# polli-labs/linnaeus

Hardware: AMD Instinct MI355X
Metric: images/sec (train fwd+bwd) mFormerV1_sm 3x224x224 (higher is better)
Workload: dtype bf16; 1 GPU; mFormerV1_sm train step (forward + 4-task CE loss + backward + AdamW (one HIP launch)), bf16 operands / fp32 accumulate+residual, batch 256/GPU, 3x224x224 synthetic, DropPath 0.2, gradient checkpointing off; per_gpu_batch=256, global_batch=256, parallelism=dp1, grad_mode=direct

## Files before the change

include/lnx.h:

```cpp
#ifndef LNX_H
#define LNX_H
#include <stdint.h>

#ifdef __cplusplus
extern "C" {
#endif

#define LNX_F32 0
#define LNX_BF16 1

const char* lnx_last_error(void);
int lnx_version(void);
int lnx_device_cus(void);
int lnx_set_cu_margin(int cus);
int lnx_set_deterministic(int on);
int lnx_get_deterministic(void);
int lnx_tile_sched_static(void);

typedef struct lnx_rowmap {
    int group, pad, off;
} lnx_rowmap;

enum { LNX_ACT_NONE = 0, LNX_ACT_GELU = 1, LNX_ACT_RELU = 2, LNX_ACT_GELU_BWD = 3, LNX_ACT_RELU_BWD = 4,
       LNX_ACT_GELU_D = 5, LNX_ACT_MUL_AUX = 6 };
enum { LNX_ADDR_PLAIN = 0, LNX_ADDR_PATCH2 = 1 };

typedef struct lnx_gemm_args {
    int dtype;
    int M, N, K;
    const void* A;
    int64_t lda;
    const void* W;
    int64_t ldw;
    void* C;
    int64_t ldc;
    int out_f32;
    int a_mode, Hin, Win, Cin;
    int c_mode;
    lnx_rowmap c_map;
    const float* bias;
    void* c2;
    int64_t ldc2;
    int act;
    const void* aux;
    int64_t ldaux;
    const float* gamma;
    const float* rowscale;
    int rows_per_sample;
    const float* res;
    int64_t ldres;
    void* c8;
    int64_t ldc8;
    void* c8_scales;
    const int* m_dev;
    const int* perm;
} lnx_gemm_args;

int lnx_gemm_nt(const lnx_gemm_args* args, void* stream);

#define LNX_GEMM_GROUP_MAX 8
int lnx_gemm_nt_group_ok(const lnx_gemm_args* problems, int n, int accumulate);
int lnx_gemm_nt_group(const lnx_gemm_args* problems, int n, int accumulate, void* stream);

enum { LNX_NT_KERNEL_NONE = 0, LNX_NT_KERNEL_V1 = 1 , LNX_NT_KERNEL_V2 = 2 ,
       LNX_NT_KERNEL_SKINNY = 3 , LNX_NT_KERNEL_V4 = 4 ,
       LNX_NT_KERNEL_FP8 = 6 , LNX_NT_KERNEL_V7 = 7 ,
       LNX_NT_KERNEL_MX8 = 8 , LNX_NT_KERNEL_V9 = 9 ,
       LNX_NT_KERNEL_EXPERIMENT = 15 , LNX_NT_KERNEL_KINDS = 16 };
int lnx_last_nt_kernel(void);
int64_t lnx_nt_kernel_launches(int kind);
int lnx_nt_dispatch(const lnx_gemm_args* args);

int lnx_amax(const void* x, int x_dtype, int64_t ldx, int rows, int cols, float* amax, void* stream);
int lnx_quantize_fp8(const void* x, int x_dtype, int64_t ldx, int rows, int cols, const float* amax, void* y, int64_t ldy, float* scale_out, void* stream);
int lnx_gemm_nt_fp8(const lnx_gemm_args* args, const float* a_scale, const float* w_scale, void* stream);

int lnx_quantize_mxfp8(const void* x, int x_dtype, int64_t ldx, int rows, int cols, void* y, int64_t ldy, void* scales, void* stream);
int lnx_gemm_nt_mxfp8(const lnx_gemm_args* args, const void* a_scales, const void* w_scales, void* stream);

typedef struct lnx_wgrad_args {
    int dtype;
    int M, N, K;
    const void* dY;
    int64_t lddy;
    const void* A;
    int64_t lda;
    int a_mode, Hin, Win, Cin;
    float* dW;
    int64_t lddw;
    int k_perm_c;
    float* db;
    int splits;
    int k_store;
    float* ws;
    int64_t ws_floats;
    int defer;
    const int* m_dev;
} lnx_wgrad_args;
#define LNX_TN_WS_FLOATS (256 * (256 * 128 + 256))

int lnx_gemm_tn(const lnx_wgrad_args* args, void* stream);
enum { LNX_TN_KERNEL_V1 = 1 ,
       LNX_TN_KERNEL_RING = 2  };
typedef struct lnx_tn_launch {
    int kernel;
    int rw, cw;
    int patch;
    int tiles_n, tiles_k;
    int splits;
    int m_per_split;
    int workspace;
} lnx_tn_launch;
int lnx_gemm_tn_query(const lnx_wgrad_args* args, lnx_tn_launch* out);
int lnx_gemm_tn_flush(void* stream);
int lnx_gemm_tn_discard(void);


typedef struct lnx_ln_args {
    int M, C;
    float eps;
    const void* x;
    int x_dtype;
    int64_t ldx;
    lnx_rowmap x_map;
    const float* w;
    const float* b;
    void* y;
    int y_dtype;
    int64_t ldy;
    lnx_rowmap y_map;
    const void* add;
    int64_t ldadd;
    float* mean;
    float* rstd;
    void* y8;
    int64_t ldy8;
    void* y8_scales;
    const int* perm;
    const int* m_dev;
    int rows_per_sample;
} lnx_ln_args;
int lnx_layernorm_fwd(const lnx_ln_args* args, void* stream);

typedef struct lnx_ln_bwd_args {
    int M, C;
    const void* dy;
    int dy_dtype;
    int64_t lddy;
    lnx_rowmap dy_map;
    const void* x;
    int x_dtype;
    int64_t ldx;
    lnx_rowmap x_map;
    const float* w;
    const float* mean;
    const float* rstd;
    const float* gin;
    int64_t ldgin;
    void* dx;
    int dx_dtype;
    int64_t lddx;
    float* dw;
    float* db;
    int relu_mask;
    float* ws;
    int64_t ws_floats;
    void* dx2;
    int dx2_dtype;
    int64_t lddx2;
    const float* dx2_rowscale;
    int dx2_rows_per_sample;
    void* dx2_8;
    void* dx2_8_scales;
    int64_t lddx2_8;
    int defer;
    const int* perm;
    const int* m_dev;
    const int* dx2_inv;
    const int* dx2_nkeep;
} lnx_ln_bwd_args;
int lnx_layernorm_bwd(const lnx_ln_bwd_args* args, void* stream);
int lnx_layernorm_bwd_flush(void* stream);
int lnx_layernorm_bwd_discard(void);

enum { LNX_LN_COLS_NONE = 0 , LNX_LN_COLS_ATOMICS = 1 ,
       LNX_LN_COLS_WORKSPACE = 2  };
typedef struct lnx_ln_launch {
    int G;
    int V;
    int pair;
    int full;
    int mx;
    int grid;
    int cols;
    int slices;
} lnx_ln_launch;
int lnx_layernorm_fwd_query(const lnx_ln_args* args, lnx_ln_launch* out);
int lnx_layernorm_bwd_query(const lnx_ln_bwd_args* args, lnx_ln_launch* out);

typedef struct lnx_dwconv_args {
    int B, H, W, C;
    const void* x;
    int x_dtype;
    const float* w49;
    const float* bias;
    int flip;
    const float* res;
    void* y;
    int y_dtype;
} lnx_dwconv_args;
int lnx_dwconv7_fwd(const lnx_dwconv_args* args, void* stream);
int lnx_dwconv7_fwd_kept(const lnx_dwconv_args* args, const int* perm, const int* nkeep, void* stream);

typedef struct lnx_dwconv_wgrad_args {
    int B, H, W, C;
    const void* x;
    int x_dtype;
    const void* dy;
    int dy_dtype;
    float* dw;
    float* db;
    float* ws;
    int64_t ws_floats;
} lnx_dwconv_wgrad_args;
int lnx_dwconv7_wgrad(const lnx_dwconv_wgrad_args* args, void* stream);
int lnx_dwconv7_wgrad_kept(const lnx_dwconv_wgrad_args* args, const int* perm, const int* nkeep, void* stream);
int64_t lnx_dwconv7_wgrad_ws_floats(int B, int H, int W, int C, int x_dtype, int dy_dtype);

enum { LNX_ROPE_COS = 0, LNX_ROPE_ROTATE = 1 };
int lnx_rope_cos_table(const float* freqs , int heads, int H, int W, float* cos_out ,
                       float* dsin_out ,
                       void* stream);
int lnx_rope_cos_table_hd(const float* freqs, int heads, int head_dim, int H, int W, float* cos_out, float* dsin_out, void* stream);
int lnx_rope_cossin_table_hd(const float* freqs, int heads, int head_dim, int H, int W, float* cos_out, float* sin_out, float* dsin_out, void* stream);
#define LNX_ROPE_TABLES_MAX 24
typedef struct {
    const float* freqs;
    float* cos_out;
    float* dsin_out;
    int heads, H, W;
    int head_dim;
    int rope_mode;
    float* sin_out;
} lnx_rope_table;
int lnx_rope_cos_tables(const lnx_rope_table* tables, int n, void* stream);
int64_t lnx_attn_bwd_ws_floats(int B, int N, int heads);
int64_t lnx_attn_bwd_ws_floats_hd(int B, int N, int heads, int head_dim);

typedef struct lnx_attn_args {
    int dtype;
    int B, N, E, heads;
    const void* qkv;
    const float* cos_tab;
    void* o;
    float* lse;
    const unsigned char* drop_mask;
    float drop_inv_keep;
    int head_dim;
    int rope_mode;
    const float* sin_tab;
} lnx_attn_args;
int lnx_attn_fwd(const lnx_attn_args* args, void* stream);

typedef struct lnx_attn_bwd_args {
    int dtype;
    int B, N, E, heads;
    const void* qkv;
    const float* cos_tab;
// ... 708 lines not shown
```

linnaeus_amd/_lib.py:

```python
from __future__ import annotations

import ctypes as C
import os

_HERE = os.path.dirname(os.path.abspath(__file__))
LIB_PATH = os.environ.get("LNX_LIB_PATH") or os.path.join(_HERE, "liblnx_hip.so")

F32, BF16 = 0, 1
ACT_NONE, ACT_GELU, ACT_RELU, ACT_GELU_BWD, ACT_RELU_BWD, ACT_GELU_D, ACT_MUL_AUX = 0, 1, 2, 3, 4, 5, 6
TN_WS_FLOATS = 256 * (256 * 128 + 256)
DROP_PARTITION_MAX = 64


def drop_list_ints(B: int) -> int:
    return 2 * B + 2
ADDR_PLAIN, ADDR_PATCH2 = 0, 1


class LnxError(RuntimeError):
    pass


class RowMap(C.Structure):
    _fields_ = [("group", C.c_int), ("pad", C.c_int), ("off", C.c_int)]
# ... 203 lines not shown


class HierLossArgs(C.Structure):
    _fields_ = [("dtype", C.c_int), ("B", C.c_int), ("n_tasks", C.c_int), ("prob", C.c_float), ("mask_mul", C.c_int), ("draws", C.c_void_p),
                ("weights", C.c_void_p), ("ws", C.c_void_p), ("out", C.c_void_p), ("counts", C.c_void_p), ("task", HierLossTask * METRICS_MAX_TASKS)]


HIER_ROUTE_SOFT, HIER_ROUTE_HARD, HIER_ROUTE_GUMBEL = range(3)


class HierRefineLevel(C.Structure):
    _fields_ = [("base", C.c_void_p), ("out", C.c_void_p), ("dout", C.c_void_p), ("dbase", C.c_void_p), ("ld", C.c_int64), ("ldd", C.c_int64),
                ("C", C.c_int), ("mode", C.c_int), ("parent", C.c_void_p), ("child_start", C.c_void_p), ("child_idx", C.c_void_p),
                ("noise", C.c_void_p), ("temperature", C.c_float)]


class HierRefineArgs(C.Structure):
    _fields_ = [("dtype", C.c_int), ("B", C.c_int), ("n_tasks", C.c_int), ("stats", C.c_void_p), ("level", HierRefineLevel * METRICS_MAX_TASKS)]


HIER_REFINE_STRUCTS = {"lnx_hier_refine_level": HierRefineLevel, "lnx_hier_refine_args": HierRefineArgs}


ABSTAIN_MULTITASK, ABSTAIN_SEQUENTIAL = range(2)
ABSTAIN_REWARD_SIMPLE, ABSTAIN_REWARD_OUTCOME = range(2)
ABSTAIN_RANKS_ALL, ABSTAIN_RANKS_FIRST = range(2)
ABSTAIN_CORRECT, ABSTAIN_CORRECT_ABSTAIN, ABSTAIN_MISCLASSIFIED, ABSTAIN_UNNECESSARY_ABSTAIN, ABSTAIN_PREDICTED_AT_NULL, ABSTAIN_OUTCOMES = range(6)
(ABSTAIN_CNT_ABSTAINED, ABSTAIN_CNT_TOTAL, ABSTAIN_CNT_CORRECT_ABSTAIN, ABSTAIN_CNT_UNNECESSARY_ABSTAIN, ABSTAIN_CNT_MISSED_ABSTAIN,
 ABSTAIN_CNT_CORRECT_CLASSIFY, ABSTAIN_CNT_MISCLASSIFY) = range(7)
ABSTAIN_CNT_STRIDE, ABSTAIN_CNT_EPISODES, ABSTAIN_CNT_LENGTH_SUM, ABSTAIN_CNT_REWARD_FIX, ABSTAIN_COUNTS = 8, 64, 65, 66, 72
ABSTAIN_REWARD_FIX_BITS = 20
PPO_WS_LSE, PPO_WS_H, PPO_WS_LOGP, PPO_WS_COEF, PPO_WS_ROWS = range(5)
PPO_OUT_POLICY, PPO_OUT_VALUE, PPO_OUT_ENTROPY, PPO_OUT_TOTAL, PPO_OUT_N, PPO_OUT_RATIO_MEAN, PPO_OUT_CLIP_FRAC = range(7)
PPO_OUT_FLOATS = 8


class AbstainRank(C.Structure):
    _fields_ = [("logits", C.c_void_p), ("ld", C.c_int64), ("C", C.c_int), ("abstain_index", C.c_int), ("null_index", C.c_int), ("target", C.c_void_p),
                ("dlogits", C.c_void_p), ("ldd", C.c_int64)]


class AbstainActArgs(C.Structure):
    _fields_ = [("dtype", C.c_int), ("B", C.c_int), ("R", C.c_int), ("mode", C.c_int), ("greedy", C.c_int), ("reward_kind", C.c_int),
                ("reward_ranks", C.c_int), ("table", C.c_float * ABSTAIN_OUTCOMES), ("outcome_reward", C.c_float * 2), ("u", C.c_void_p),
                ("actions", C.c_void_p), ("logp", C.c_void_p), ("entropy", C.c_void_p), ("taken", C.c_void_p), ("length", C.c_void_p),
                ("reward", C.c_void_p), ("counts", C.c_void_p), ("rank", AbstainRank * METRICS_MAX_TASKS)]


class PpoAdvArgs(C.Structure):
    _fields_ = [("B", C.c_int), ("R", C.c_int), ("mode", C.c_int), ("gamma", C.c_float), ("gae_lambda", C.c_float), ("reward", C.c_void_p),
                ("value", C.c_void_p), ("length", C.c_void_p), ("adv", C.c_void_p), ("ret", C.c_void_p), ("n_trans", C.c_void_p)]


class PpoLossArgs(C.Structure):
    _fields_ = [("dtype", C.c_int), ("B", C.c_int), ("R", C.c_int), ("mode", C.c_int), ("clip_eps", C.c_float), ("vf_coef", C.c_float),
                ("ent_coef", C.c_float), ("actions", C.c_void_p), ("taken", C.c_void_p), ("logp_old", C.c_void_p), ("adv", C.c_void_p),
                ("ret", C.c_void_p), ("value", C.c_void_p), ("ws", C.c_void_p), ("out", C.c_void_p), ("dvalue", C.c_void_p),
                ("rank", AbstainRank * METRICS_MAX_TASKS)]


ABSTENTION_STRUCTS = {"lnx_abstain_rank": AbstainRank, "lnx_abstain_act_args": AbstainActArgs, "lnx_ppo_adv_args": PpoAdvArgs,
                      "lnx_ppo_loss_args": PpoLossArgs}


_lib = None


def lib() -> C.CDLL:
    global _lib
    if _lib is None:
        if not os.path.exists(LIB_PATH):
            raise LnxError(
                f"{LIB_PATH} is missing: build it with `python -c 'import __graft_entry__ as g; g.build()'` "
                "(or `make -C linnaeus_amd/csrc`). linnaeus_amd has no CPU fallback."
            )
        _lib = C.CDLL(LIB_PATH)
        _lib.lnx_last_error.restype = C.c_char_p
        _lib.lnx_nt_kernel_launches.restype = C.c_int64
        _lib.lnx_convmlp_bwd_ws_floats.restype = C.c_int64
        _lib.lnx_meta_heads_bwd_part_floats.restype = C.c_int64
        if hasattr(_lib, "lnx_set_deterministic"):
            _lib.lnx_dwconv7_wgrad_ws_floats.restype = C.c_int64
            _lib.lnx_layerscale_bwd_ws_floats.restype = C.c_int64
        _lib.lnx_attn_bwd_ws_floats.restype = C.c_int64
        _lib.lnx_attn_bwd_ws_floats_hd.restype = C.c_int64
        if hasattr(_lib, "lnx_ademamix_step"):
            _lib.lnx_ademamix_step.argtypes = [C.c_void_p, C.c_void_p, C.c_int, C.c_int, C.POINTER(AdEMAMixHyper), C.c_void_p, C.c_float, C.c_void_p]
        if hasattr(_lib, "lnx_sgd_step"):
            _lib.lnx_sgd_step.argtypes = [C.c_void_p, C.c_int, C.c_int, C.POINTER(SGDHyper), C.c_void_p, C.c_float, C.c_void_p]
            _lib.lnx_optim_launches.restype = C.c_int64
        if hasattr(_lib, "lnx_muon_step"):
            _lib.lnx_muon_layout.argtypes = [C.c_void_p, C.c_int, C.c_void_p, C.c_void_p, C.c_int64, C.POINTER(MuonInfo)]
            _lib.lnx_muon_step.argtypes = [C.POINTER(MuonStepArgs), C.c_void_p]
            _lib.lnx_muon_launches.restype = C.c_int64
        if hasattr(_lib, "lnx_muon_partition"):
            _lib.lnx_muon_partition.argtypes = [C.c_void_p, C.c_void_p, C.c_int, C.c_int, C.c_void_p, C.c_void_p, C.POINTER(C.c_int64), C.c_void_p]
            _lib.lnx_muon_orthogonalize.argtypes = [C.POINTER(MuonStepArgs), C.c_void_p, C.c_void_p, C.c_void_p, C.c_int64, C.c_void_p]
            _lib.lnx_muon_apply_packed.argtypes = [C.c_void_p, C.c_void_p, C.c_int, C.c_void_p, C.c_int64, C.c_int, C.POINTER(StepGuard), C.c_void_p]
        if hasattr(_lib, "lnx_grad_sumsq_guarded"):
            guard = C.POINTER(StepGuard)
            _lib.lnx_grad_sumsq_guarded.argtypes = [C.c_void_p, C.c_int, C.c_int, C.c_void_p, C.c_void_p, guard, C.c_void_p]
            _lib.lnx_adamw_step_guarded.argtypes = [C.c_void_p, C.c_int, C.c_int, C.POINTER(AdamWHyper), C.c_void_p, C.c_float, guard, C.c_void_p]
            _lib.lnx_ademamix_step_guarded.argtypes = [C.c_void_p, C.c_void_p, C.c_int, C.c_int, C.POINTER(AdEMAMixHyper), C.c_void_p, C.c_float, guard, C.c_void_p]
            _lib.lnx_sgd_step_guarded.argtypes = [C.c_void_p, C.c_int, C.c_int, C.POINTER(SGDHyper), C.c_void_p, C.c_float, guard, C.c_void_p]
        if hasattr(_lib, "lnx_gradnorm_sumsq"):
            _lib.lnx_gradnorm_sumsq.argtypes = [C.c_void_p, C.c_int, C.c_int, C.c_int, C.c_int64, C.c_void_p, C.c_void_p, C.c_void_p, C.c_void_p]
        if hasattr(_lib, "lnx_metrics_update"):
            _lib.lnx_metrics_update.argtypes = [C.POINTER(MetricsArgs), C.c_void_p]
            _lib.lnx_metrics_table_sizes.argtypes = [C.c_int, C.c_int, C.c_int, C.POINTER(C.c_int64), C.POINTER(C.c_int64)]
        if hasattr(_lib, "lnx_predict"):
            _lib.lnx_predict.argtypes = [C.POINTER(PredictArgs), C.c_void_p]
            _lib.lnx_predict.restype = C.c_int
        if hasattr(_lib, "lnx_hier_loss_fwd"):
            _lib.lnx_hier_loss_fwd.argtypes = [C.POINTER(HierLossArgs), C.c_void_p]
            _lib.lnx_hier_loss_bwd.argtypes = [C.POINTER(HierLossArgs), C.c_void_p, C.c_void_p]
        if hasattr(_lib, "lnx_taxonomy_rows"):
            _lib.lnx_taxonomy_rows.argtypes = [C.POINTER(TaxonomyRowsArgs), C.c_void_p]
        if hasattr(_lib, "lnx_hier_refine_fwd"):
            _lib.lnx_hier_refine_fwd.argtypes = [C.POINTER(HierRefineArgs), C.c_void_p]
            _lib.lnx_hier_refine_bwd.argtypes = [C.POINTER(HierRefineArgs), C.c_void_p]
            _lib.lnx_hier_refine_launches.restype = C.c_int64
        if hasattr(_lib, "lnx_abstain_act"):
            _lib.lnx_abstain_act.argtypes = [C.POINTER(AbstainActArgs), C.c_void_p]
            _lib.lnx_ppo_advantages.argtypes = [C.POINTER(PpoAdvArgs), C.c_void_p]
            _lib.lnx_ppo_loss_fwd.argtypes = [C.POINTER(PpoLossArgs), C.c_void_p]
            _lib.lnx_ppo_loss_bwd.argtypes = [C.POINTER(PpoLossArgs), C.c_void_p, C.c_void_p]
            _lib.lnx_abstain_launches.restype = C.c_int64
        if hasattr(_lib, "lnx_preprocess"):
            _lib.lnx_resize_taps.argtypes = [C.c_int, C.c_int, C.c_int]
            _lib.lnx_resize_coeffs.argtypes = [C.c_int, C.c_int, C.c_int, C.c_void_p, C.c_void_p]
            _lib.lnx_preprocess_scratch_bytes.argtypes = [C.POINTER(PreprocessImage), C.c_int, C.c_int, C.c_int, C.c_int]
            _lib.lnx_preprocess_scratch_bytes.restype = C.c_int64
            _lib.lnx_preprocess.argtypes = [C.POINTER(PreprocessArgs), C.c_void_p]
            _lib.lnx_preprocess.restype = C.c_int
        if hasattr(_lib, "lnx_meta_mask"):
            _lib.lnx_meta_mask.argtypes = [C.POINTER(MetaMaskArgs), C.c_void_p]
            _lib.lnx_meta_mask.restype = C.c_int
        if hasattr(_lib, "lnx_drop_partition"):
            _lib.lnx_drop_partition.argtypes = [C.c_void_p, C.c_int, C.c_int, C.c_char_p, C.POINTER(C.c_int), C.c_void_p, C.c_void_p]
            _lib.lnx_copy_dropped_rows.argtypes = [C.c_void_p, C.c_void_p, C.c_int64, C.c_void_p, C.c_void_p, C.c_int, C.c_int, C.c_int, C.c_void_p]
            _lib.lnx_drop_compact_branches.restype = C.c_int64
            if hasattr(_lib, "lnx_drop_compact_conv_blocks"):
                _lib.lnx_drop_compact_conv_blocks.restype = C.c_int64
                _lib.lnx_dwconv7_fwd_kept.argtypes = [C.POINTER(DwconvArgs), C.c_void_p, C.c_void_p, C.c_void_p]
                _lib.lnx_dwconv7_wgrad_kept.argtypes = [C.POINTER(DwconvWgradArgs), C.c_void_p, C.c_void_p, C.c_void_p]
            _lib.lnx_scale_cast_compact.argtypes = [C.c_void_p, C.c_int64, C.c_void_p, C.c_int, C.c_void_p, C.c_void_p, C.c_void_p, C.c_int, C.c_int64, C.c_int, C.c_int,
                                                    C.c_void_p]
        if hasattr(_lib, "lnx_plan_set_trainable"):
            _lib.lnx_plan_unit_name.argtypes = [C.c_void_p, C.c_int]
            _lib.lnx_plan_unit_name.restype = C.c_char_p
            _lib.lnx_plan_set_trainable.argtypes = [C.c_void_p, C.c_char_p]
        if hasattr(_lib, "lnx_gemm_tn_query"):
            _lib.lnx_gemm_tn_query.argtypes = [C.POINTER(WgradArgs), C.POINTER(TnLaunch)]
        if hasattr(_lib, "lnx_layernorm_fwd_query"):
            _lib.lnx_layernorm_fwd_query.argtypes = [C.POINTER(LnArgs), C.POINTER(LnLaunch)]
            _lib.lnx_layernorm_bwd_query.argtypes = [C.POINTER(LnBwdArgs), C.POINTER(LnLaunch)]
        older = bool(os.environ.get("LNX_LIB_PATH")) and os.environ.get("LNX_LIB_OLDER") == "1"
        for name in EXPORTS:
            if not hasattr(_lib, name) and not older:
                raise LnxError(f"{LIB_PATH} does not export {name}; rebuild it")
    return _lib


def set_deterministic(on: bool) -> bool:
    return bool(lib().lnx_set_deterministic(1 if on else 0))


def is_deterministic() -> bool:
    return bool(lib().lnx_get_deterministic())


def check(rc: int, what: str) -> None:
    if rc != 0:
        raise LnxError(f"{what} failed (rc={rc}): {lib().lnx_last_error().decode()}")


AUG_CLAMP, AUG_POSTERIZE, AUG_SOLARIZE, AUG_SOLARIZE_ADD, AUG_INVERT, AUG_BRIGHTNESS, AUG_CONTRAST = range(7)

NT_KERNEL_NONE, NT_KERNEL_V1, NT_KERNEL_V2, NT_KERNEL_SKINNY, NT_KERNEL_V4, NT_KERNEL_FP8, NT_KERNEL_V7, NT_KERNEL_MX8, NT_KERNEL_V9, NT_KERNEL_EXPERIMENT = 0, 1, 2, 3, 4, 6, 7, 8, 9, 15

ROPE_COS, ROPE_ROTATE = 0, 1

ATTN_KERNEL_NONE, ATTN_KERNEL_RES4, ATTN_KERNEL_RES8, ATTN_KERNEL_TILED4, ATTN_KERNEL_TILED8 = range(5)

EXPORTS = [
    "lnx_last_error", "lnx_version", "lnx_device_cus", "lnx_set_cu_margin", "lnx_set_deterministic", "lnx_get_deterministic", "lnx_tile_sched_static",
    "lnx_gemm_nt", "lnx_last_nt_kernel", "lnx_nt_kernel_launches", "lnx_nt_dispatch", "lnx_gemm_tn", "lnx_gemm_tn_query", "lnx_gemm_tn_flush", "lnx_gemm_tn_discard", "lnx_amax", "lnx_quantize_fp8", "lnx_gemm_nt_fp8", "lnx_quantize_mxfp8", "lnx_gemm_nt_mxfp8", "lnx_dropout_mul", "lnx_dropout_residual", "lnx_plan_dropout_bytes", "lnx_plan_set_dropout", "lnx_plan_attn_dropout_bytes", "lnx_plan_set_attn_dropout",
    "lnx_layernorm_fwd", "lnx_layernorm_bwd", "lnx_layernorm_bwd_flush", "lnx_layernorm_bwd_discard", "lnx_layernorm_fwd_query", "lnx_layernorm_bwd_query",
    "lnx_dwconv7_fwd", "lnx_dwconv7_fwd_kept", "lnx_dwconv7_wgrad", "lnx_dwconv7_wgrad_kept", "lnx_dwconv7_wgrad_ws_floats",
    "lnx_gemm_nt_group_ok", "lnx_gemm_nt_group", "lnx_rope_cos_table", "lnx_rope_cos_table_hd", "lnx_rope_cossin_table_hd", "lnx_rope_cos_tables", "lnx_attn_bwd_ws_floats", "lnx_attn_bwd_ws_floats_hd", "lnx_attn_fwd", "lnx_attn_bwd", "lnx_attn_bwd_sized", "lnx_attn_fwd_compact", "lnx_attn_bwd_compact", "lnx_attn_bwd_flush", "lnx_attn_bwd_discard", "lnx_attn_dispatch", "lnx_last_attn_kernel", "lnx_last_attn_bwd_launches",
    "lnx_im2col_stem", "lnx_scale_cast", "lnx_scale_cast_compact", "lnx_drop_partition", "lnx_copy_dropped_rows", "lnx_set_drop_compact", "lnx_drop_compact_branches", "lnx_drop_compact_conv_blocks", "lnx_layerscale_bwd", "lnx_layerscale_bwd_ws", "lnx_layerscale_bwd_ws_floats", "lnx_layerscale_apply_wgrad", "lnx_fill_rows", "lnx_colsum_rows",
    "lnx_agg2_fwd", "lnx_agg2_bwd", "lnx_pack_meta", "lnx_meta_heads_supported", "lnx_meta_heads_fwd", "lnx_meta_heads_bwd", "lnx_meta_heads_bwd_part_floats", "lnx_prep_weights", "lnx_prep_blocks", "lnx_softce", "lnx_softce_multi", "lnx_taxonomy_rows", "lnx_stem_fwd", "lnx_stem_fwd_ok", "lnx_adamw_blocks", "lnx_grad_sumsq", "lnx_adamw_step", "lnx_ademamix_step", "lnx_sgd_step", "lnx_optim_launches", "lnx_grad_sumsq_guarded", "lnx_adamw_step_guarded", "lnx_ademamix_step_guarded", "lnx_sgd_step_guarded", "lnx_muon_layout", "lnx_muon_step", "lnx_muon_launches", "lnx_muon_partition", "lnx_muon_orthogonalize", "lnx_muon_apply_packed", "lnx_gradnorm_sumsq", "lnx_gradnorm_update",
    "lnx_metrics_table_sizes", "lnx_metrics_update", "lnx_predict", "lnx_resize_taps", "lnx_resize_coeffs", "lnx_preprocess_scratch_bytes", "lnx_preprocess", "lnx_hier_loss_fwd", "lnx_hier_loss_bwd",
    "lnx_hier_refine_fwd", "lnx_hier_refine_bwd", "lnx_hier_refine_launches",
    "lnx_abstain_act", "lnx_ppo_advantages", "lnx_ppo_loss_fwd", "lnx_ppo_loss_bwd", "lnx_abstain_launches",
    "lnx_mix_rows", "lnx_mix_meta", "lnx_meta_mask",
    "lnx_aug_pointwise", "lnx_aug_saturation", "lnx_aug_rowstat", "lnx_aug_rescale", "lnx_aug_affine", "lnx_aug_stencil", "lnx_erase_rects", "lnx_u8hwc_to_f32chw",
    "lnx_convmlp_supported", "lnx_convmlp_fwd", "lnx_convmlp_bwd", "lnx_convmlp_bwd_ws_floats",
    "lnx_plan_create", "lnx_plan_destroy", "lnx_plan_workspace_bytes", "lnx_plan_num_params", "lnx_plan_param_name",
    "lnx_plan_param_numel", "lnx_plan_num_drop_calls", "lnx_plan_logits_numel", "lnx_plan_logits_offset", "lnx_plan_logits_ld",
    "lnx_plan_bind", "lnx_plan_forward", "lnx_plan_backward", "lnx_plan_backward_into", "lnx_plan_segment_params", "lnx_plan_profile_begin", "lnx_plan_profile_end", "lnx_plan_profile_begin_spans", "lnx_plan_profile_end_ex", "lnx_plan_set_wgrad_stream", "lnx_plan_set_meta_stream",
    "lnx_plan_num_units", "lnx_plan_unit_name", "lnx_plan_param_unit", "lnx_plan_set_trainable", "lnx_plan_first_trained_unit", "lnx_plan_last_backward_units",
]


class MetaHeadArgs(C.Structure):
    _fields_ = [
        ("B", C.c_int), ("C", C.c_int), ("dim", C.c_int), ("off", C.c_int),
        ("meta", C.c_void_p), ("meta_width", C.c_int), ("eps", C.c_float),
        ("w0", C.c_void_p), ("ldw0", C.c_int), ("b0", C.c_void_p), ("ln0_w", C.c_void_p), ("ln0_b", C.c_void_p),
        ("w1", C.c_void_p), ("ldw1", C.c_int), ("b1", C.c_void_p), ("ln1_w", C.c_void_p), ("ln1_b", C.c_void_p),
        ("w2", C.c_void_p), ("ldw2", C.c_int), ("b2", C.c_void_p), ("ln2_w", C.c_void_p), ("ln2_b", C.c_void_p),
        ("t0", C.c_void_p), ("h0", C.c_void_p), ("x", C.c_void_p), ("h1", C.c_void_p), ("n1", C.c_void_p), ("h2", C.c_void_p),
        ("m0", C.c_void_p), ("r0", C.c_void_p), ("m1", C.c_void_p), ("r1", C.c_void_p), ("m2", C.c_void_p), ("r2", C.c_void_p),
        ("tok", C.c_void_p), ("tok_row_stride", C.c_int64), ("tok_row_offset", C.c_int64),
    ]


class MetaHeadBwdArgs(C.Structure):
    _fields_ = [
        ("B", C.c_int), ("C", C.c_int), ("dim", C.c_int),
        ("g", C.c_void_p), ("g_row_stride", C.c_int64), ("g_row_offset", C.c_int64),
        ("w1t", C.c_void_p), ("ldw1t", C.c_int), ("w2t", C.c_void_p), ("ldw2t", C.c_int),
        ("ln0_w", C.c_void_p), ("ln1_w", C.c_void_p), ("ln2_w", C.c_void_p),
        ("t0", C.c_void_p), ("h0", C.c_void_p), ("x", C.c_void_p), ("h1", C.c_void_p), ("n1", C.c_void_p), ("h2", C.c_void_p),
        ("m0", C.c_void_p), ("r0", C.c_void_p), ("m1", C.c_void_p), ("r1", C.c_void_p), ("m2", C.c_void_p), ("r2", C.c_void_p),
        ("dp2", C.c_void_p), ("dp1", C.c_void_p), ("dp0", C.c_void_p), ("part", C.c_void_p),
        ("d_w0", C.c_void_p), ("d_b0", C.c_void_p), ("d_ln0_w", C.c_void_p), ("d_ln0_b", C.c_void_p),
        ("d_w1", C.c_void_p), ("d_b1", C.c_void_p), ("d_ln1_w", C.c_void_p), ("d_ln1_b", C.c_void_p),
        ("d_w2", C.c_void_p), ("d_b2", C.c_void_p), ("d_ln2_w", C.c_void_p), ("d_ln2_b", C.c_void_p),
    ]


class LnArgs(C.Structure):
    _fields_ = [
        ("M", C.c_int), ("C", C.c_int), ("eps", C.c_float),
        ("x", C.c_void_p), ("x_dtype", C.c_int), ("ldx", C.c_int64), ("x_map", RowMap),
        ("w", C.c_void_p), ("b", C.c_void_p),
        ("y", C.c_void_p), ("y_dtype", C.c_int), ("ldy", C.c_int64), ("y_map", RowMap),
        ("add", C.c_void_p), ("ldadd", C.c_int64),
        ("mean", C.c_void_p), ("rstd", C.c_void_p),
        ("y8", C.c_void_p), ("ldy8", C.c_int64), ("y8_scales", C.c_void_p),
        ("perm", C.c_void_p), ("m_dev", C.c_void_p), ("rows_per_sample", C.c_int),
    ]


class LnBwdArgs(C.Structure):
    _fields_ = [
        ("M", C.c_int), ("C", C.c_int),
        ("dy", C.c_void_p), ("dy_dtype", C.c_int), ("lddy", C.c_int64), ("dy_map", RowMap),
        ("x", C.c_void_p), ("x_dtype", C.c_int), ("ldx", C.c_int64), ("x_map", RowMap),
        ("w", C.c_void_p), ("mean", C.c_void_p), ("rstd", C.c_void_p),
        ("gin", C.c_void_p), ("ldgin", C.c_int64),
        ("dx", C.c_void_p), ("dx_dtype", C.c_int), ("lddx", C.c_int64),
        ("dw", C.c_void_p), ("db", C.c_void_p), ("relu_mask", C.c_int),
        ("ws", C.c_void_p), ("ws_floats", C.c_int64),
        ("dx2", C.c_void_p), ("dx2_dtype", C.c_int), ("lddx2", C.c_int64), ("dx2_rowscale", C.c_void_p), ("dx2_rows_per_sample", C.c_int),
        ("dx2_8", C.c_void_p), ("dx2_8_scales", C.c_void_p), ("lddx2_8", C.c_int64),
        ("defer", C.c_int),
        ("perm", C.c_void_p), ("m_dev", C.c_void_p), ("dx2_inv", C.c_void_p), ("dx2_nkeep", C.c_void_p),
    ]


LN_COLS_NONE, LN_COLS_ATOMICS, LN_COLS_WORKSPACE = range(3)


class LnLaunch(C.Structure):
    _fields_ = [("G", C.c_int), ("V", C.c_int), ("pair", C.c_int), ("full", C.c_int), ("mx", C.c_int), ("grid", C.c_int), ("cols", C.c_int), ("slices", C.c_int)]


class RopeTable(C.Structure):
    _fields_ = [
        ("freqs", C.c_void_p), ("cos_out", C.c_void_p), ("dsin_out", C.c_void_p),
        ("heads", C.c_int), ("H", C.c_int), ("W", C.c_int), ("head_dim", C.c_int),
        ("rope_mode", C.c_int), ("sin_out", C.c_void_p),
    ]


class DwconvArgs(C.Structure):
    _fields_ = [
        ("B", C.c_int), ("H", C.c_int), ("W", C.c_int), ("C", C.c_int),
        ("x", C.c_void_p), ("x_dtype", C.c_int), ("w49", C.c_void_p), ("bias", C.c_void_p),
        ("flip", C.c_int), ("res", C.c_void_p), ("y", C.c_void_p), ("y_dtype", C.c_int),
    ]


class DwconvWgradArgs(C.Structure):
    _fields_ = [
        ("B", C.c_int), ("H", C.c_int), ("W", C.c_int), ("C", C.c_int),
        ("x", C.c_void_p), ("x_dtype", C.c_int), ("dy", C.c_void_p), ("dy_dtype", C.c_int),
        ("dw", C.c_void_p), ("db", C.c_void_p),
        ("ws", C.c_void_p), ("ws_floats", C.c_int64),
    ]


class AttnArgs(C.Structure):
    _fields_ = [
        ("dtype", C.c_int), ("B", C.c_int), ("N", C.c_int), ("E", C.c_int), ("heads", C.c_int),
        ("qkv", C.c_void_p), ("cos_tab", C.c_void_p), ("o", C.c_void_p), ("lse", C.c_void_p),
        ("drop_mask", C.c_void_p), ("drop_inv_keep", C.c_float), ("head_dim", C.c_int),
        ("rope_mode", C.c_int), ("sin_tab", C.c_void_p),
    ]


class AttnBwdArgs(C.Structure):
    _fields_ = [
        ("dtype", C.c_int), ("B", C.c_int), ("N", C.c_int), ("E", C.c_int), ("heads", C.c_int),
        ("qkv", C.c_void_p), ("cos_tab", C.c_void_p), ("o", C.c_void_p), ("lse", C.c_void_p),
        ("d_o", C.c_void_p), ("dqkv", C.c_void_p), ("freq_ws", C.c_void_p), ("delta", C.c_void_p),
        ("drop_mask", C.c_void_p), ("drop_inv_keep", C.c_float),
        ("dsin_tab", C.c_void_p), ("dfreqs", C.c_void_p), ("defer_freqs", C.c_int), ("head_dim", C.c_int),
        ("rope_mode", C.c_int), ("sin_tab", C.c_void_p), ("grid_w", C.c_int),
    ]


class PrepDesc(C.Structure):
    _fields_ = [
        ("src", C.c_void_p), ("dst", C.c_void_p), ("dst_t", C.c_void_p),
        ("rows", C.c_int), ("cols", C.c_int), ("ld", C.c_int), ("ld_t", C.c_int),
        ("P", C.c_int), ("mode", C.c_int), ("block_start", C.c_int),
    ]


PREP_CAST, PREP_CONV_PERM, PREP_DW49 = 0, 1, 2


class ConvMlpArgs(C.Structure):
    _fields_ = [
        ("dtype", C.c_int), ("M", C.c_int), ("C", C.c_int),
        ("ln", C.c_void_p), ("w1", C.c_void_p), ("b1", C.c_void_p), ("w2", C.c_void_p), ("b2", C.c_void_p),
        ("gamma", C.c_void_p), ("rowscale", C.c_void_p), ("rows_per_sample", C.c_int),
        ("x", C.c_void_p), ("out", C.c_void_p), ("z", C.c_void_p),
        ("y", C.c_void_p), ("ln_w", C.c_void_p), ("ln_b", C.c_void_p), ("ln_eps", C.c_float), ("ln_out", C.c_void_p),
        ("mean", C.c_void_p), ("rstd", C.c_void_p),
        ("perm", C.c_void_p), ("m_dev", C.c_void_p),
    ]


class ConvMlpBwdArgs(C.Structure):
    _fields_ = [
# ... 37 lines not shown
```

linnaeus_amd/csrc/api.cpp:

```cpp
#include <hip/hip_runtime.h>
#include <stdarg.h>
#include <stdio.h>
#include <stdlib.h>
#include <string.h>

#include <atomic>
#include <mutex>

#include "../../include/lnx.h"

static thread_local char g_err[1024] = "";

void lnx_set_error(const char* fmt, ...) {
    va_list ap;
    va_start(ap, fmt);
    vsnprintf(g_err, sizeof(g_err), fmt, ap);
    va_end(ap);
}

extern "C" const char* lnx_last_error(void) { return g_err; }
extern "C" int lnx_version(void) { return 118; }
extern "C" int lnx_device_cus(void) {
    int dev = 0;
    if (hipGetDevice(&dev) != hipSuccess) return -1;
    hipDeviceProp_t prop;
    if (hipGetDeviceProperties(&prop, dev) != hipSuccess) return -1;
    return prop.multiProcessorCount;
}

static std::atomic<int> g_cu_margin{-1};
int persistent_cus(int cus) {
    int m = g_cu_margin.load(std::memory_order_relaxed);
    if (m < 0) {
        const char* e = getenv("LNX_CU_MARGIN");
        m = e ? atoi(e) : 0;
        if (m < 0) m = 0;
        g_cu_margin.store(m, std::memory_order_relaxed);
    }
    const int room = cus - m;
    return room < 8 ? 8 : room;
}
void set_cu_margin(int m) { g_cu_margin.store(m < 0 ? 0 : m, std::memory_order_relaxed); }
static std::atomic<int> g_deterministic{-1};
bool deterministic() {
    int d = g_deterministic.load(std::memory_order_relaxed);
    if (d < 0) {
        const char* e = getenv("LNX_DETERMINISTIC");
        d = e && atoi(e) == 1 ? 1 : 0;
        int unset = -1;
        if (!g_deterministic.compare_exchange_strong(unset, d, std::memory_order_relaxed)) d = unset;
    }
    return d != 0;
}
extern "C" int lnx_get_deterministic(void) { return deterministic() ? 1 : 0; }
extern "C" int lnx_set_deterministic(int on) {
    const int prev = deterministic() ? 1 : 0;
    g_deterministic.store(on ? 1 : 0, std::memory_order_relaxed);
    return prev;
}
bool tile_sched_static() {
    if (deterministic()) return true;
    const char* e = getenv("LNX_TILE_SCHED");
    return e && strcmp(e, "static") == 0;
}
extern "C" int lnx_tile_sched_static(void) { return tile_sched_static() ? 1 : 0; }
int tile_slot_of(hipStream_t st) {
    static std::mutex mu;
    static hipStream_t known[64];
    static int n = 0;
    std::lock_guard<std::mutex> lock(mu);
    for (int i = 0; i < n; ++i)
        if (known[i] == st) return i;
    if (n < 64) {
        known[n] = st;
        return n++;
    }
    return -1;
}
int device_cus() {
    static std::atomic<int> cached{0};
    int c = cached.load(std::memory_order_relaxed);
    if (c == 0) {
        c = lnx_device_cus();
        if (c > 0) cached.store(c, std::memory_order_relaxed);
    }
    return c > 0 ? c : 0;
}
extern "C" int lnx_set_cu_margin(int cus) {
    if (cus < 0 || cus > 1024) {
        lnx_set_error("lnx_set_cu_margin: %d (0..1024 compute units)", cus);
        return 1;
    }
    set_cu_margin(cus);
    return 0;
}
```

linnaeus_amd/csrc/gemm2.hip:

```cpp
#include "gemm_common.hpp"

namespace lnxg {

template <bool OUT_F32, bool PATCH, int F>
__global__ __launch_bounds__(512) void gemm_nt_v2_kernel(const GemmP p_host) {
    typedef bf16_t T;
    typedef NarrowRing R;
    constexpr int BK = R::BK;
    extern __shared__ __attribute__((aligned(16))) unsigned char smem[];

    const int tid = threadIdx.x;
    const int lane = tid & 63;
    const int wave = __builtin_amdgcn_readfirstlane(tid >> 6);
    const int wm = wave >> 1, wn = wave & 1;
    const int s = lane & 15, g = lane >> 4;

    GemmP p = p_host;
    effective_rows(p);
    int m0, n0;
    one_shot_origin<R::BM, R::BN>(p, m0, n0);
    if (m0 >= p.M) return;

    const unsigned char* src[R::PIECES];
#pragma unroll
// ... 84 lines not shown
}

template <bool OUT_F32, int F>
__global__ __launch_bounds__(512) void gemm_nt_v4_kernel(const GemmP p_host) {
    typedef bf16_t T;
    typedef WideRing R;
    extern __shared__ __attribute__((aligned(16))) unsigned char smem[];

    const int tid = threadIdx.x;
    const int lane = tid & 63;
    const int wave = __builtin_amdgcn_readfirstlane(tid >> 6);
    const int wm = wave & 1, wn = wave >> 1;
    const int s = lane & 15, g = lane >> 4;

    GemmP p = p_host;
    effective_rows(p);
    int m0, n0;
    one_shot_origin<R::BM, R::BN>(p, m0, n0);
    if (m0 >= p.M) return;

    const unsigned char* src[R::PIECES];
#pragma unroll
    for (int j = 0; j < R::PIECES; ++j) {
        const int i = wave + 8 * j;
        const int row = R::ROWS_PER_PIECE * i + (lane >> R::CHUNK_SHIFT);
        const int slot = lane & (R::CHUNKS - 1);
        if (row < R::BM) {
            const int chunk = slot ^ R::key(row);
            int m = m0 + row;
            if (m >= p.M) m = p.M - 1;
            src[j] = p.A + ((int64_t)m * p.lda + chunk * 8) * 2;
        } else {
            const int wr = row - R::BM;
            const int chunk = slot ^ R::key(wr);
            int n = n0 + wr;
            if (n >= p.N) n = p.N - 1;
            src[j] = p.W + ((int64_t)n * p.ldw + chunk * 8) * 2;
        }
    }
    auto issue_stage = [&](int kt, int stage) {
#pragma unroll
        for (int j = 0; j < R::PIECES; ++j) {
            const int i = wave + 8 * j;
            __builtin_amdgcn_global_load_lds((const __attribute__((address_space(1))) void*)(src[j] + (int64_t)kt * R::BK * 2),
                                             (__attribute__((address_space(3))) void*)(smem + stage * R::STAGE + i * 1024), 16, 0, 0);
        }
    };

    const int frag_row = (s >> 2) * 16 + (s & 3);
    const uint32_t chunk_off = (uint32_t)((g ^ (((s >> 2) & 1) * 3)) << 4);
    const uint32_t lds_base = (uint32_t)(uintptr_t)(__attribute__((address_space(3))) unsigned char*)smem;
    const uint32_t a_off = (uint32_t)((wm * 128 + frag_row) * R::ROWBYTES) + chunk_off;
    const uint32_t w_off = (uint32_t)((R::BM + wn * 64 + frag_row) * R::ROWBYTES) + chunk_off;

    f32x4_t acc0[4][4], acc1[4][4];
#pragma unroll
    for (int i = 0; i < 4; ++i)
#pragma unroll
        for (int j = 0; j < 4; ++j) {
            acc0[i][j] = f32x4_t{0.f, 0.f, 0.f, 0.f};
            acc1[i][j] = f32x4_t{0.f, 0.f, 0.f, 0.f};
        }

    const int nk = p.K / R::BK;
    issue_stage(0, 0);
    issue_stage(1, 1);
    issue_stage(2, 2);
    const int grp = wave >> 2;
    asm volatile("s_waitcnt vmcnt(8)" ::: "memory");
    __builtin_amdgcn_s_barrier();
    if (grp) __builtin_amdgcn_s_barrier();
    for (int kt = 0; kt < nk; ++kt) {
        const uint32_t st = lds_base + (kt % R::NST) * R::STAGE;
        uint4 wf[4], af0[4], af1[4];
        lds_read4<R::ROWBYTES>(wf, st + w_off);
        lds_read4<R::ROWBYTES>(af0, st + a_off);
        lds_read4<R::ROWBYTES>(af1, st + a_off + 64 * R::ROWBYTES);
        if (kt + 3 < nk) {
            issue_stage(kt + 3, (kt + 3) % R::NST);
            asm volatile("s_waitcnt vmcnt(8)" ::: "memory");
        } else if (kt + 2 < nk) {
            asm volatile("s_waitcnt vmcnt(4)" ::: "memory");
        } else {
            asm volatile("s_waitcnt vmcnt(0)" ::: "memory");
        }
        asm volatile("s_waitcnt lgkmcnt(0)" ::: "memory");
        __builtin_amdgcn_s_barrier();
        __builtin_amdgcn_sched_barrier(0);
        __builtin_amdgcn_s_setprio(1);
#pragma unroll
        for (int ni = 0; ni < 4; ++ni)
#pragma unroll
            for (int mi = 0; mi < 4; ++mi) Mfma<T>::run(acc0[ni][mi], wf[ni], af0[mi]);
#pragma unroll
        for (int ni = 0; ni < 4; ++ni)
#pragma unroll
            for (int mi = 0; mi < 4; ++mi) Mfma<T>::run(acc1[ni][mi], wf[ni], af1[mi]);
        __builtin_amdgcn_s_setprio(0);
        __builtin_amdgcn_sched_barrier(0);
        if (!(grp && kt + 1 == nk)) __builtin_amdgcn_s_barrier();
    }
    if (F == F_GENERIC) {
        gemm_epilogue<T, OUT_F32>(p, acc0, m0 + wm * 128, n0 + wn * 64, lane);
        gemm_epilogue<T, OUT_F32>(p, acc1, m0 + wm * 128 + 64, n0 + wn * 64, lane);
    } else {
        gemm_epilogue_fast<T, OUT_F32, F>(p, acc0, m0 + wm * 128, n0 + wn * 64, lane);
        gemm_epilogue_fast<T, OUT_F32, F>(p, acc1, m0 + wm * 128 + 64, n0 + wn * 64, lane);
    }
}

constexpr bool nt_v2_carries(bool out_f32, int f) { return f == F_GENERIC || nt_v4_carries(out_f32, f); }

int launch_nt_v4(const GemmP& p0, int f, bool out_f32, hipStream_t st) {
    typedef WideRing R;
    GemmP p = p0;
    p.tiles_m = cdiv(p.M, R::BM);
    p.tiles_n = p.N / R::BN;
    const int grid = p.tiles_m * p.tiles_n;
    return with_nt_form<nt_v4_carries>("gemm_nt_v4", out_f32, f, [&](auto form) {
        using Form = decltype(form);
        return launch_with_lds<gemm_nt_v4_kernel<Form::out_f32, Form::f>>(grid, 512, R::NST * R::STAGE, st, p);
    });
}

int launch_nt_v2(const GemmP& p0, int f, bool out_f32, hipStream_t st) {
    typedef NarrowRing R;
    GemmP p = p0;
    p.tiles_m = cdiv(p.M, R::BM);
    p.tiles_n = cdiv(p.N, R::BN);
    const int grid = p.tiles_m * p.tiles_n;
    const size_t lds = R::NST * R::STAGE;
    const bool patch = p.a_mode == LNX_ADDR_PATCH2;
    LNX_CHECK(!patch || f == F_GENERIC, "gemm_nt_v2: the 2x2 patch gather is compiled with the generic epilogue only (f = %d)", f);
    return with_nt_form<nt_v2_carries>("gemm_nt_v2", out_f32, f, [&](auto form) {
        using Form = decltype(form);
        if constexpr (Form::f == F_GENERIC) {
            if (patch) return launch_with_lds<gemm_nt_v2_kernel<Form::out_f32, true, Form::f>>(grid, 512, lds, st, p);
        }
        return launch_with_lds<gemm_nt_v2_kernel<Form::out_f32, false, Form::f>>(grid, 512, lds, st, p);
    });
}

constexpr int TBM = 64;
__device__ const uint4 g_tn_zero16 = {0u, 0u, 0u, 0u};

#define DS_READ_TR2(lo, hi, addr, off2)                                                                                  \
    do {                                                                                                                 \
        const uint32_t a_ = (addr);                                                                                      \
        asm volatile("ds_read_b64_tr_b16 %0, %1" : "=v"(lo) : "v"(a_) : "memory");                                       \
        asm volatile("ds_read_b64_tr_b16 %0, %1 offset:%2" : "=v"(hi) : "v"(a_), "i"(off2) : "memory");                 \
    } while (0)

template <int RW, int CW, bool PATCH>
__global__ __launch_bounds__(512) void gemm_tn_v2_kernel(const WgradP p) {
    typedef bf16_t T;
    constexpr int RROW = RW * 2, CROW = CW * 2;
    constexpr int RBYTES = TBM * RROW, CBYTES = TBM * CROW;
    constexpr int STG = RBYTES + CBYTES;
    constexpr int RINS = RBYTES / 1024, CINS = CBYTES / 1024;
    constexpr int NINS = (RINS + CINS) / 8;
    constexpr int WC = CW / 64;
    extern __shared__ __attribute__((aligned(16))) unsigned char smem[];

    const int tid = threadIdx.x;
    const int lane = tid & 63;
    const int wave = __builtin_amdgcn_readfirstlane(tid >> 6);
    const int wr = wave / WC, wc = wave % WC;
    const int s = lane & 15, g = lane >> 4;

    int bid = xcd_remap(blockIdx.x, p.tiles_n * p.tiles_k * p.splits);
    const int split = bid / (p.tiles_n * p.tiles_k);
    bid -= split * (p.tiles_n * p.tiles_k);
    const int tc = bid % p.tiles_k;
    const int tr = bid / p.tiles_k;
    const int n0 = tr * RW, k0 = tc * CW;
    int m_all = p.M, m_per = p.m_per_split;
    if (p.m_dev) {
        m_all = min(p.M, max(*p.m_dev, 0));
        const int mt = (m_all + TBM - 1) / TBM;
        m_per = (mt + p.splits - 1) / p.splits * TBM;
    }
    const int m_begin = split * m_per;
    const int m_end = min(m_all, m_begin + m_per);
    if (m_begin >= m_end && !(p.m_dev && p.ws)) return;
    const int ntile = m_begin < m_end ? (m_end - m_begin + TBM - 1) / TBM : 0;

    const unsigned char* src[NINS];
    int64_t step[NINS];
    int pr[NINS], po[NINS];
    const int Wo = PATCH ? p.pg.Win >> 1 : 1;
    const int qa = TBM / Wo, qb = TBM - qa * Wo;
#pragma unroll
    for (int j = 0; j < NINS; ++j) {
        pr[j] = po[j] = 0;
        const int i = wave + 8 * j;
        if (i < RINS) {
            constexpr int CPR = RW / 8, RPI = 64 / CPR;
            const int row = i * RPI + lane / CPR, slot = lane % CPR;
            int col = n0 + ((slot ^ ((row & 7) << 1)) << 3);
            const int lim = ((p.N + 7) >> 3) << 3;
            if (col >= lim) col = lim - 8;
            src[j] = p.dY + ((int64_t)(m_begin + row) * p.lddy + col) * 2;
            step[j] = (int64_t)TBM * p.lddy * 2;
        } else {
            constexpr int CPR = CW / 8, RPI = 64 / CPR;
            const int row = (i - RINS) * RPI + lane / CPR, slot = lane % CPR;
            int col = k0 + ((slot ^ ((row & 7) << 1)) << 3);
            const int lim = ((p.K + 7) >> 3) << 3;
            if (col >= lim) col = lim - 8;
            if (PATCH) {
                src[j] = p.A + patch_col(p.pg, col) * 2;
                step[j] = (int64_t)p.pg.Cin * 4;
                const int m = m_begin + row, t = m / Wo;
                pr[j] = m - t * Wo;
                po[j] = m + t * Wo;
            } else {
                src[j] = p.A + ((int64_t)(m_begin + row) * p.lda + col) * 2;
                step[j] = (int64_t)TBM * p.lda * 2;
            }
        }
    }
    int m_issue = m_begin;
    auto issue_tile = [&](int stage) {
        const bool ragged = m_issue + TBM > m_end;
#pragma unroll
        for (int j = 0; j < NINS; ++j) {
            const int i = wave + 8 * j;
            const unsigned char* gp = src[j];
            if (PATCH && i >= RINS) {
                gp += (int64_t)po[j] * step[j];
                const int r = pr[j] + qb;
                const bool wrap = r >= Wo;
                pr[j] = wrap ? r - Wo : r;
                po[j] += TBM + (qa + (wrap ? 1 : 0)) * Wo;
            } else {
                src[j] += step[j];
            }
            if (ragged) {
                const int row = i < RINS ? i * (64 / (RW / 8)) + lane / (RW / 8) : (i - RINS) * (64 / (CW / 8)) + lane / (CW / 8);
                if (m_issue + row >= m_end) gp = reinterpret_cast<const unsigned char*>(&g_tn_zero16);
            }
            __builtin_amdgcn_global_load_lds((const __attribute__((address_space(1))) void*)gp,
                                             (__attribute__((address_space(3))) void*)(smem + stage * STG + i * 1024), 16, 0, 0);
        }
        m_issue += TBM;
    };

    const int q = s >> 2, pp = s & 3;
    uint32_t offR[2][4], offC[2][4];
#pragma unroll
    for (int ks = 0; ks < 2; ++ks) {
        const int row = ks * 32 + 4 * g + q;
        const int key = (row & 7) << 1;
#pragma unroll
        for (int i = 0; i < 4; ++i) {
            const int cr = (wr * 64 + i * 16 + 4 * pp) >> 3, cc = (wc * 64 + i * 16 + 4 * pp) >> 3;
            offR[ks][i] = row * RROW + ((cr ^ key) << 4) + (pp & 1) * 8;
            offC[ks][i] = RBYTES + row * CROW + ((cc ^ key) << 4) + (pp & 1) * 8;
        }
    }
    const uint32_t lds_base = (uint32_t)(uintptr_t)(__attribute__((address_space(3))) unsigned char*)smem;

    f32x4_t acc[4][4], accb[4];
#pragma unroll
    for (int i = 0; i < 4; ++i) {
        accb[i] = f32x4_t{0.f, 0.f, 0.f, 0.f};
#pragma unroll
        for (int j = 0; j < 4; ++j) acc[i][j] = f32x4_t{0.f, 0.f, 0.f, 0.f};
    }
    const bool do_bias = p.db != nullptr && tc == 0 && wc == 0;
    const uint4 ones = make_uint4(0x3F803F80u, 0x3F803F80u, 0x3F803F80u, 0x3F803F80u);

    if (ntile > 0) issue_tile(0);
    if (ntile > 1) issue_tile(1);
    const int grp = wave >> 2;
    if (ntile > 1) asm volatile("s_waitcnt vmcnt(6)" ::: "memory");
    else asm volatile("s_waitcnt vmcnt(0)" ::: "memory");
    __builtin_amdgcn_s_barrier();
    if (grp && ntile > 0) __builtin_amdgcn_s_barrier();
    for (int t = 0; t < ntile; ++t) {
        const uint32_t st = lds_base + (t % NarrowRing::NST) * STG;
        uint2 rl[2][4], rh[2][4], cl[2][4], chh[2][4];
#pragma unroll
        for (int ks = 0; ks < 2; ++ks)
#pragma unroll
            for (int i = 0; i < 4; ++i) {
                DS_READ_TR2(rl[ks][i], rh[ks][i], st + offR[ks][i], 16 * RROW);
                DS_READ_TR2(cl[ks][i], chh[ks][i], st + offC[ks][i], 16 * CROW);
            }
        if (t + 2 < ntile) {
            issue_tile((t + 2) % NarrowRing::NST);
            asm volatile("s_waitcnt vmcnt(6)" ::: "memory");
        } else {
            asm volatile("s_waitcnt vmcnt(0)" ::: "memory");
        }
        asm volatile("s_waitcnt lgkmcnt(0)" ::: "memory");
        __builtin_amdgcn_s_barrier();
        __builtin_amdgcn_sched_barrier(0);
        __builtin_amdgcn_s_setprio(1);
#pragma unroll
        for (int ks = 0; ks < 2; ++ks) {
            uint4 rf[4], cf[4];
#pragma unroll
            for (int i = 0; i < 4; ++i) {
                rf[i] = make_uint4(rl[ks][i].x, rl[ks][i].y, rh[ks][i].x, rh[ks][i].y);
                cf[i] = make_uint4(cl[ks][i].x, cl[ks][i].y, chh[ks][i].x, chh[ks][i].y);
            }
#pragma unroll
            for (int ri = 0; ri < 4; ++ri)
#pragma unroll
                for (int ci = 0; ci < 4; ++ci) Mfma<T>::run(acc[ri][ci], rf[ri], cf[ci]);
            if (do_bias) {
#pragma unroll
                for (int ri = 0; ri < 4; ++ri) Mfma<T>::run(accb[ri], rf[ri], ones);
            }
        }
        __builtin_amdgcn_s_setprio(0);
        __builtin_amdgcn_sched_barrier(0);
        if (!(grp && t + 1 == ntile)) __builtin_amdgcn_s_barrier();
    }
    if (p.ws) {
        const int tiles = p.tiles_n * p.tiles_k;
        float4* wt = reinterpret_cast<float4*>(p.ws + (size_t)(split * tiles + tr * p.tiles_k + tc) * (RW * CW)) + (wave * 16) * 64 + lane;
#pragma unroll
        for (int ri = 0; ri < 4; ++ri)
#pragma unroll
            for (int ci = 0; ci < 4; ++ci) wt[(ri * 4 + ci) * 64] = make_float4(acc[ri][ci][0], acc[ri][ci][1], acc[ri][ci][2], acc[ri][ci][3]);
        if (do_bias && s == 0) {
#pragma unroll
            for (int ri = 0; ri < 4; ++ri)
#pragma unroll
                for (int r = 0; r < 4; ++r)
                    p.ws[(size_t)p.splits * tiles * (RW * CW) + (size_t)(split * p.tiles_n + tr) * RW + wr * 64 + ri * 16 + 4 * g + r] = accb[ri][r];
        }
        return;
    }
#pragma unroll
    for (int ri = 0; ri < 4; ++ri) {
#pragma unroll
        for (int r = 0; r < 4; ++r) {
            const int n = n0 + wr * 64 + ri * 16 + 4 * g + r;
            if (n >= p.N) continue;
#pragma unroll
            for (int ci = 0; ci < 4; ++ci) {
                const int k = k0 + wc * 64 + ci * 16 + s;
                if (k >= p.k_store) continue;
                int col = k;
                if (p.k_perm_c > 0) {
                    const int P = p.K / p.k_perm_c;
                    const int pq = k / p.k_perm_c;
                    col = (k - pq * p.k_perm_c) * P + pq;
                }
                atomicAdd(p.dW + (int64_t)n * p.lddw + col, acc[ri][ci][r]);
            }
            if (do_bias && s == 0) atomicAdd(p.db + n, accb[ri][r]);
        }
    }
}

__device__ __forceinline__ void tn_reduce_body(const WgradP& p, int RW, int CW, const int64_t idx) {
    const int tiles = p.tiles_n * p.tiles_k;
    const int tile_f4 = RW * CW / 4;
    const size_t tile_floats = (size_t)RW * CW;
    if (idx < (int64_t)tiles * tile_f4) {
        const int tile = (int)(idx / tile_f4), f = (int)(idx - (int64_t)tile * tile_f4);
        const int tr = tile / p.tiles_k, tc = tile - tr * p.tiles_k;
        const int lane = f & 63, ci = (f >> 6) & 3, ri = (f >> 8) & 3, wave = f >> 10;
        const int WC = CW / 64, wr = wave / WC, wc = wave - wr * WC;
        const int n0 = tr * RW + wr * 64 + ri * 16 + 4 * (lane >> 4);
        const int k = tc * CW + wc * 64 + ci * 16 + (lane & 15);
        if (n0 >= p.N || k >= p.k_store) return;
        const float4* src = reinterpret_cast<const float4*>(p.ws + (size_t)tile * tile_floats) + f;
        float4 part[8];
#pragma unroll
        for (int j = 0; j < 8; ++j) part[j] = make_float4(0.f, 0.f, 0.f, 0.f);
        const size_t sstep = (size_t)tiles * tile_floats / 4;
        int sp = 0;
        for (; sp + 8 <= p.splits; sp += 8) {
            float4 v[8];
#pragma unroll
            for (int j = 0; j < 8; ++j) v[j] = src[(size_t)(sp + j) * sstep];
#pragma unroll
            for (int j = 0; j < 8; ++j) {
                part[j].x += v[j].x;
                part[j].y += v[j].y;
                part[j].z += v[j].z;
                part[j].w += v[j].w;
            }
        }
        for (; sp < p.splits; ++sp) {
            const float4 v = src[(size_t)sp * sstep];
            part[0].x += v.x;
            part[0].y += v.y;
            part[0].z += v.z;
            part[0].w += v.w;
        }
#pragma unroll
        for (int w = 4; w > 0; w >>= 1)
#pragma unroll
            for (int j = 0; j < w; ++j) {
                part[j].x += part[j + w].x;
                part[j].y += part[j + w].y;
                part[j].z += part[j + w].z;
                part[j].w += part[j + w].w;
            }
        const float av[4] = {part[0].x, part[0].y, part[0].z, part[0].w};
        int col = k;
        if (p.k_perm_c > 0) {
            const int P = p.K / p.k_perm_c;
            const int pq = k / p.k_perm_c;
            col = (k - pq * p.k_perm_c) * P + pq;
        }
#pragma unroll
        for (int r = 0; r < 4; ++r)
            if (n0 + r < p.N) p.dW[(int64_t)(n0 + r) * p.lddw + col] += av[r];
    } else if (p.db != nullptr) {
        const int64_t n = idx - (int64_t)tiles * tile_f4;
        if (n < p.N) {
            const int tr = (int)n / RW;
            const float* src = p.ws + (size_t)p.splits * tiles * tile_floats + (size_t)tr * RW + (n - tr * RW);
            float a = 0.f;
            for (int sp = 0; sp < p.splits; ++sp) a += src[(size_t)sp * p.tiles_n * RW];
            p.db[n] += a;
        }
    }
}

__global__ __launch_bounds__(256) void gemm_tn_reduce_kernel(const WgradP p, int RW, int CW) {
    tn_reduce_body(p, RW, CW, (int64_t)blockIdx.x * 256 + threadIdx.x);
}

constexpr int TN_BATCH = 8;
struct TnReduceDesc {
    WgradP p;
    int RW, CW, block_start;
};
struct TnReduceBatch {
    TnReduceDesc d[TN_BATCH];
    int n;
};
__global__ __launch_bounds__(256) void gemm_tn_reduce_batch_kernel(const TnReduceBatch b) {
    int j = 0;
#pragma unroll
    for (int i = 1; i < TN_BATCH; ++i)
        if (i < b.n && (int)blockIdx.x >= b.d[i].block_start) j = i;
    tn_reduce_body(b.d[j].p, b.d[j].RW, b.d[j].CW, (int64_t)((int)blockIdx.x - b.d[j].block_start) * 256 + threadIdx.x);
}

static thread_local TnReduceBatch g_tn_pending = {};
static thread_local int g_tn_pending_blocks = 0;
static thread_local hipStream_t g_tn_pending_stream = nullptr;

int tn_flush(hipStream_t st) {
    if (g_tn_pending.n == 0) return 0;
    if (st != nullptr && st != g_tn_pending_stream) return 1;
    hipLaunchKernelGGL(gemm_tn_reduce_batch_kernel, dim3((unsigned)g_tn_pending_blocks), dim3(256), 0, g_tn_pending_stream, g_tn_pending);
    g_tn_pending.n = 0;
    g_tn_pending_blocks = 0;
    return 0;
}

int tn_discard() {
    const int n = g_tn_pending.n;
    g_tn_pending.n = 0;
    g_tn_pending_blocks = 0;
    g_tn_pending_stream = nullptr;
    return n;
}

int launch_tn_v2(const WgradP& p, const TnPlan& t, hipStream_t st, bool defer) {
    static_assert(TBM == TN_RING_ROWS, "tn_plan splits the contraction in this kernel's ring stages");
    const bool wide_r = t.RW == 256, patch = t.patch;
    const int RW = t.RW, CW = t.CW;
    const int tiles = p.tiles_n * p.tiles_k;
    const int grid = tiles * p.splits;
    const size_t lds = NarrowRing::NST * (size_t)(TBM * (RW + CW) * 2);
    int rc;
    if (wide_r) rc = patch ? launch_with_lds<gemm_tn_v2_kernel<256, 128, true>>(grid, 512, lds, st, p) : launch_with_lds<gemm_tn_v2_kernel<256, 128, false>>(grid, 512, lds, st, p);
    else rc = patch ? launch_with_lds<gemm_tn_v2_kernel<128, 256, true>>(grid, 512, lds, st, p) : launch_with_lds<gemm_tn_v2_kernel<128, 256, false>>(grid, 512, lds, st, p);
    if (rc != 0) return rc;
    if (p.ws) {
        const int64_t work = (int64_t)tiles * (RW * CW / 4) + (p.db ? p.N : 0);
        const int blocks = (int)cdiv(work, 256);
        if (defer) {
            if (g_tn_pending.n > 0 && (g_tn_pending_stream != st || g_tn_pending.n == TN_BATCH)) (void)tn_flush(nullptr);
            TnReduceDesc& d = g_tn_pending.d[g_tn_pending.n++];
            d.p = p;
            d.RW = RW;
            d.CW = CW;
            d.block_start = g_tn_pending_blocks;
            g_tn_pending_blocks += blocks;
            g_tn_pending_stream = st;
        } else {
            hipLaunchKernelGGL(gemm_tn_reduce_kernel, dim3((unsigned)blocks), dim3(256), 0, st, p, RW, CW);
        }
    }
    return 0;
}

}
```

linnaeus_amd/csrc/gemm_common.hpp:

```cpp
#pragma once
#include "common.hpp"
#include "../../include/lnx.h"

namespace lnxg {

constexpr int TILE = 128;
constexpr int ROWB = 128;
constexpr int TILE_BYTES = TILE * ROWB;

struct PatchGeom {
    int Hin, Win, Cin;
};

struct GemmP {
    const unsigned char* A;
    const unsigned char* W;
    unsigned char* C;
    unsigned char* C2;
    const unsigned char* aux;
    const float* bias;
    const float* gamma;
    const float* rowscale;
    const float* res;
    int64_t lda, ldw, ldc, ldc2, ldaux, ldres;
// ... 430 lines not shown
    if (p.N % 16 != 0 || !al16(p.C) || (p.ldc * (out_f32 ? 4 : esz)) % 16 != 0) return F_GENERIC;
    const int64_t lim = (int64_t)1 << 31;
    if ((int64_t)p.M * p.ldc >= lim) return F_GENERIC;
    int f = 0;
    if (p.bias) {
        if (!al16(p.bias)) return F_GENERIC;
        f |= F_BIAS;
    }
    if (p.C2) {
        if (!al16(p.C2) || (p.ldc2 * esz) % 16 != 0 || (int64_t)p.M * p.ldc2 >= lim) return F_GENERIC;
        f |= F_C2;
    }
    if (p.act == LNX_ACT_GELU) f |= F_GELU;
    else if (p.act == LNX_ACT_GELU_D) {
        if (!p.C2) return F_GENERIC;
        f |= F_GELU;
    } else if (p.act == LNX_ACT_GELU_BWD || p.act == LNX_ACT_MUL_AUX) {
        if (!al16(p.aux) || (p.ldaux * esz) % 16 != 0 || (int64_t)p.M * p.ldaux >= lim) return F_GENERIC;
        f |= F_GELU_BWD;
    } else if (p.act != LNX_ACT_NONE) return F_GENERIC;
    if (p.res) {
        if (!al16(p.res) || (p.ldres * 4) % 16 != 0 || (int64_t)p.M * p.ldres >= lim) return F_GENERIC;
        f |= F_RES;
    }
    if (p.rowscale && !p.res) return F_GENERIC;
    if (!out_f32 && (f == 0 || f == F_BIAS || f == (F_BIAS | F_C2 | F_GELU) || f == (F_BIAS | F_GELU) || f == F_GELU_BWD)) return f;
    if (out_f32 && f == (F_BIAS | F_RES)) return f;
    return F_GENERIC;
}

struct WgradP {
    const unsigned char* dY;
    const unsigned char* A;
    float* dW;
    float* db;
    int64_t lddy, lda, lddw;
    int M, N, K;
    int a_mode;
    PatchGeom pg;
    int k_perm_c, k_store;
    float* ws;
    int64_t ws_floats;
    int tiles_n, tiles_k, splits, m_per_split;
    const int* m_dev = nullptr;
};


struct NtSwitches {
    bool force_v1;
    bool skinny;
    bool v4;
    bool tile_cost;
    bool generic_epi;
    int v7, v9;
    bool fp8_x8;
};
NtSwitches nt_switches();

void fill_gemm_p(const lnx_gemm_args* a, GemmP& p);

struct NtChoice {
    int kind, f;
};
NtChoice nt_choose(const GemmP& p, int dtype, bool out_f32);

typedef int (*nt_experiment_fn)(const GemmP& p, int f, bool out_f32, hipStream_t st);
extern nt_experiment_fn g_nt_experiment;

void note_nt_kernel(int kind);

template <bool O, int FF>
struct NtForm {
    static constexpr bool out_f32 = O;
    static constexpr int f = FF;
};
int nt_form_error(const char* family, bool out_f32, int f);

template <auto Carries, bool O, int FF, class Launch>
int nt_form_case(const char* family, Launch& launch) {
    if constexpr (Carries(O, FF)) return launch(NtForm<O, FF>{});
    else return nt_form_error(family, O, FF);
}

template <auto Carries, class Launch>
int with_nt_form(const char* family, bool out_f32, int f, Launch&& launch) {
    if (f == F_GENERIC) return out_f32 ? nt_form_case<Carries, true, F_GENERIC>(family, launch) : nt_form_case<Carries, false, F_GENERIC>(family, launch);
    if (out_f32) {
        if (f == (F_BIAS | F_RES)) return nt_form_case<Carries, true, F_BIAS | F_RES>(family, launch);
        return nt_form_error(family, out_f32, f);
    }
    switch (f) {
        case 0: return nt_form_case<Carries, false, 0>(family, launch);
        case F_BIAS: return nt_form_case<Carries, false, F_BIAS>(family, launch);
        case F_BIAS | F_C2 | F_GELU: return nt_form_case<Carries, false, F_BIAS | F_C2 | F_GELU>(family, launch);
        case F_BIAS | F_C2 | F_GELU | F_MXOUT: return nt_form_case<Carries, false, F_BIAS | F_C2 | F_GELU | F_MXOUT>(family, launch);
        case F_BIAS | F_GELU: return nt_form_case<Carries, false, F_BIAS | F_GELU>(family, launch);
        case F_GELU_BWD: return nt_form_case<Carries, false, F_GELU_BWD>(family, launch);
        case F_GELU_BWD | F_MXOUT: return nt_form_case<Carries, false, F_GELU_BWD | F_MXOUT>(family, launch);
    }
    return nt_form_error(family, out_f32, f);
}

int launch_nt_v1(const GemmP& p, int dtype, bool out_f32, hipStream_t st);
int launch_tn_v1(const WgradP& p, int dtype, hipStream_t st);

bool nt_skinny_ok(const GemmP& p, int dtype, bool out_f32);
int launch_nt_skinny(const GemmP& p, bool out_f32, hipStream_t st);
int launch_nt_skinny_group(const GemmP* ps, int n, bool accumulate, bool out_f32, hipStream_t st);

int launch_nt_v2(const GemmP& p, int f, bool out_f32, hipStream_t st);
int launch_nt_v4(const GemmP& p, int f, bool out_f32, hipStream_t st);

constexpr bool nt_v4_carries(bool out_f32, int f) {
    if (out_f32) return f == (F_BIAS | F_RES);
    return f == 0 || f == F_BIAS || f == (F_BIAS | F_C2 | F_GELU) || f == (F_BIAS | F_GELU) || f == F_GELU_BWD;
}

inline bool fits_32bit_offsets(const GemmP& p) {
    const int64_t lim = (int64_t)1 << 31;
    return (int64_t)p.M * p.lda * 2 < lim && (int64_t)p.N * p.ldw * 2 < lim;
}
template <class R>
int persistent_geometry(GemmP& p, hipStream_t st, size_t& lds) {
    const int ntiles = p.tiles_m * p.tiles_n;
    const int cus = device_cus();
    if (cus <= 0) return 0;
    const int room = persistent_cus(cus);
    lds = R::NST * R::STAGE + 16;
    p.tile_slot = tile_sched_static() ? -1 : tile_slot_of(st);
    return ntiles < room ? ntiles : room;
}

bool nt_v7_ok(const GemmP& p, int f, bool out_f32);
int launch_nt_v7(const GemmP& p, int f, bool out_f32, hipStream_t st);

bool nt_v9_ok(const GemmP& p, int f, bool out_f32);
int launch_nt_v9(const GemmP& p, int f, bool out_f32, hipStream_t st);

constexpr int TN_RING_ROWS = 64;
struct TnPlan {
    bool ring;
    int RW, CW;
    bool patch;
    int tiles_n, tiles_k, splits, m_per_split;
    bool workspace;
};
TnPlan tn_plan(const WgradP& p, int dtype, int splits_hint);

int launch_tn_v2(const WgradP& p, const TnPlan& t, hipStream_t st, bool defer);
int tn_flush(hipStream_t st);
int tn_discard();
bool tn_v2_ok(const WgradP& p, int dtype);

}
using namespace lnxg;
```

linnaeus_amd/csrc/gemm_tn_dispatch.cpp:

```cpp
#include <stdlib.h>

#include "gemm_common.hpp"

namespace lnxg {

bool tn_v2_ok(const WgradP& p, int dtype) {
    return dtype == LNX_BF16 && p.M % TN_RING_ROWS == 0 && p.M >= 4096 && p.N >= 8 && p.K >= 8;
}

TnPlan tn_plan(const WgradP& p, int dtype, int splits_hint) {
    TnPlan t{};
    t.patch = p.a_mode == LNX_ADDR_PATCH2;
    t.ring = tn_v2_ok(p, dtype) && !nt_switches().force_v1;
    if (!t.ring) {
        t.RW = t.CW = TILE;
        t.tiles_n = cdiv(p.N, TILE);
        t.tiles_k = cdiv(p.K, TILE);
        const int bmc = dtype == LNX_BF16 ? 64 : 32;
        int splits = splits_hint;
        if (splits <= 0) {
            const int tiles = t.tiles_n * t.tiles_k;
            splits = cdiv(2 * 256, tiles);
            const int max_splits = cdiv(p.M, 4 * bmc);
            if (splits > max_splits) splits = max_splits;
            if (splits < 1) splits = 1;
        }
        if (deterministic()) splits = 1;
        int mps = cdiv(p.M, splits);
        mps = cdiv(mps, bmc) * bmc;
        t.splits = cdiv(p.M, mps);
        t.m_per_split = mps;
        t.workspace = false;
        return t;
    }
    auto waste = [&](int rw, int cw) { return (double)cdiv(p.N, rw) * rw * cdiv(p.K, cw) * cw; };
    static const char* force = getenv("LNX_TN_ORIENT");
    const bool wide_r = force ? force[0] == 'r' : waste(256, 128) <= waste(128, 256);
    const int RW = wide_r ? 256 : 128, CW = wide_r ? 128 : 256;
    t.RW = RW;
    t.CW = CW;
    t.tiles_n = cdiv(p.N, RW);
    t.tiles_k = cdiv(p.K, CW);
    const int tiles = t.tiles_n * t.tiles_k;
    const int mtiles = p.M / TN_RING_ROWS;
    int splits = splits_hint;
    if (splits <= 0) {
        splits = 256 / tiles;
        if (splits < 1) splits = 1;
        const int max_splits = mtiles / 8 > 0 ? mtiles / 8 : 1;
        if (splits > max_splits) splits = max_splits;
    }
    if (splits > mtiles) splits = mtiles;
    if (splits < 1) splits = 1;
    const bool det = deterministic();
    auto ws_need = [&](int sp) { return (size_t)sp * tiles * (256 * 128) + (size_t)sp * t.tiles_n * RW; };
    const size_t have = p.ws ? (size_t)p.ws_floats : 0;
    if (det) {
        while (splits > 1 && ws_need(cdiv(mtiles, cdiv(mtiles, splits))) > have) --splits;
    }
    const int per = cdiv(mtiles, splits);
    t.m_per_split = per * TN_RING_ROWS;
    t.splits = cdiv(mtiles, per);
    static const bool no_ws = getenv("LNX_TN_ATOMIC") != nullptr;
    const bool sparse_tiles = (double)p.N * p.k_store < 0.7 * (double)tiles * (256 * 128);
    if (det) t.workspace = t.splits >= 2;
    else t.workspace = !(no_ws || p.ws == nullptr || have < ws_need(t.splits) || t.splits < 2 || sparse_tiles);
    return t;
}

}

namespace {

int tn_check_sizes(const lnx_wgrad_args* a, const char* who) {
    LNX_CHECK(a != nullptr, "%s: null args", who);
    LNX_CHECK(a->dtype == LNX_F32 || a->dtype == LNX_BF16, "%s: bad dtype %d", who, a->dtype);
    const int epv = a->dtype == LNX_F32 ? 4 : 8;
    LNX_CHECK(a->M > 0 && a->N > 0 && a->K > 0, "%s: empty problem", who);
    LNX_CHECK(a->lddy % epv == 0 && a->lddy >= (int64_t)cdiv(a->N, epv) * epv, "%s: lddy=%lld must be a multiple of %d and >= roundup(N)", who, (long long)a->lddy, epv);
    LNX_CHECK(a->K % epv == 0, "%s: K=%d must be a multiple of %d", who, a->K, epv);
    if (a->a_mode == LNX_ADDR_PATCH2) {
        LNX_CHECK(a->Hin % 2 == 0 && a->Win % 2 == 0 && a->Cin % epv == 0 && a->K == 4 * a->Cin, "%s: bad PATCH2 geometry", who);
    } else {
        LNX_CHECK(a->lda % epv == 0, "%s: lda must be a multiple of %d", who, epv);
    }
    if (a->k_perm_c > 0) LNX_CHECK(a->K % a->k_perm_c == 0, "%s: K %% k_perm_c != 0", who);
    return 0;
}

void fill_wgrad_p(const lnx_wgrad_args* a, WgradP& p) {
    p.dY = (const unsigned char*)a->dY;
    p.A = (const unsigned char*)a->A;
    p.dW = a->dW;
    p.db = a->db;
    p.lddy = a->lddy;
    p.lda = a->lda;
    p.lddw = a->lddw;
    p.M = a->M;
    p.N = a->N;
    p.K = a->K;
    p.a_mode = a->a_mode;
    p.pg = PatchGeom{a->Hin, a->Win, a->Cin};
    p.k_perm_c = a->k_perm_c;
    p.ws = a->ws;
    p.ws_floats = a->ws ? a->ws_floats : 0;
    p.k_store = (a->k_store > 0 && a->k_store < a->K) ? a->k_store : a->K;
    p.m_dev = a->m_dev;
}

}

extern "C" int lnx_gemm_tn_query(const lnx_wgrad_args* a, lnx_tn_launch* out) {
    LNX_CHECK(out != nullptr, "lnx_gemm_tn_query: null result");
    if (tn_check_sizes(a, "lnx_gemm_tn_query") != 0) return 1;
    WgradP p;
    fill_wgrad_p(a, p);
    const TnPlan t = tn_plan(p, a->dtype, a->splits);
    out->kernel = t.ring ? LNX_TN_KERNEL_RING : LNX_TN_KERNEL_V1;
    out->rw = t.RW;
    out->cw = t.CW;
    out->patch = t.patch ? 1 : 0;
    out->tiles_n = t.tiles_n;
    out->tiles_k = t.tiles_k;
    out->splits = t.splits;
    out->m_per_split = t.m_per_split;
    out->workspace = t.workspace ? 1 : 0;
    return 0;
}

extern "C" int lnx_gemm_tn(const lnx_wgrad_args* a, void* stream) {
    if (tn_check_sizes(a, "lnx_gemm_tn") != 0) return 1;
    LNX_CHECK(a->dY && a->A && a->dW, "lnx_gemm_tn: null operand");
    LNX_CHECK((((uintptr_t)a->A) & 15) == 0 && (((uintptr_t)a->dY) & 15) == 0, "lnx_gemm_tn: operands must be 16-byte aligned");
    WgradP p;
    fill_wgrad_p(a, p);
    const TnPlan t = tn_plan(p, a->dtype, a->splits);
    p.tiles_n = t.tiles_n;
    p.tiles_k = t.tiles_k;
    p.splits = t.splits;
    p.m_per_split = t.m_per_split;
    if (t.ring && !t.workspace) p.ws = nullptr;
    hipStream_t st = (hipStream_t)stream;
    static const bool no_defer = getenv("LNX_TN_NO_DEFER") != nullptr;
    int rc;
    if (t.ring) rc = launch_tn_v2(p, t, st, a->defer != 0 && !no_defer);
    else rc = launch_tn_v1(p, a->dtype, st);
    if (rc != 0) return rc;
    LNX_LAUNCH_CHECK();
    return 0;
}
```

linnaeus_amd/csrc/plan.cpp:

```cpp
#include <hip/hip_runtime.h>
#include <stdlib.h>
#include <string.h>

#include <mutex>
#include <atomic>
#include <string>
#include <vector>

#include "../../include/lnx.h"

void lnx_set_error(const char* fmt, ...);

#define RUN(expr)                  \
    do {                           \
        const int rc_ = (expr);    \
        if (rc_ != 0) return rc_;  \
    } while (0)
#define FAIL(...)                   \
    do {                            \
        lnx_set_error(__VA_ARGS__); \
        return 1;                   \
    } while (0)
#define HIPRUN(expr)                                                         \
    do {                                                                     \
        const hipError_t e_ = (expr);                                        \
        if (e_ != hipSuccess) FAIL("%s: %s", #expr, hipGetErrorString(e_)); \
    } while (0)

namespace {

constexpr int LN_DEFER_SLOTS = 16;
constexpr int FREQ_DEFER_SLOTS = 8;

inline int64_t align_up(int64_t v, int64_t a) { return (v + a - 1) / a * a; }

struct OpW {
    int param = -1;
    int N = 0, K = 0;
    int ld = 0;
    int ld_t = 0;
    int mode = LNX_PREP_CAST, P = 0;
    bool f32 = false;
    int64_t off = 0, off_t = 0;
    int64_t off8 = 0, off8s = 0;
    int64_t off8t = 0, off8ts = 0;
};

struct ConvBlk {
    bool fused = false;
    bool fused_ln = false;
    int gamma, dww, dwb, lnw, lnb, b1, b2;
    OpW w1, w2;
    int64_t w49;
    int64_t xin, y, ln, mean, rstd, hpre, act, z;
};
struct RopeBlk {
    int n1w, n1b, n2w, n2b, freqs, qkvb, projb, fc1b, fc2b;
    OpW qkv, proj, fc1, fc2;
    int64_t xin, n1, mean1, rstd1, qkvbuf, cos, dsin, o, lse, xmid, n2, mean2, rstd2, hpre, act;
    int64_t dm_proj = 0, dm_hid = 0, dm_fc2 = 0;
    int64_t dm_attn = 0;
};
struct MetaHead {
    int b0, lnw0, lnb0, nf1w, nf1b, nf2w, nf2b, b1, b2;
    OpW w0, w1, w2;
    int dim, off;
    int64_t t0, h0, x, m0, r0, h1, n1, m1, r1, h2, m2, r2;
    int64_t dp2 = 0, dp1 = 0, dp0 = 0, part = 0;
};
struct Down {
    int lnw, lnb, cb;
    OpW w;
    int64_t ln, mean, rstd;
};

}

constexpr int TN_WS_SLOTS = 4;

struct lnx_plan {
    lnx_mformer_cfg c;
    int esz;
    int E;
    int H[4], W[4], HW[4];
    int Ntok[2];
    std::vector<std::string> names;
    std::vector<int64_t> numel;
    std::vector<signed char> seg;
    std::vector<std::string> unit_names;
    std::vector<int> unit_of;
    int u_conv[2] = {0, 0}, u_down[2] = {0, 0}, u_tok[2] = {0, 0}, u_rope[2] = {0, 0}, u_mid = 0, u_tail = 0, u_heads = 0;
    int cut = 0;
    bool frozen_prefix = true;
    int bwd_units = 0;
    bool runs(int unit) const { return unit >= cut; }
    std::vector<const float*> P;
    std::vector<float*> G;
    bool bound = false, has_grads = false, fwd_done = false;
    unsigned char* ws = nullptr;
    int64_t ws_bytes = 0;

    int stem_b, stem_lnw, stem_lnb, cls[2], norm_w[2], norm_b[2], fin_w, fin_b, agg_w, agg_b, cl_b1, cl_b2, cl_lnw, cl_lnb;
    OpW stem_w, cl_w1, cl_w2;
    std::vector<int> head_b;
    std::vector<OpW> head_w;
    std::vector<int> logit_ld;
    std::vector<int64_t> logit_off;
    int64_t logits_numel = 0;
    Down down[3];
    std::vector<ConvBlk> conv[2];
    std::vector<RopeBlk> rope[2];
    std::vector<MetaHead> meta[2];
    std::vector<OpW*> all_w;
    std::vector<int> drop_conv[2], drop_attn[2], drop_mlp[2];
    int n_drop = 0;

    int64_t o_descs = 0, n_descs = 0, prep_blocks = 0;
    int64_t arena_end = 0;
    int64_t n_descs_t = 0, n_descs_f = 0, prep_blocks_f = 0;
    int64_t o_patches, o_stem_pre, o_stem_mean, o_stem_rstd;
    int64_t o_stage_out[4];
    int64_t o_tok[2];
    int64_t o_t1, o_t1_mean, o_t1_rstd;
    int64_t o_cl_hpre, o_cl_act, o_cl_u, o_cl_mean, o_cl_rstd, o_c1n;
    int64_t o_c2n, o_n2_mean, o_n2_rstd, o_agg, o_fin_mean, o_fin_rstd, o_feats, o_featsT;
    int64_t o_g[4];
    int64_t o_sA, o_sB = 0, o_sC, o_sD;
    int64_t o_lnws = 0, lnws_floats = 0, o_lnws_side = 0, lnws_side_floats = 0;
    int64_t lnws_defer_floats = 0;
    int64_t o_lnws_defer = 0;
    int ln_pending = 0;
    int64_t gcos_floats = 0;
    int freq_pending = 0;
    bool freq_defer = true;
    bool ln_defer = true;
    int64_t o_tnws = 0;
    int64_t o_lsws = 0, lsws_floats = 0;
    bool det = false;
    int64_t o_detws = 0, detws_floats = 0;
    int64_t o_gcos , o_delta, o_dt1, o_tail[6], o_mtmp[4], o_dlT;
    int64_t o_a8 = 0, o_a8s = 0, o_h8 = 0, o_h8s = 0;
    const float* last_drop = nullptr;
    const unsigned char* last_mask = nullptr;
    std::vector<unsigned char> mask_host;
    const float* last_meta = nullptr;
    int resident[4] = {-1, -1, -1, -1};
    const unsigned char* dmask = nullptr;
    float inv_keep = 1.0f;
    int64_t dmask_bytes = 0;
    const unsigned char* amask = nullptr;
    float a_inv_keep = 1.0f;
    int64_t amask_bytes = 0;
    hipStream_t side = nullptr;
    hipEvent_t ev_fork = nullptr, ev_meta = nullptr, ev_bfork[2] = {nullptr, nullptr}, ev_bjoin[2] = {nullptr, nullptr};
    hipStream_t wgs = nullptr;
    bool wgs_on = true;
    bool meta_forked[2] = {false, false};
    int meta_mode = 1;
    bool meta_chain = true;
    bool chain_ok[2] = {false, false};
    bool dy8_ready = false;
    hipEvent_t ev_wf[4] = {nullptr, nullptr, nullptr, nullptr}, ev_wj[4] = {nullptr, nullptr, nullptr, nullptr};
    bool profile = false;
    bool profile_spans = false;
    struct Span { hipEvent_t e0, e1; int cls; double work, bytes; };
    std::vector<Span> spans;
    std::vector<hipEvent_t> ev_pool;
    size_t ev_used = 0;

    template <typename U> U* at(int64_t off) const { return reinterpret_cast<U*>(ws + off); }
    const float* drop_ptr(int call) const {
        if (last_drop == nullptr || call < 0 || !mask_host[call]) return nullptr;
        return last_drop + (int64_t)call * c.batch;
    }
    int* droplists = nullptr;
    bool compact_now = false;
    bool compact_conv_now = false;
    const int* drop_list(int call) const {
        if (!compact_now || droplists == nullptr || drop_ptr(call) == nullptr) return nullptr;
        return droplists + (int64_t)call * LNX_DROP_LIST_INTS(c.batch);
    }
};

static std::atomic<int> g_drop_compact{-1};
static std::atomic<long long> g_compact_branches{0};
extern "C" int lnx_set_drop_compact(int on) {
    const int was = g_drop_compact.exchange(on < 0 ? -1 : (on ? 1 : 0));
    return was;
}
extern "C" int64_t lnx_drop_compact_branches(void) { return (int64_t)g_compact_branches.load(std::memory_order_relaxed); }
static std::atomic<long long> g_compact_conv_blocks{0};
extern "C" int64_t lnx_drop_compact_conv_blocks(void) { return (int64_t)g_compact_conv_blocks.load(std::memory_order_relaxed); }

namespace {

bool env_set(const char* name) { return getenv(name) != nullptr; }
bool env_off(const char* name) {
    const char* e = getenv(name);
    return e != nullptr && atoi(e) == 0;
}

OpW make_w(lnx_plan* p, int param, int N, int K, bool want_t, int mode = LNX_PREP_CAST, int P = 0, bool f32 = false) {
    OpW w;
    w.param = param;
    w.N = N;
    w.K = K;
    w.f32 = f32 || p->esz == 4;
    const int epv = w.f32 ? 4 : 8;
    w.ld = (int)align_up(K, epv);
    if (K < 16) w.ld = 16;
    w.ld_t = want_t ? (int)align_up(N, epv) : 0;
    w.mode = mode;
    w.P = P;
    return w;
}

void build_params(lnx_plan* p) {
    const lnx_mformer_cfg& c = p->c;
    const int* D = c.dims;
    const int B = c.batch;
    char b[128];
    auto add = [&](const std::string& name, int64_t numel, int seg) {
        p->names.push_back(name);
        p->numel.push_back(numel);
        p->seg.push_back((signed char)seg);
        return (int)p->names.size() - 1;
    };
    p->cls[0] = add("cls_token_1", D[2], 1);
    p->cls[1] = add("cls_token_2", D[3], 0);
    p->stem_w = make_w(p, add("stem.0.weight", (int64_t)D[0] * c.in_chans * 16, 3), D[0], c.in_chans * 16, false);
    p->stem_w.ld = 64;
    p->stem_b = add("stem.0.bias", D[0], 3);
    p->stem_lnw = add("stem.1.weight", D[0], 3);
    p->stem_lnb = add("stem.1.bias", D[0], 3);
    for (int i = 0; i < 3; ++i) {
        snprintf(b, sizeof b, "downsample_layers.%d.", i);
        const std::string pre(b);
        Down& k = p->down[i];
        const int seg = 2 - i;
        k.lnw = add(pre + "norm.weight", D[i], seg);
        k.lnb = add(pre + "norm.bias", D[i], seg);
        k.w = make_w(p, add(pre + "conv.weight", (int64_t)D[i + 1] * D[i] * 4, seg), D[i + 1], 4 * D[i], true, LNX_PREP_CONV_PERM, 4);
        k.cb = add(pre + "conv.bias", D[i + 1], seg);
    }
    int call = 0;
    for (int s = 0; s < 2; ++s) {
        p->conv[s].resize(c.conv_depths[s]);
        for (int i = 0; i < c.conv_depths[s]; ++i) {
            snprintf(b, sizeof b, "stages.%d.%d.", s, i);
            const std::string pre(b);
            ConvBlk& k = p->conv[s][i];
            const int C = D[s], seg = 3 - s;
            k.gamma = add(pre + "gamma", C, seg);
            k.dww = add(pre + "dwconv.weight", (int64_t)C * 49, seg);
            k.dwb = add(pre + "dwconv.bias", C, seg);
            k.lnw = add(pre + "norm.weight", C, seg);
            k.lnb = add(pre + "norm.bias", C, seg);
            k.w1 = make_w(p, add(pre + "pwconv1.weight", (int64_t)4 * C * C, seg), 4 * C, C, true);
            k.b1 = add(pre + "pwconv1.bias", 4 * C, seg);
            k.w2 = make_w(p, add(pre + "pwconv2.weight", (int64_t)4 * C * C, seg), C, 4 * C, true);
            k.b2 = add(pre + "pwconv2.bias", C, seg);
            p->drop_conv[s].push_back(call++);
        }
    }
    for (int s = 0; s < 2; ++s) {
        p->rope[s].resize(c.rope_depths[s]);
        for (int i = 0; i < c.rope_depths[s]; ++i) {
            snprintf(b, sizeof b, "stages.%d.%d.", s + 2, i);
            const std::string pre(b);
            RopeBlk& k = p->rope[s][i];
            const int C = D[2 + s], hid = c.mlp_hidden[s], seg = 1 - s;
            k.n1w = add(pre + "norm1.weight", C, seg);
            k.n1b = add(pre + "norm1.bias", C, seg);
            k.n2w = add(pre + "norm2.weight", C, seg);
            k.n2b = add(pre + "norm2.bias", C, seg);
            k.freqs = add(pre + "attn.freqs", C, seg);
            k.qkv = make_w(p, add(pre + "attn.qkv.weight", (int64_t)3 * C * C, seg), 3 * C, C, true);
            k.qkvb = add(pre + "attn.qkv.bias", 3 * C, seg);
            k.proj = make_w(p, add(pre + "attn.proj.weight", (int64_t)C * C, seg), C, C, true);
            k.projb = add(pre + "attn.proj.bias", C, seg);
            k.fc1 = make_w(p, add(pre + "mlp.fc1.weight", (int64_t)hid * C, seg), hid, C, true);
            k.fc1b = add(pre + "mlp.fc1.bias", hid, seg);
            k.fc2 = make_w(p, add(pre + "mlp.fc2.weight", (int64_t)C * hid, seg), C, hid, true);
            k.fc2b = add(pre + "mlp.fc2.bias", C, seg);
            p->drop_attn[s].push_back(call++);
            p->drop_mlp[s].push_back(call++);
        }
    }
    p->n_drop = call;
    for (int s = 0; s < 2; ++s) {
        snprintf(b, sizeof b, "norm_%d.", s + 1);
        p->norm_w[s] = add(std::string(b) + "weight", D[2 + s], 0);
        p->norm_b[s] = add(std::string(b) + "bias", D[2 + s], 0);
        p->meta[s].resize(c.n_meta);
    }
    int off = 0;
    for (int m = 0; m < c.n_meta; ++m) {
        for (int s = 0; s < 2; ++s) {
            snprintf(b, sizeof b, "meta.%d.head_%d.", m, s + 1);
            const std::string pre(b);
            MetaHead& k = p->meta[s][m];
            const int C = D[2 + s], seg = 2 - s;
            k.dim = c.meta_dims[m];
            k.off = off;
            k.w0 = make_w(p, add(pre + "0.weight", (int64_t)C * k.dim, seg), C, k.dim, false, LNX_PREP_CAST, 0, true);
            k.b0 = add(pre + "0.bias", C, seg);
            k.lnw0 = add(pre + "2.weight", C, seg);
            k.lnb0 = add(pre + "2.bias", C, seg);
            k.nf1w = add(pre + "3.norm_fn1.weight", C, seg);
            k.nf1b = add(pre + "3.norm_fn1.bias", C, seg);
            k.nf2w = add(pre + "3.norm_fn2.weight", C, seg);
            k.nf2b = add(pre + "3.norm_fn2.bias", C, seg);
            k.w1 = make_w(p, add(pre + "3.w1.weight", (int64_t)C * C, seg), C, C, true, LNX_PREP_CAST, 0, true);
            k.b1 = add(pre + "3.w1.bias", C, seg);
            k.w2 = make_w(p, add(pre + "3.w2.weight", (int64_t)C * C, seg), C, C, true, LNX_PREP_CAST, 0, true);
            k.b2 = add(pre + "3.w2.bias", C, seg);
        }
        off += c.meta_dims[m];
    }
    if (!c.only_last_cls) {
        p->cl_w1 = make_w(p, add("cl_1_fc.0.fc1.weight", (int64_t)D[2] * D[2], 0), D[2], D[2], true);
        p->cl_b1 = add("cl_1_fc.0.fc1.bias", D[2], 0);
        p->cl_w2 = make_w(p, add("cl_1_fc.0.fc2.weight", (int64_t)D[3] * D[2], 0), D[3], D[2], true);
        p->cl_b2 = add("cl_1_fc.0.fc2.bias", D[3], 0);
        p->cl_lnw = add("cl_1_fc.1.weight", D[3], 0);
        p->cl_lnb = add("cl_1_fc.1.bias", D[3], 0);
        p->agg_w = add("aggregate.weight", 2, 0);
        p->agg_b = add("aggregate.bias", 1, 0);
    }
    p->fin_w = add("final_norm.weight", D[3], 0);
    p->fin_b = add("final_norm.bias", D[3], 0);
    p->head_w.resize(c.n_tasks);
    p->head_b.resize(c.n_tasks);
    p->logit_ld.resize(c.n_tasks);
    p->logit_off.resize(c.n_tasks);
    for (int t = 0; t < c.n_tasks; ++t) {
        snprintf(b, sizeof b, "head.%d.", t);
        p->head_w[t] = make_w(p, add(std::string(b) + "weight", (int64_t)c.task_classes[t] * D[3], 0), c.task_classes[t], D[3], true);
        p->head_b[t] = add(std::string(b) + "bias", c.task_classes[t], 0);
        p->logit_ld[t] = (int)align_up(c.task_classes[t], 8);
        p->head_w[t].ld_t = p->logit_ld[t];
        p->logit_off[t] = p->logits_numel;
        p->logits_numel += (int64_t)B * p->logit_ld[t];
    }
}

bool build_units(lnx_plan* p) {
    const lnx_mformer_cfg& c = p->c;
    char b[64];
    auto unit = [&](const std::string& name) {
        p->unit_names.push_back(name);
        return (int)p->unit_names.size() - 1;
    };
    auto blocks = [&](int stage, int depth) {
        const int first = (int)p->unit_names.size();
        for (int i = 0; i < depth; ++i) {
            snprintf(b, sizeof b, "stages.%d.%d", stage, i);
            unit(b);
        }
        return first;
    };
    unit("stem");
    for (int s = 0; s < 2; ++s) {
        p->u_conv[s] = blocks(s, c.conv_depths[s]);
        snprintf(b, sizeof b, "downsample_layers.%d", s);
        p->u_down[s] = unit(b);
    }
    p->u_tok[0] = unit("tokens_1");
    p->u_rope[0] = blocks(2, c.rope_depths[0]);
    p->u_mid = unit("mid");
    p->u_tok[1] = unit("tokens_2");
    p->u_rope[1] = blocks(3, c.rope_depths[1]);
    p->u_tail = unit("tail");
    p->u_heads = unit("heads");
    auto starts = [](const std::string& s, const char* pre) { return s.compare(0, strlen(pre), pre) == 0; };
    p->unit_of.assign(p->names.size(), -1);
    for (size_t i = 0; i < p->names.size(); ++i) {
        const std::string& n = p->names[i];
        int u = -1, s = 0, k = 0, m = 0;
        if (starts(n, "stem.")) u = 0;
        else if (sscanf(n.c_str(), "stages.%d.%d.", &s, &k) == 2 && s >= 0 && s < 4) u = (s < 2 ? p->u_conv[s] : p->u_rope[s - 2]) + k;
        else if (sscanf(n.c_str(), "downsample_layers.%d.", &s) == 1) u = s < 2 ? p->u_down[s] : p->u_mid;
        else if (sscanf(n.c_str(), "cls_token_%d", &s) == 1 && (s == 1 || s == 2)) u = p->u_tok[s - 1];
        else if (sscanf(n.c_str(), "meta.%d.head_%d.", &m, &s) == 2 && (s == 1 || s == 2)) u = p->u_tok[s - 1];
        else if (starts(n, "norm_1.") || starts(n, "cl_1_fc.")) u = p->u_mid;
        else if (starts(n, "norm_2.") || starts(n, "aggregate.") || starts(n, "final_norm.")) u = p->u_tail;
        else if (starts(n, "head.")) u = p->u_heads;
        if (u < 0 || u >= (int)p->unit_names.size()) return false;
        p->unit_of[i] = u;
    }
    return true;
}

struct Carver {
    int64_t cur = 0;
    int64_t take(int64_t bytes) {
        const int64_t o = cur;
        cur += align_up(bytes > 0 ? bytes : 16, 256);
        return o;
    }
};

}

static void layout_workspace(lnx_plan* p);

extern "C" int lnx_plan_create(const lnx_mformer_cfg* cfg, lnx_plan** out) {
    if (!cfg || !out) FAIL("lnx_plan_create: null argument");
    const lnx_mformer_cfg& c = *cfg;
    if (c.dtype != LNX_F32 && c.dtype != LNX_BF16) FAIL("lnx_plan_create: bad dtype %d", c.dtype);
    if (c.batch <= 0 || c.img_h <= 0 || c.img_w <= 0 || c.in_chans <= 0 || c.in_chans > 4) FAIL("lnx_plan_create: bad input geometry");
    if (c.img_h % 32 != 0 || c.img_w % 32 != 0) FAIL("lnx_plan_create: image size %dx%d must be divisible by 32 (4*2*2*2 patchify)", c.img_h, c.img_w);
    for (int i = 0; i < 4; ++i)
        if (c.dims[i] <= 0 || c.dims[i] % 32 != 0 || c.dims[i] > 2048) FAIL("lnx_plan_create: dims[%d]=%d must be a multiple of 32 in (0, 2048]", i, c.dims[i]);
    for (int s = 0; s < 2; ++s) {
        if (c.conv_depths[s] < 0 || c.rope_depths[s] <= 0) FAIL("lnx_plan_create: bad depths");
        const int hd = c.rope_heads[s] > 0 && c.dims[2 + s] % c.rope_heads[s] == 0 ? c.dims[2 + s] / c.rope_heads[s] : 0;
        if (hd != 32 && hd != 64 && hd != 128)
            FAIL("lnx_plan_create: head_dim = dim / heads must be 32, 64 or 128 (dim %d, heads %d)", c.dims[2 + s], c.rope_heads[s]);
        if (c.mlp_hidden[s] <= 0 || c.mlp_hidden[s] % 16 != 0) FAIL("lnx_plan_create: mlp_hidden must be a multiple of 16");
    }
    if (c.n_meta < 0 || c.n_meta > LNX_MAX_META || c.n_tasks < 0 || c.n_tasks > LNX_MAX_TASKS) FAIL("lnx_plan_create: too many meta components / tasks");
    for (int m = 0; m < c.n_meta; ++m)
        if (c.meta_dims[m] <= 0 || c.meta_dims[m] > 16) FAIL("lnx_plan_create: meta dim %d must be in 1..16", c.meta_dims[m]);
    if (c.rope_mode != LNX_ROPE_COS && c.rope_mode != LNX_ROPE_ROTATE) FAIL("lnx_plan_create: rope_mode %d (LNX_ROPE_COS or LNX_ROPE_ROTATE)", c.rope_mode);

    if (c.fp8) {
        if (c.dtype != LNX_BF16) FAIL("lnx_plan_create: fp8 = 1 needs dtype = LNX_BF16 (fp8 operands, bf16 storage)");
        for (int s = 0; s < 2; ++s)
            if (c.dims[2 + s] % 128 != 0 || c.mlp_hidden[s] % 128 != 0)
                FAIL("lnx_plan_create: fp8 = 1 needs RoPE dims and MLP widths that are multiples of 128 (stage %d: %d / %d)", s + 2, c.dims[2 + s], c.mlp_hidden[s]);
    }
    lnx_plan* p = new lnx_plan();
    p->c = c;
    p->esz = c.dtype == LNX_BF16 ? 2 : 4;
    p->meta_chain = !env_off("LNX_META_CHAIN");
    p->ln_defer = !env_off("LNX_LN_DEFER");
    p->det = lnx_get_deterministic() != 0;
    p->freq_defer = !env_off("LNX_FREQ_DEFER");
    for (int s = 0; s < 2; ++s) p->chain_ok[s] = p->meta_chain && lnx_meta_heads_supported(c.dims[2 + s]) != 0;
    p->E = 1 + c.n_meta;
    p->H[0] = c.img_h / 4;
    p->W[0] = c.img_w / 4;
    for (int i = 1; i < 4; ++i) {
        p->H[i] = p->H[i - 1] / 2;
        p->W[i] = p->W[i - 1] / 2;
    }
    for (int i = 0; i < 4; ++i) p->HW[i] = p->H[i] * p->W[i];
    for (int s = 0; s < 2; ++s) p->Ntok[s] = p->HW[2 + s] + p->E;
    build_params(p);
    p->frozen_prefix = !env_off("LNX_FROZEN_PREFIX");
    if (!build_units(p)) {
        delete p;
        FAIL("lnx_plan_create: a parameter without a unit (build_units does not know its name)");
    }

    auto reg = [&](OpW& w) { p->all_w.push_back(&w); };
    reg(p->stem_w);
    for (int i = 0; i < 3; ++i) reg(p->down[i].w);
    for (int s = 0; s < 2; ++s)
        for (auto& k : p->conv[s]) {
            reg(k.w1);
            reg(k.w2);
        }
    for (int s = 0; s < 2; ++s)
        for (auto& k : p->rope[s]) {
            reg(k.qkv);
            reg(k.proj);
            reg(k.fc1);
            reg(k.fc2);
        }
    for (int s = 0; s < 2; ++s)
        for (auto& k : p->meta[s]) {
            reg(k.w0);
            reg(k.w1);
            reg(k.w2);
        }
    if (!c.only_last_cls) {
        reg(p->cl_w1);
        reg(p->cl_w2);
    }
    for (auto& w : p->head_w) reg(w);
    layout_workspace(p);
    *out = p;
    return 0;
}

static void layout_workspace(lnx_plan* p) {
    const lnx_mformer_cfg& c = p->c;
    const int* D = c.dims;
    const int B = c.batch;
    const int esz = p->esz;
    const int cut = p->cut;
    p->dmask_bytes = p->amask_bytes = 0;
    p->detws_floats = 0;
    Carver cv;
    int ndw = 0;
    for (int s = 0; s < 2; ++s) ndw += c.conv_depths[s];
    p->n_descs = (int64_t)p->all_w.size() + ndw;
    p->o_descs = cv.take(p->n_descs * sizeof(lnx_prep_desc));
    for (OpW* w : p->all_w) {
        const int wes = w->f32 ? 4 : 2;
        w->off = cv.take((int64_t)w->N * w->ld * wes);
        if (w->ld_t) w->off_t = cv.take((int64_t)w->K * w->ld_t * wes);
    }
    p->arena_end = cv.cur;
    for (int s = 0; s < 2; ++s)
        for (auto& k : p->conv[s]) k.w49 = cv.take((int64_t)49 * D[s] * 4);
    if (c.fp8) {
        const bool fp8_dgrad = !c.inference && !env_off("LNX_FP8_DGRAD");
        for (int s = 0; s < 2; ++s)
            for (auto& k : p->rope[s]) {
                for (OpW* w : {&k.qkv, &k.fc1, &k.fc2}) {
                    w->off8 = cv.take((int64_t)w->N * w->K);
                    w->off8s = cv.take((int64_t)(w->K / 128) * w->N * 4);
                }
                if (fp8_dgrad)
                    for (OpW* w : {&k.proj, &k.fc1, &k.fc2}) {
                        w->off8t = cv.take((int64_t)w->K * w->N);
                        w->off8ts = cv.take((int64_t)(w->N / 128) * w->K * 4);
                    }
            }
    }

    const int64_t M0 = (int64_t)B * p->HW[0];
    p->o_patches = cv.take(M0 * 64 * esz);
    p->o_stem_pre = cv.take(M0 * D[0] * esz);
    p->o_stem_mean = cv.take(M0 * 4);
    p->o_stem_rstd = cv.take(M0 * 4);
    int64_t maxMC = 0, maxM4C = 0;
    int64_t fwdMC = 0;
    bool any_fused = false;
    const bool inf = c.inference != 0;
    const bool ck = !inf && c.recompute != 0;
    const bool fuse_mlp = !env_set("LNX_NO_FUSED_MLP"), fuse_ln = !env_set("LNX_NO_FUSED_LN");
    int fuse_maxc = 2048;
    if (const char* e = getenv("LNX_FUSED_MLP_MAXC")) fuse_maxc = atoi(e);
    p->lnws_floats = (int64_t)2048 * 2 * (D[3] > D[0] ? D[3] : D[0]);
    p->lnws_side_floats = (int64_t)256 * 2 * D[3];
    if (p->det)
        for (int s = 0; s < 2; ++s) {
            const int64_t need = lnx_convmlp_bwd_ws_floats((int)D[s], (int)((int64_t)B * p->HW[s]));
            if (need > p->lnws_floats) p->lnws_floats = need;
        }
    auto frozen_blocks = [&](int first_unit, size_t nb) {
        if (inf || cut <= first_unit) return 0;
        return cut - first_unit < (int)nb ? cut - first_unit : (int)nb;
    };
    for (int s = 0; s < 2; ++s) {
        const int64_t M = (int64_t)B * p->HW[s], C = D[s];
        const bool active = cut <= p->u_down[s];
        if (active && M * C > maxMC) maxMC = M * C;
        if (active && M * 4 * C > maxM4C) maxM4C = M * 4 * C;
        int64_t pp[2] = {0, 0};
        if (inf) {
            pp[0] = cv.take(M * C * 4);
            pp[1] = cv.take(M * C * 4);
        }
        const size_t nb = p->conv[s].size();
        const int nf = frozen_blocks(p->u_conv[s], nb);
        auto stream_buf = [&](size_t k) {
            if (inf) return pp[k & 1];
            if ((int)k > nf) return cv.take(M * C * 4);
            if (pp[k & 1] == 0) pp[k & 1] = cv.take(M * C * 4);
            return pp[k & 1];
        };
        for (size_t i = 0; i < nb; ++i) {
            ConvBlk& k = p->conv[s][i];
            const bool share = i > 0 && (inf || ck || (int)i < nf);
            const ConvBlk& f = p->conv[s][0];
            k.xin = stream_buf(i);
            k.y = share ? f.y : cv.take(M * C * esz);
            k.ln = share ? f.ln : cv.take(M * C * esz);
            k.mean = share ? f.mean : cv.take(M * 4);
            k.rstd = share ? f.rstd : cv.take(M * 4);
            k.fused = lnx_convmlp_supported(c.dtype, (int)C) != 0 && fuse_mlp && C <= fuse_maxc;
            any_fused = any_fused || k.fused;
            k.fused_ln = k.fused && fuse_ln && lnx_convmlp_bwd_ws_floats((int)C, (int)M) <= p->lnws_floats;
            if (!k.fused) {
                k.hpre = share ? f.hpre : cv.take(M * 4 * C * esz);
                k.act = share ? f.act : cv.take(M * 4 * C * esz);
                k.z = share ? f.z : cv.take(M * C * esz);
            }
        }
        p->o_stage_out[s] = stream_buf(nb);
        p->down[s].ln = cv.take(M * C * esz);
        p->down[s].mean = cv.take(M * 4);
        p->down[s].rstd = cv.take(M * 4);
        p->o_g[s] = inf || !active ? 0 : cv.take(M * C * 4);
    }
// ... 392 lines not shown
    return p->ev_pool[p->ev_used++];
}
struct Timed {
    lnx_plan* p;
    hipStream_t st;
    bool on;
    lnx_plan::Span sp;
    Timed(const Ctx& c, int cls, double work, double bytes = 0.0)
        : p(c.p), st((hipStream_t)c.st), on(cls >= 0 && (cls >= 8 ? c.p->profile_spans : (c.p->profile && !c.p->profile_spans))) {
        if (on) {
            sp.cls = cls;
            sp.work = work;
            sp.bytes = bytes;
            sp.e0 = take_event(p);
            sp.e1 = take_event(p);
            (void)hipEventRecord(sp.e0, st);
        }
    }
    ~Timed() {
        if (on) {
            (void)hipEventRecord(sp.e1, st);
            p->spans.push_back(sp);
        }
    }
};
double nt_bytes(const Ctx& c, const lnx_gemm_args* a, int a_elem = 0) {
    const double e = c.p->esz, ea = a_elem ? a_elem : e, mn = (double)a->M * a->N;
    return ea * ((double)a->M * a->K + (double)a->N * a->K) + (a->out_f32 ? 4.0 : e) * mn + (a->c2 ? e * mn : 0.0) + (a->aux ? e * mn : 0.0) +
           (a->res ? 4.0 * mn : 0.0) + (a->c8 ? mn * (1.0 + 1.0 / 32) : 0.0);
}
int gemm_nt_t(const Ctx& c, const lnx_gemm_args* a) {
    Timed t(c, a->M >= 1024 ? 0 : -1, 2.0 * a->M * a->N * a->K, nt_bytes(c, a));
    return lnx_gemm_nt(a, c.st);
}

int heads_nt(const Ctx& c, lnx_gemm_args* hg, int n, bool accumulate) {
    static const bool off = env_off("LNX_HEADS_GROUP");
    int gmax = LNX_GEMM_GROUP_MAX;
    if (const char* e = getenv("LNX_HEADS_GROUP_MAX")) {
        const int v = atoi(e);
        if (v >= 1 && v < gmax) gmax = v;
    }
    for (int t0 = 0; t0 < n; t0 += gmax) {
        const int m = n - t0 < gmax ? n - t0 : gmax;
        lnx_gemm_args* g = hg + t0;
        if (accumulate && t0 > 0) {
            g[0].C = hg[0].C; g[0].ldc = hg[0].ldc; g[0].res = (const float*)hg[0].C; g[0].ldres = hg[0].ldc;
        }
        if (!off && lnx_gemm_nt_group_ok(g, m, accumulate ? 1 : 0)) {
            RUN(lnx_gemm_nt_group(g, m, accumulate ? 1 : 0, c.st));
            continue;
        }
        for (int t = 0; t < m; ++t) {
            lnx_gemm_args a = g[t];
            if (accumulate && t > 0) {
                a.C = g[0].C; a.ldc = g[0].ldc; a.res = (const float*)g[0].C; a.ldres = g[0].ldc;
            }
            RUN(gemm_nt_t(c, &a));
        }
    }
    return 0;
}

lnx_gemm_args gemm_base(const Ctx& c, int M, int N, int K, const void* A, int64_t lda, const void* W, int64_t ldw, void* C, int64_t ldc, bool out_f32) {
    lnx_gemm_args a;
    memset(&a, 0, sizeof a);
    a.dtype = c.dt;
    a.M = M;
    a.N = N;
    a.K = K;
    a.A = A;
    a.lda = lda;
    a.W = W;
    a.ldw = ldw;
    a.C = C;
    a.ldc = ldc;
    a.out_f32 = out_f32 ? 1 : 0;
    return a;
}

struct Compact {
    const int* nkeep = nullptr;
    const int* m_dev = nullptr;
    const int* perm = nullptr;
    const int* inv = nullptr;
    int rps = 0;
    explicit operator bool() const { return perm != nullptr; }
};

int ln_fwd(const Ctx& c, int M, int C, float eps, const void* x, int xdt, int64_t ldx, lnx_rowmap xm, int wi, int bi, void* y, int ydt, int64_t ldy,
           lnx_rowmap ym, const void* add, int64_t ldadd, float* mean, float* rstd, void* y8 = nullptr, void* y8s = nullptr, Compact cl = Compact()) {
    lnx_ln_args a;
    memset(&a, 0, sizeof a);
    a.perm = cl.perm; a.m_dev = cl.m_dev; a.rows_per_sample = cl.rps;
    a.y8 = y8; a.ldy8 = C; a.y8_scales = y8s;
    a.M = M; a.C = C; a.eps = eps;
    a.x = x; a.x_dtype = xdt; a.ldx = ldx; a.x_map = xm;
    a.w = c.p->P[wi]; a.b = c.p->P[bi];
    a.y = y; a.y_dtype = ydt; a.ldy = ldy; a.y_map = ym;
    a.add = add; a.ldadd = ldadd; a.mean = mean; a.rstd = rstd;
    return lnx_layernorm_fwd(&a, c.st);
}

int ln_defer_slot(const Ctx& c, float*& ws, int64_t& ws_floats) {
    lnx_plan* p = c.p;
    if (p->ln_pending == LN_DEFER_SLOTS) {
        RUN(lnx_layernorm_bwd_flush(c.st));
        p->ln_pending = 0;
    }
    ws = c.at<float>(p->o_lnws_defer) + (int64_t)p->ln_pending * p->lnws_defer_floats;
    ws_floats = p->lnws_defer_floats;
    ++p->ln_pending;
    return 0;
}

struct Dx2 {
    void* p = nullptr;
    const float* rowscale = nullptr;
    int rps = 0;
    void* p8 = nullptr;
    void* p8s = nullptr;
    const int* inv = nullptr;
    const int* nkeep = nullptr;
};
int ln_bwd(const Ctx& c, int M, int C, const void* dy, int dydt, int64_t lddy, lnx_rowmap dym, const void* x, int xdt, int64_t ldx, lnx_rowmap xm, int wi,
           int bi, const float* mean, const float* rstd, const float* gin, void* dx, int dxdt, int64_t lddx, bool relu, Dx2 d2 = Dx2(), Compact cl = Compact()) {
    lnx_ln_bwd_args a;
    memset(&a, 0, sizeof a);
    a.perm = cl.perm; a.m_dev = cl.m_dev; a.dx2_inv = d2.inv; a.dx2_nkeep = d2.nkeep;
    a.dx2 = d2.p; a.dx2_dtype = c.dt; a.lddx2 = C; a.dx2_rowscale = d2.rowscale; a.dx2_rows_per_sample = d2.rps > 0 ? d2.rps : cl.rps;
    if (d2.p && d2.p8) {
        a.dx2_8 = d2.p8; a.dx2_8_scales = d2.p8s; a.lddx2_8 = C;
    }
    a.M = M; a.C = C;
    a.dy = dy; a.dy_dtype = dydt; a.lddy = lddy; a.dy_map = dym;
    a.x = x; a.x_dtype = xdt; a.ldx = ldx; a.x_map = xm;
    a.w = c.p->P[wi]; a.mean = mean; a.rstd = rstd;
    a.gin = gin; a.ldgin = lddx;
    a.dx = dx; a.dx_dtype = dxdt; a.lddx = lddx;
    a.dw = c.p->G[wi]; a.db = c.p->G[bi];
    a.relu_mask = relu ? 1 : 0;
    const bool on_side = c.p->side != nullptr && c.st == (void*)c.p->side;
    a.ws = c.at<float>(on_side ? c.p->o_lnws_side : c.p->o_lnws);
    a.ws_floats = on_side ? c.p->lnws_side_floats : c.p->lnws_floats;
    lnx_plan* p = c.p;
    const bool on_wgs = p->wgs != nullptr && c.st == (void*)p->wgs;
    if (p->ln_defer && !on_side && !on_wgs && p->o_lnws_defer != 0 && (a.dw || a.db)) {
        RUN(ln_defer_slot(c, a.ws, a.ws_floats));
        a.defer = 1;
    }
    return lnx_layernorm_bwd(&a, c.st);
}

int wgrad_to(const Ctx& c, int M, int N, int K, const void* dY, int64_t lddy, const void* A, int64_t lda, float* dW, float* db, int64_t lddw, int k_store, int slot,
             const int* m_dev = nullptr) {
    lnx_wgrad_args a;
    memset(&a, 0, sizeof a);
    a.m_dev = m_dev;
    a.dtype = c.dt;
    a.M = M; a.N = N; a.K = K;
    a.dY = dY; a.lddy = lddy;
    a.A = A; a.lda = lda;
    a.dW = dW; a.lddw = lddw;
    a.db = db;
    a.k_store = k_store;
    if (!(c.p->side != nullptr && c.st == (void*)c.p->side)) {
        a.ws = c.at<float>(c.p->o_tnws) + (int64_t)(slot > 0 ? slot : 0) * LNX_TN_WS_FLOATS;
        a.ws_floats = LNX_TN_WS_FLOATS;
        a.defer = slot >= 0 ? 1 : 0;
    }
    Timed t(c, M >= 1024 ? 1 : -1, 2.0 * M * N * K, (double)c.p->esz * ((double)M * N + (double)M * K) + 8.0 * N * K);
    return lnx_gemm_tn(&a, c.st);
}
int wgrad(const Ctx& c, int M, int N, int K, const void* dY, int64_t lddy, const void* A, int64_t lda, int wparam, int bparam, int64_t lddw, int k_store = 0,
          int slot = -1, const int* m_dev = nullptr) {
    return wgrad_to(c, M, N, K, dY, lddy, A, lda, c.p->G[wparam], bparam >= 0 ? c.p->G[bparam] : nullptr, lddw, k_store, slot, m_dev);
}
int wgrad_into(const Ctx& c, int M, int N, int K, const void* dY, int64_t lddy, const void* A, int64_t lda, float* dW, float* db, int64_t lddw, int slot,
               const int* m_dev = nullptr) {
    return wgrad_to(c, M, N, K, dY, lddy, A, lda, dW, db, lddw, 0, slot, m_dev);
}

const lnx_rowmap IDM = {0, 0, 0};

bool fp8_rows(const lnx_plan* p, int M, int width) { return p->c.fp8 != 0 && M >= 256 && width >= 256; }
int linear_fwd(const Ctx& c, lnx_gemm_args g, const OpW& w, int64_t a8, int64_t a8s, int64_t out8 = 0, int64_t out8s = 0) {
    lnx_plan* p = c.p;
    if (!fp8_rows(p, g.M, g.K < g.N ? g.K : g.N) || w.off8s == 0) return gemm_nt_t(c, &g);
    g.A = c.at<void>(a8);
    g.lda = g.K;
    g.W = c.at<void>(w.off8);
    g.ldw = w.K;
    if (out8s) {
        g.c8 = c.at<void>(out8); g.ldc8 = g.N; g.c8_scales = c.at<void>(out8s);
    }
    Timed t(c, g.M >= 1024 ? 0 : -1, 2.0 * g.M * g.N * g.K, nt_bytes(c, &g, 1));
    return lnx_gemm_nt_mxfp8(&g, c.at<void>(a8s), c.at<void>(w.off8s), c.st);
}

int linear_dgrad(const Ctx& c, lnx_gemm_args g, const OpW& w, bool quantise, int64_t a8, int64_t a8s, int64_t out8 = 0, int64_t out8s = 0) {
    lnx_plan* p = c.p;
    if (!fp8_rows(p, g.M, g.K < g.N ? g.K : g.N) || w.off8ts == 0) return gemm_nt_t(c, &g);
    if (quantise) RUN(lnx_quantize_mxfp8(g.A, LNX_BF16, g.lda, g.M, g.K, c.at<void>(a8), g.K, c.at<void>(a8s), c.st));
    g.A = c.at<void>(a8);
    g.lda = g.K;
    g.W = c.at<void>(w.off8t);
    g.ldw = w.N;
    if (out8s) {
        g.c8 = c.at<void>(out8); g.ldc8 = g.N; g.c8_scales = c.at<void>(out8s);
    }
    Timed t(c, g.M >= 1024 ? 0 : -1, 2.0 * g.M * g.N * g.K, nt_bytes(c, &g, 1));
    return lnx_gemm_nt_mxfp8(&g, c.at<void>(a8s), c.at<void>(w.off8ts), c.st);
}

Compact conv_compact_of(const lnx_plan* p, int s, int i) {
    Compact cl;
    const ConvBlk& k = p->conv[s][i];
    const int* list = p->compact_conv_now && k.fused && k.fused_ln ? p->drop_list(p->drop_conv[s][i]) : nullptr;
    if (list == nullptr) return cl;
    cl.nkeep = list; cl.m_dev = list + 1; cl.perm = list + 2; cl.inv = list + 2 + p->c.batch; cl.rps = p->H[s] * p->W[s];
    return cl;
}

int conv_block_fwd(const Ctx& c, int s, int i, float* xout) {
    lnx_plan* p = c.p;
    ConvBlk& k = p->conv[s][i];
    const int B = p->c.batch, H = p->H[s], W = p->W[s], C = p->c.dims[s];
    const int M = B * H * W;
    p->resident[s] = i;
    Timed span(c, 9, 2.0 * M * C * (8.0 * C + 49.0));
    lnx_dwconv_args d;
    memset(&d, 0, sizeof d);
    d.B = B; d.H = H; d.W = W; d.C = C;
    d.x = c.at<float>(k.xin); d.x_dtype = LNX_F32;
    d.w49 = c.at<float>(k.w49); d.bias = p->P[k.dwb];
    d.y = c.at<void>(k.y); d.y_dtype = c.dt;
    const Compact cl = conv_compact_of(p, s, i);
    {
        Timed t(c, 4, (double)M * C * (4 + p->esz));
        RUN(lnx_dwconv7_fwd_kept(&d, cl.perm, cl.nkeep, c.st));
    }
    if (!k.fused_ln)
        RUN(ln_fwd(c, M, C, 1e-6f, c.at<void>(k.y), c.dt, C, IDM, k.lnw, k.lnb, c.at<void>(k.ln), c.dt, C, IDM, nullptr, 0, c.at<float>(k.mean), c.at<float>(k.rstd)));
    if (k.fused) {
        lnx_convmlp_args f;
        memset(&f, 0, sizeof f);
        f.dtype = c.dt; f.M = M; f.C = C;
        if (k.fused_ln) {
            f.y = c.at<void>(k.y); f.ln_w = p->P[k.lnw]; f.ln_b = p->P[k.lnb]; f.ln_eps = 1e-6f;
            if (!p->c.inference) {
                f.ln_out = c.at<void>(k.ln); f.mean = c.at<float>(k.mean); f.rstd = c.at<float>(k.rstd);
            }
        } else {
            f.ln = c.at<void>(k.ln);
        }
        f.w1 = c.wptr(k.w1); f.b1 = p->P[k.b1]; f.w2 = c.wptr(k.w2); f.b2 = p->P[k.b2];
        f.gamma = p->P[k.gamma]; f.rowscale = p->drop_ptr(p->drop_conv[s][i]); f.rows_per_sample = H * W;
        f.x = c.at<float>(k.xin); f.out = xout;
        f.perm = cl.perm; f.m_dev = cl.m_dev;
        if (cl) g_compact_conv_blocks.fetch_add(1, std::memory_order_relaxed);
        Timed t(c, 6, 2.0 * M * C * 4 * C * 2);
        RUN(lnx_convmlp_fwd(&f, c.st));
        return 0;
    }
    lnx_gemm_args g = gemm_base(c, M, 4 * C, C, c.at<void>(k.ln), C, c.wptr(k.w1), k.w1.ld, c.at<void>(k.act), 4 * C, false);
    g.bias = p->P[k.b1]; g.act = LNX_ACT_GELU;
    if (!p->c.inference) {
        g.act = LNX_ACT_GELU_D;
        g.c2 = c.at<void>(k.hpre); g.ldc2 = 4 * C;
    }
    RUN(gemm_nt_t(c, &g));
    g = gemm_base(c, M, C, 4 * C, c.at<void>(k.act), 4 * C, c.wptr(k.w2), k.w2.ld, xout, C, true);
    g.bias = p->P[k.b2]; g.c2 = c.at<void>(k.z); g.ldc2 = C;
    g.gamma = p->P[k.gamma]; g.rowscale = p->drop_ptr(p->drop_conv[s][i]); g.rows_per_sample = H * W;
    g.res = c.at<float>(k.xin); g.ldres = C;
    RUN(gemm_nt_t(c, &g));
    return 0;
}

int downsample_fwd(const Ctx& c, int i, const void* x, int xdt, int64_t ldx, lnx_rowmap xm, float* out, int64_t ldout, lnx_rowmap om) {
    lnx_plan* p = c.p;
    Down& d = p->down[i];
    const int B = p->c.batch, Hin = p->H[i], Win = p->W[i], Cin = p->c.dims[i], Cout = p->c.dims[i + 1];
    const int Min = B * Hin * Win, Mout = Min / 4;
    RUN(ln_fwd(c, Min, Cin, 1e-6f, x, xdt, ldx, xm, d.lnw, d.lnb, c.at<void>(d.ln), c.dt, Cin, IDM, nullptr, 0, c.at<float>(d.mean), c.at<float>(d.rstd)));
    lnx_gemm_args g = gemm_base(c, Mout, Cout, 4 * Cin, c.at<void>(d.ln), 0, c.wptr(d.w), d.w.ld, out, ldout, true);
    g.a_mode = LNX_ADDR_PATCH2; g.Hin = Hin; g.Win = Win; g.Cin = Cin;
    g.bias = p->P[d.cb]; g.c_map = om;
    RUN(gemm_nt_t(c, &g));
    return 0;
}

int meta_head_fwd(const Ctx& cc, int s, int m, const float* meta, int meta_width) {
    const Ctx c{cc.p, cc.st, LNX_F32};
    lnx_plan* p = c.p;
    MetaHead& k = p->meta[s][m];
    const int B = p->c.batch, C = p->c.dims[2 + s], N = p->Ntok[s];
    float* tok = c.at<float>(p->o_tok[s]);
    RUN(lnx_pack_meta(meta, meta_width, k.off, k.dim, c.at<void>(k.t0), c.dt, B, c.st));
    lnx_gemm_args g = gemm_base(c, B, C, 16, c.at<void>(k.t0), 16, c.wptr(k.w0), k.w0.ld, c.at<void>(k.h0), C, false);
    g.bias = p->P[k.b0]; g.act = LNX_ACT_RELU;
    RUN(gemm_nt_t(c, &g));
    RUN(ln_fwd(c, B, C, 1e-5f, c.at<void>(k.h0), c.dt, C, IDM, k.lnw0, k.lnb0, c.at<void>(k.x), c.dt, C, IDM, nullptr, 0, c.at<float>(k.m0), c.at<float>(k.r0)));
    g = gemm_base(c, B, C, C, c.at<void>(k.x), C, c.wptr(k.w1), k.w1.ld, c.at<void>(k.h1), C, false);
    g.bias = p->P[k.b1]; g.act = LNX_ACT_RELU;
    RUN(gemm_nt_t(c, &g));
    RUN(ln_fwd(c, B, C, 1e-5f, c.at<void>(k.h1), c.dt, C, IDM, k.nf1w, k.nf1b, c.at<void>(k.n1), c.dt, C, IDM, nullptr, 0, c.at<float>(k.m1), c.at<float>(k.r1)));
    g = gemm_base(c, B, C, C, c.at<void>(k.n1), C, c.wptr(k.w2), k.w2.ld, c.at<void>(k.h2), C, false);
    g.bias = p->P[k.b2]; g.act = LNX_ACT_RELU;
    RUN(gemm_nt_t(c, &g));
    const lnx_rowmap om = {1, N - 1, 1 + m};
    RUN(ln_fwd(c, B, C, 1e-5f, c.at<void>(k.h2), c.dt, C, IDM, k.nf2w, k.nf2b, tok, LNX_F32, C, om, c.at<void>(k.x), C, c.at<float>(k.m2), c.at<float>(k.r2)));
    return 0;
}

int meta_chain_fwd(const Ctx& c, int s_lo, int s_hi, const float* meta, int meta_width) {
    lnx_plan* p = c.p;
    lnx_meta_head_args a[2 * LNX_MAX_META];
    int n = 0;
    for (int s = s_lo; s < s_hi; ++s)
        for (int m = 0; m < p->c.n_meta; ++m) {
            MetaHead& k = p->meta[s][m];
            const int C = p->c.dims[2 + s], N = p->Ntok[s];
            lnx_meta_head_args& h = a[n++];
            memset(&h, 0, sizeof h);
// ... 212 lines not shown
        for (int s = 0; s < 2; ++s)
            for (auto& k : p->rope[s]) {
                lnx_rope_table t;
                memset(&t, 0, sizeof t);
                t.freqs = p->P[k.freqs]; t.heads = cf.rope_heads[s]; t.H = p->H[2 + s]; t.W = p->W[2 + s]; t.head_dim = cf.dims[2 + s] / cf.rope_heads[s];
                t.cos_out = c.at<float>(k.cos);
                if (cf.rope_mode == LNX_ROPE_ROTATE) {
                    t.rope_mode = LNX_ROPE_ROTATE; t.sin_out = c.at<float>(k.dsin);
                } else {
                    t.dsin_out = cf.inference ? nullptr : c.at<float>(k.dsin);
                }
                tabs.push_back(t);
            }
        if (!tabs.empty()) RUN(lnx_rope_cos_tables(tabs.data(), (int)tabs.size(), mst ? (void*)mst : stream));
    }
    if (mst) HIPRUN(hipEventRecord(p->ev_meta, mst));

    const int M0 = B * p->HW[0];
    float* first = conv_out(p, 0, -1);
    if (lnx_stem_fwd_ok(cf.dtype, cf.in_chans, cf.img_h, cf.img_w, D[0])) {
        lnx_stem_args sa;
        memset(&sa, 0, sizeof sa);
        sa.x = x; sa.w = c.wptr(p->stem_w); sa.bias = p->P[p->stem_b]; sa.ln_w = p->P[p->stem_lnw]; sa.ln_b = p->P[p->stem_lnb];
        sa.y = first;
        if (!cf.inference) {
            sa.patches = c.at<void>(p->o_patches); sa.pre = c.at<void>(p->o_stem_pre);
            sa.mean = c.at<float>(p->o_stem_mean); sa.rstd = c.at<float>(p->o_stem_rstd);
        }
        sa.B = B; sa.Cin = cf.in_chans; sa.H = cf.img_h; sa.W = cf.img_w; sa.Cout = D[0]; sa.eps = 1e-6f;
        RUN(lnx_stem_fwd(&sa, stream));
    } else {
        RUN(lnx_im2col_stem(x, B, cf.in_chans, cf.img_h, cf.img_w, c.at<void>(p->o_patches), cf.dtype, 64, stream));
        {
            lnx_gemm_args g = gemm_base(c, M0, D[0], 64, c.at<void>(p->o_patches), 64, c.wptr(p->stem_w), 64, c.at<void>(p->o_stem_pre), D[0], false);
            g.bias = p->P[p->stem_b];
            RUN(gemm_nt_t(c, &g));
        }
        RUN(ln_fwd(c, M0, D[0], 1e-6f, c.at<void>(p->o_stem_pre), cf.dtype, D[0], IDM, p->stem_lnw, p->stem_lnb, first, LNX_F32, D[0], IDM, nullptr, 0,
                   c.at<float>(p->o_stem_mean), c.at<float>(p->o_stem_rstd)));
    }

    for (int s = 0; s < 2; ++s) {
        for (int i = 0; i < cf.conv_depths[s]; ++i) RUN(conv_block_fwd(c, s, i, conv_out(p, s, i)));
        if (s == 0) {
            RUN(downsample_fwd(c, 0, c.at<float>(p->o_stage_out[0]), LNX_F32, D[0], IDM, conv_out(p, 1, -1), D[1], IDM));
        } else {
            const lnx_rowmap tm = {p->HW[2], p->E, p->E};
            RUN(downsample_fwd(c, 1, c.at<float>(p->o_stage_out[1]), LNX_F32, D[1], IDM, c.at<float>(p->o_tok[0]), D[2], tm));
        }
    }

    for (int s = 0; s < 2; ++s) {
        const int N = p->Ntok[s], C = D[2 + s];
        float* tok = c.at<float>(p->o_tok[s]);
        const lnx_rowmap clsmap = {1, N - 1, 0};
        RUN(lnx_fill_rows(p->P[p->cls[s]], tok, C, clsmap, B, C, stream));
        if (mst) {
            if (s == 0) HIPRUN(hipStreamWaitEvent((hipStream_t)stream, p->ev_meta, 0));
        } else {
            RUN(meta_fwd(c, s, s + 1, meta, mw_all));
        }
        for (int i = 0; i < cf.rope_depths[s]; ++i) RUN(rope_block_fwd(c, s, i, rope_out(p, s, i)));
        if (s == 0) {
            const int M2 = B * p->Ntok[0];
            RUN(ln_fwd(c, M2, C, 1e-5f, c.at<float>(p->o_stage_out[2]), LNX_F32, C, IDM, p->norm_w[0], p->norm_b[0], c.at<void>(p->o_t1), cf.dtype, C, IDM,
                       nullptr, 0, c.at<float>(p->o_t1_mean), c.at<float>(p->o_t1_rstd)));
            if (!cf.only_last_cls) {
                lnx_gemm_args g = gemm_base(c, B, D[2], D[2], c.at<void>(p->o_t1), (int64_t)p->Ntok[0] * D[2], c.wptr(p->cl_w1), p->cl_w1.ld, c.at<void>(p->o_cl_act),
                                            D[2], false);
                g.bias = p->P[p->cl_b1]; g.act = LNX_ACT_GELU; g.c2 = c.at<void>(p->o_cl_hpre); g.ldc2 = D[2];
                RUN(gemm_nt_t(c, &g));
                g = gemm_base(c, B, D[3], D[2], c.at<void>(p->o_cl_act), D[2], c.wptr(p->cl_w2), p->cl_w2.ld, c.at<float>(p->o_cl_u), D[3], true);
                g.bias = p->P[p->cl_b2];
                RUN(gemm_nt_t(c, &g));
                RUN(ln_fwd(c, B, D[3], 1e-5f, c.at<float>(p->o_cl_u), LNX_F32, D[3], IDM, p->cl_lnw, p->cl_lnb, c.at<float>(p->o_c1n), LNX_F32, D[3], IDM, nullptr,
                           0, c.at<float>(p->o_cl_mean), c.at<float>(p->o_cl_rstd)));
            }
            const lnx_rowmap pm = {p->HW[2], p->E, p->E};
            const lnx_rowmap tm = {p->HW[3], p->E, p->E};
            RUN(downsample_fwd(c, 2, c.at<void>(p->o_t1), cf.dtype, C, pm, c.at<float>(p->o_tok[1]), D[3], tm));
        }
    }

    {
        const int C = D[3];
        const lnx_rowmap clsrow = {1, p->Ntok[1] - 1, 0};
        RUN(ln_fwd(c, B, C, 1e-5f, c.at<float>(p->o_stage_out[3]), LNX_F32, C, clsrow, p->norm_w[1], p->norm_b[1], c.at<float>(p->o_c2n), LNX_F32, C, IDM, nullptr,
                   0, c.at<float>(p->o_n2_mean), c.at<float>(p->o_n2_rstd)));
        const float* fin_in = c.at<float>(p->o_c2n);
        if (!cf.only_last_cls) {
            RUN(lnx_agg2_fwd(c.at<float>(p->o_c1n), c.at<float>(p->o_c2n), p->P[p->agg_w], p->P[p->agg_b], c.at<float>(p->o_agg), B, C, stream));
            fin_in = c.at<float>(p->o_agg);
        }
        RUN(ln_fwd(c, B, C, 1e-5f, fin_in, LNX_F32, C, IDM, p->fin_w, p->fin_b, c.at<float>(p->o_feats), LNX_F32, C, IDM, nullptr, 0, c.at<float>(p->o_fin_mean),
                   c.at<float>(p->o_fin_rstd)));
        if (feats) HIPRUN(hipMemcpyAsync(feats, c.at<float>(p->o_feats), (size_t)B * C * 4, hipMemcpyDeviceToDevice, (hipStream_t)stream));
        if (cf.n_tasks > 0) {
            RUN(lnx_scale_cast(c.at<float>(p->o_feats), C, IDM, nullptr, 0, c.at<void>(p->o_featsT), cf.dtype, C, B, C, stream));
            lnx_gemm_args hg[LNX_MAX_TASKS];
            for (int t = 0; t < cf.n_tasks; ++t) {
                hg[t] = gemm_base(c, B, cf.task_classes[t], C, c.at<void>(p->o_featsT), C, c.wptr(p->head_w[t]), p->head_w[t].ld, logits + p->logit_off[t],
                                  p->logit_ld[t], true);
                hg[t].bias = p->P[p->head_b[t]];
            }
            RUN(heads_nt(c, hg, cf.n_tasks, false));
        }
    }
    p->fwd_done = true;
    return 0;
}

namespace {

static inline bool wg_on(const lnx_plan* p) { return p->wgs != nullptr && p->wgs_on; }
Ctx wg_ctx(const Ctx& c) { return Ctx{c.p, wg_on(c.p) ? (void*)c.p->wgs : c.st, c.dt}; }
int wg_fork(const Ctx& c, int j) {
    if (!wg_on(c.p)) return 0;
    HIPRUN(hipEventRecord(c.p->ev_wf[j], (hipStream_t)c.st));
    HIPRUN(hipStreamWaitEvent(c.p->wgs, c.p->ev_wf[j], 0));
    return 0;
}
int wg_done(const Ctx& c, int j) {
    if (!wg_on(c.p)) return 0;
    HIPRUN(hipEventRecord(c.p->ev_wj[j], c.p->wgs));
    return 0;
}
int wg_join(const Ctx& c, int j) {
    if (!wg_on(c.p)) return 0;
    HIPRUN(hipStreamWaitEvent((hipStream_t)c.st, c.p->ev_wj[j], 0));
    return 0;
}

int rope_block_bwd(const Ctx& c, int s, int i, float* g, bool have_dy) {
    lnx_plan* p = c.p;
    RopeBlk& k = p->rope[s][i];
    const int B = p->c.batch, C = p->c.dims[2 + s], heads = p->c.rope_heads[s], hid = p->c.mlp_hidden[s];
    const int N = p->Ntok[s], M = B * N, E = p->E;
    void* sA = c.at<void>(p->o_sA);
    void* sC = c.at<void>(p->o_sC);
    void* sD = c.at<void>(p->o_sD);
    Timed span(c, 8, 2.0 * rope_block_flops(B, N, C, hid));
    const Ctx cw = wg_ctx(c);
    auto wfork = [&](int j) { return wg_fork(c, j); };
    auto wdone = [&](int j) { return wg_done(c, j); };
    auto wjoin = [&](int j) { return wg_join(c, j); };
    const Compact ca = compact_of(p, p->drop_attn[s][i], M, C, N), cm = compact_of(p, p->drop_mlp[s][i], M, C, N);
    const bool prev_runs = i > 0 && p->runs(p->u_rope[s] + i - 1);
    const Compact cprev = prev_runs ? compact_of(p, p->drop_mlp[s][i - 1], M, C, N) : Compact();
    if (!have_dy) {
        if (cm) RUN(lnx_scale_cast_compact(g, C, p->drop_ptr(p->drop_mlp[s][i]), N, cm.perm, cm.m_dev, sC, c.dt, C, M, C, c.st));
        else RUN(lnx_scale_cast(g, C, IDM, p->drop_ptr(p->drop_mlp[s][i]), N, sC, c.dt, C, M, C, c.st));
    }
    if (p->dmask) RUN(lnx_dropout_mul(sC, c.dt, p->dmask + k.dm_fc2, p->inv_keep, M, C, c.st));
    RUN(wfork(0));
    RUN(wgrad(cw, M, C, hid, sC, C, c.at<void>(k.act), hid, k.fc2.param, k.fc2b, hid, 0, 0, cm.m_dev));
    RUN(wdone(0));
    lnx_gemm_args a = gemm_base(c, M, hid, C, sC, C, c.wtptr(k.fc2), k.fc2.ld_t, sA, hid, false);
    a.m_dev = cm.m_dev;
    a.act = fp8_rows(p, M, C) ? LNX_ACT_GELU_BWD : LNX_ACT_MUL_AUX; a.aux = c.at<void>(k.hpre); a.ldaux = hid;
    const bool qpass = env_set("LNX_FP8_DGRAD_QPASS");
    const bool mx_dgrad = c.dt == LNX_BF16 && fp8_rows(p, M, C) && k.fc2.off8ts != 0 && k.proj.off8ts != 0 && !p->dmask && C % 128 == 0 && !qpass;
    RUN(linear_dgrad(c, a, k.fc2, !(have_dy && p->dy8_ready), p->o_a8, p->o_a8s, p->o_h8, p->o_h8s));
    p->dy8_ready = false;
    if (p->dmask) RUN(lnx_dropout_mul(sA, c.dt, p->dmask + k.dm_hid, p->inv_keep, M, hid, c.st));
    RUN(wfork(1));
    RUN(wgrad(cw, M, hid, C, sA, hid, c.at<void>(k.n2), C, k.fc1.param, k.fc1b, C, 0, 1, cm.m_dev));
    RUN(wdone(1));
    a = gemm_base(c, M, C, hid, sA, hid, c.wtptr(k.fc1), k.fc1.ld_t, sD, C, false);
    a.m_dev = cm.m_dev;
    RUN(linear_dgrad(c, a, k.fc1, false, p->o_h8, p->o_h8s));
    RUN(wjoin(0));
    Dx2 d2;
    d2.p = sC; d2.rowscale = p->drop_ptr(p->drop_attn[s][i]); d2.rps = N; d2.inv = ca.inv; d2.nkeep = ca.nkeep;
    if (mx_dgrad) {
        d2.p8 = c.at<void>(p->o_a8); d2.p8s = c.at<void>(p->o_a8s);
    }
    RUN(ln_bwd(c, M, C, sD, c.dt, C, IDM, c.at<float>(k.xmid), LNX_F32, C, IDM, k.n2w, k.n2b, c.at<float>(k.mean2), c.at<float>(k.rstd2), g, g, LNX_F32, C, false, d2, cm));
    if (p->dmask) RUN(lnx_dropout_mul(sC, c.dt, p->dmask + k.dm_proj, p->inv_keep, M, C, c.st));
    RUN(wfork(2));
    RUN(wgrad(cw, M, C, C, sC, C, c.at<void>(k.o), C, k.proj.param, k.projb, C, 0, 2, ca.m_dev));
    RUN(wdone(2));
    a = gemm_base(c, M, C, C, sC, C, c.wtptr(k.proj), k.proj.ld_t, sD, C, false);
    a.m_dev = ca.m_dev;
    RUN(linear_dgrad(c, a, k.proj, !mx_dgrad, p->o_a8, p->o_a8s));
    RUN(wjoin(1));
    lnx_attn_bwd_args ab;
    memset(&ab, 0, sizeof ab);
    ab.dtype = c.dt; ab.B = B; ab.N = N; ab.E = E; ab.heads = heads; ab.head_dim = C / heads;
    ab.qkv = c.at<void>(k.qkvbuf); ab.cos_tab = c.at<float>(k.cos); ab.o = c.at<void>(k.o); ab.lse = c.at<float>(k.lse);
    ab.d_o = sD; ab.dqkv = sA; ab.freq_ws = c.at<float>(p->o_gcos); ab.delta = c.at<float>(p->o_delta);
    if (p->freq_defer && E < N) {
        if (p->freq_pending == FREQ_DEFER_SLOTS) {
            RUN(lnx_attn_bwd_flush(c.st));
            p->freq_pending = 0;
        }
        ab.freq_ws = c.at<float>(p->o_gcos) + (int64_t)p->freq_pending * p->gcos_floats;
        ab.defer_freqs = 1;
        ++p->freq_pending;
    }
    ab.dsin_tab = c.at<float>(k.dsin); ab.dfreqs = p->G[k.freqs];
    if (p->c.rope_mode == LNX_ROPE_ROTATE) {
        ab.rope_mode = LNX_ROPE_ROTATE; ab.sin_tab = c.at<float>(k.dsin); ab.dsin_tab = nullptr; ab.grid_w = p->W[2 + s];
    }
    if (p->amask) {
        ab.drop_mask = p->amask + k.dm_attn; ab.drop_inv_keep = p->a_inv_keep;
    }
    {
        Timed t(c, 3, 14.0 * B * (double)N * N * C);
        RUN(lnx_attn_bwd_compact(&ab, ca.nkeep, p->gcos_floats, c.st));
    }
    RUN(wfork(3));
    RUN(wgrad(cw, M, 3 * C, C, sA, 3 * C, c.at<void>(k.n1), C, k.qkv.param, k.qkvb, C, 0, 3, ca.m_dev));
    RUN(lnx_gemm_tn_flush(cw.st));
    RUN(wdone(3));
    RUN(wjoin(2));
    void* dn1 = (ca || cprev) ? sD : sC;
    a = gemm_base(c, M, C, 3 * C, sA, 3 * C, c.wtptr(k.qkv), k.qkv.ld_t, dn1, C, false);
    a.m_dev = ca.m_dev;
    RUN(gemm_nt_t(c, &a));
    Dx2 d1;
    if (prev_runs) {
        d1.p = sC; d1.rowscale = p->drop_ptr(p->drop_mlp[s][i - 1]); d1.rps = N; d1.inv = cprev.inv; d1.nkeep = cprev.nkeep;
        if (mx_dgrad) {
            d1.p8 = c.at<void>(p->o_a8); d1.p8s = c.at<void>(p->o_a8s);
            p->dy8_ready = true;
        }
    }
    RUN(ln_bwd(c, M, C, dn1, c.dt, C, IDM, c.at<float>(k.xin), LNX_F32, C, IDM, k.n1w, k.n1b, c.at<float>(k.mean1), c.at<float>(k.rstd1), g, g, LNX_F32, C, false, d1, ca));
    RUN(wjoin(3));
    return 0;
}

int conv_block_bwd(const Ctx& c, int s, int i, float* g, bool need_dx) {
    lnx_plan* p = c.p;
    ConvBlk& k = p->conv[s][i];
    const int B = p->c.batch, H = p->H[s], W = p->W[s], C = p->c.dims[s];
    const int M = B * H * W;
    void* sA = c.at<void>(p->o_sA);
    void* sC = c.at<void>(p->o_sC);
    void* sD = c.at<void>(p->o_sD);
    Timed span(c, 9, 4.0 * M * C * (8.0 * C + 49.0));
    bool forked = false, joined = false;
    const Compact cl = conv_compact_of(p, s, i);
    if (k.fused) {
        void* sB = c.at<void>(p->o_sB);
        lnx_convmlp_bwd_args f;
        memset(&f, 0, sizeof f);
        f.dtype = c.dt; f.M = M; f.C = C;
        f.g = g; f.ln = c.at<void>(k.ln); f.w1 = c.wptr(k.w1); f.b1 = p->P[k.b1];
        f.w2t = c.wtptr(k.w2); f.w1t = c.wtptr(k.w1); f.gamma = p->P[k.gamma];
        f.rowscale = p->drop_ptr(p->drop_conv[s][i]); f.rows_per_sample = H * W;
        f.act = sB; f.dh = sA; f.dz = sC; f.dln = sD; f.dgamma = p->G[k.gamma];
        f.dz_plain = 1;
        f.perm = cl.perm; f.m_dev = cl.m_dev;
        if (k.fused_ln) {
            f.y = c.at<void>(k.y); f.ln_w = p->P[k.lnw]; f.mean = c.at<float>(k.mean); f.rstd = c.at<float>(k.rstd);
            f.d_ln_w = p->G[k.lnw]; f.d_ln_b = p->G[k.lnb];
            f.ws = c.at<float>(p->o_lnws); f.ws_floats = p->lnws_floats;
            if (p->ln_defer && p->o_lnws_defer != 0 && lnx_convmlp_bwd_ws_floats(C, M) <= p->lnws_defer_floats) {
                RUN(ln_defer_slot(c, f.ws, f.ws_floats));
                f.ln_defer = 1;
            }
        }
        {
            Timed t(c, 7, 2.0 * M * C * 4 * C * 3);
            RUN(lnx_convmlp_bwd(&f, c.st));
        }
        const Ctx cw = wg_ctx(c);
        RUN(wg_fork(c, 0));
        forked = true;
        float* S = c.at<float>(p->o_lsws);
        float* T = S + (int64_t)C * 4 * C;
        HIPRUN(hipMemsetAsync(S, 0, ((size_t)C * 4 * C + C) * 4, (hipStream_t)cw.st));
        RUN(wgrad_into(cw, M, C, 4 * C, sC, C, sB, 4 * C, S, T, 4 * C, 0, cl.m_dev));
        RUN(wgrad(cw, M, 4 * C, C, sA, 4 * C, c.at<void>(k.ln), C, k.w1.param, k.b1, C, 0, 1, cl.m_dev));
        RUN(lnx_gemm_tn_flush(cw.st));
        RUN(lnx_layerscale_apply_wgrad(S, T, 4 * C, p->P[k.w2.param], p->P[k.b2], 4 * C, p->P[k.gamma], p->G[k.w2.param], p->G[k.b2], 4 * C, p->G[k.gamma], C, 4 * C, cw.st));
        RUN(wg_done(c, 0));
        if (!k.fused_ln) {
            RUN(wg_join(c, 0));
            joined = true;
        }
    } else {
        RUN(lnx_layerscale_bwd_ws(g, c.at<void>(k.z), c.dt, p->P[k.gamma], p->drop_ptr(p->drop_conv[s][i]), H * W, sC, p->G[k.gamma], M, C,
                                  p->det ? c.at<float>(p->o_detws) : nullptr, p->detws_floats, c.st));
        RUN(wgrad(c, M, C, 4 * C, sC, C, c.at<void>(k.act), 4 * C, k.w2.param, k.b2, 4 * C));
        lnx_gemm_args a = gemm_base(c, M, 4 * C, C, sC, C, c.wtptr(k.w2), k.w2.ld_t, sA, 4 * C, false);
        a.act = LNX_ACT_MUL_AUX; a.aux = c.at<void>(k.hpre); a.ldaux = 4 * C;
        RUN(gemm_nt_t(c, &a));
        RUN(wgrad(c, M, 4 * C, C, sA, 4 * C, c.at<void>(k.ln), C, k.w1.param, k.b1, C));
        a = gemm_base(c, M, C, 4 * C, sA, 4 * C, c.wtptr(k.w1), k.w1.ld_t, sD, C, false);
        RUN(gemm_nt_t(c, &a));
    }
    void* dy = sD;
    if (!k.fused_ln) {
        RUN(ln_bwd(c, M, C, sD, c.dt, C, IDM, c.at<void>(k.y), c.dt, C, IDM, k.lnw, k.lnb, c.at<float>(k.mean), c.at<float>(k.rstd), nullptr, sC, c.dt, C, false));
        dy = sC;
    }
    lnx_dwconv_wgrad_args w;
    memset(&w, 0, sizeof w);
    w.B = B; w.H = H; w.W = W; w.C = C;
    w.x = c.at<float>(k.xin); w.x_dtype = LNX_F32; w.dy = dy; w.dy_dtype = c.dt;
    w.dw = p->G[k.dww]; w.db = p->G[k.dwb];
    if (p->det) {
        w.ws = c.at<float>(p->o_detws); w.ws_floats = p->detws_floats;
    }
    {
        Timed t(c, 5, (double)M * C * (4 + p->esz));
        RUN(lnx_dwconv7_wgrad_kept(&w, cl.perm, cl.nkeep, c.st));
    }
    lnx_dwconv_args d;
    memset(&d, 0, sizeof d);
    d.B = B; d.H = H; d.W = W; d.C = C;
    d.x = dy; d.x_dtype = c.dt; d.w49 = c.at<float>(k.w49); d.bias = nullptr; d.flip = 1; d.res = g; d.y = g; d.y_dtype = LNX_F32;
    if (need_dx) {
        Timed t(c, 4, (double)M * C * (8 + p->esz));
        RUN(lnx_dwconv7_fwd_kept(&d, cl.perm, cl.nkeep, c.st));
    }
    if (forked && !joined) RUN(wg_join(c, 0));
    return 0;
}

int downsample_bwd(const Ctx& c, int i, const float* gout, int64_t ldg, lnx_rowmap gmap, const void* x, int xdt, int64_t ldx, lnx_rowmap xm, void* dx, int dxdt,
                   int64_t lddx) {
    lnx_plan* p = c.p;
    Down& d = p->down[i];
    const int B = p->c.batch, Hin = p->H[i], Win = p->W[i], Cin = p->c.dims[i], Cout = p->c.dims[i + 1];
    const int Min = B * Hin * Win, Mout = Min / 4;
    void* sA = c.at<void>(p->o_sA);
    void* sC = c.at<void>(p->o_sC);
    RUN(lnx_scale_cast(gout, ldg, gmap, nullptr, 0, sC, c.dt, Cout, Mout, Cout, c.st));
    lnx_wgrad_args w;
    memset(&w, 0, sizeof w);
    w.dtype = c.dt; w.M = Mout; w.N = Cout; w.K = 4 * Cin;
    w.dY = sC; w.lddy = Cout; w.A = c.at<void>(d.ln); w.a_mode = LNX_ADDR_PATCH2; w.Hin = Hin; w.Win = Win; w.Cin = Cin;
    w.dW = p->G[d.w.param]; w.lddw = 4 * Cin; w.k_perm_c = Cin; w.db = p->G[d.cb];
    w.ws = c.at<float>(p->o_tnws); w.ws_floats = LNX_TN_WS_FLOATS;
    {
        Timed t(c, 1, 2.0 * Mout * Cout * 4 * Cin);
        RUN(lnx_gemm_tn(&w, c.st));
    }
    lnx_gemm_args a = gemm_base(c, Mout, 4 * Cin, Cout, sC, Cout, c.wtptr(d.w), d.w.ld_t, sA, 0, false);
    a.c_mode = LNX_ADDR_PATCH2; a.Hin = Hin; a.Win = Win; a.Cin = Cin;
    RUN(gemm_nt_t(c, &a));
    RUN(ln_bwd(c, Min, Cin, sA, c.dt, Cin, IDM, x, xdt, ldx, xm, d.lnw, d.lnb, c.at<float>(d.mean), c.at<float>(d.rstd), nullptr, dx, dxdt, lddx, false));
    return 0;
}

int meta_head_bwd(const Ctx& cc, int s, int m, const float* g) {
    const Ctx c{cc.p, cc.st, LNX_F32};
    lnx_plan* p = c.p;
    MetaHead& k = p->meta[s][m];
    const int B = p->c.batch, C = p->c.dims[2 + s], N = p->Ntok[s];
    float* dtok = c.at<float>(p->o_mtmp[0]);
    void* t1 = c.at<void>(p->o_mtmp[1]);
    void* t2 = c.at<void>(p->o_mtmp[2]);
    float* dxf = c.at<float>(p->o_mtmp[3]);
    const lnx_rowmap rm = {1, N - 1, 1 + m};
    RUN(lnx_scale_cast(g, C, rm, nullptr, 0, dtok, LNX_F32, C, B, C, c.st));
    RUN(ln_bwd(c, B, C, dtok, LNX_F32, C, IDM, c.at<void>(k.h2), c.dt, C, IDM, k.nf2w, k.nf2b, c.at<float>(k.m2), c.at<float>(k.r2), nullptr, t1, c.dt, C, true));
    RUN(wgrad(c, B, C, C, t1, C, c.at<void>(k.n1), C, k.w2.param, k.b2, C));
    lnx_gemm_args a = gemm_base(c, B, C, C, t1, C, c.wtptr(k.w2), k.w2.ld_t, t2, C, false);
    RUN(gemm_nt_t(c, &a));
    RUN(ln_bwd(c, B, C, t2, c.dt, C, IDM, c.at<void>(k.h1), c.dt, C, IDM, k.nf1w, k.nf1b, c.at<float>(k.m1), c.at<float>(k.r1), nullptr, t1, c.dt, C, true));
    RUN(wgrad(c, B, C, C, t1, C, c.at<void>(k.x), C, k.w1.param, k.b1, C));
    a = gemm_base(c, B, C, C, t1, C, c.wtptr(k.w1), k.w1.ld_t, dxf, C, true);
    a.res = dtok; a.ldres = C;
    RUN(gemm_nt_t(c, &a));
    RUN(ln_bwd(c, B, C, dxf, LNX_F32, C, IDM, c.at<void>(k.h0), c.dt, C, IDM, k.lnw0, k.lnb0, c.at<float>(k.m0), c.at<float>(k.r0), nullptr, t1, c.dt, C, true));
    RUN(wgrad(c, B, C, 16, t1, C, c.at<void>(k.t0), 16, k.w0.param, k.b0, k.dim, k.dim));
    return 0;
}

int meta_bwd(const Ctx& c, int s, const float* g) {
    if (c.p->chain_ok[s]) return meta_chain_bwd(c, s, g);
    for (int m = 0; m < c.p->c.n_meta; ++m) RUN(meta_head_bwd(c, s, m, g));
    return 0;
}

int tokens_bwd(const Ctx& c, int s, const float* g) {
    lnx_plan* p = c.p;
    const int B = p->c.batch, C = p->c.dims[2 + s], N = p->Ntok[s];
    const lnx_rowmap clsmap = {1, N - 1, 0};
    RUN(lnx_colsum_rows(g, C, clsmap, p->G[p->cls[s]], B, C, c.st));
    hipStream_t const mst = meta_stream(p);
    p->meta_forked[s] = mst != nullptr;
    if (mst) {
        HIPRUN(hipEventRecord(p->ev_bfork[s], (hipStream_t)c.st));
        HIPRUN(hipStreamWaitEvent(mst, p->ev_bfork[s], 0));
        RUN(meta_bwd(Ctx{p, (void*)mst, c.dt}, s, g));
        HIPRUN(hipEventRecord(p->ev_bjoin[s], mst));
    } else {
        RUN(meta_bwd(c, s, g));
    }
    return 0;
}

int conv_block_restore(const Ctx& c, int s, int i) {
    lnx_plan* p = c.p;
    if (!p->c.recompute || p->resident[s] == i) return 0;
    return conv_block_fwd(c, s, i, conv_out(p, s, i));
}
int rope_block_restore(const Ctx& c, int s, int i) {
    lnx_plan* p = c.p;
    if (!p->c.recompute || p->resident[2 + s] == i) return 0;
    p->dy8_ready = false;
    return rope_block_fwd(c, s, i, rope_out(p, s, i));
}

int ln_flush(const Ctx& c) {
    lnx_plan* p = c.p;
    if (p->ln_pending > 0) {
        RUN(lnx_layernorm_bwd_flush(c.st));
        p->ln_pending = 0;
    }
    if (p->freq_pending > 0) {
        RUN(lnx_attn_bwd_flush(c.st));
        p->freq_pending = 0;
    }
    return 0;
}

int join_side(const Ctx& c, int s) {
    lnx_plan* p = c.p;
    if (p->meta_forked[s]) {
        HIPRUN(hipStreamWaitEvent((hipStream_t)c.st, p->ev_bjoin[s], 0));
        p->meta_forked[s] = false;
    }
// ... 281 lines not shown
```

linnaeus_amd/ops.py:

```python
from __future__ import annotations

import ctypes as C
from typing import Optional, Tuple

import torch

from . import _lib as L
from ._lib import F32, BF16

_TORCH_DT = {F32: torch.float32, BF16: torch.bfloat16}


def code_of(t: torch.Tensor) -> int:
    if t.dtype == torch.float32:
        return F32
    if t.dtype == torch.bfloat16:
        return BF16
    raise L.LnxError(f"unsupported tensor dtype {t.dtype}")


def torch_dtype(code: int) -> torch.dtype:
    return _TORCH_DT[code]


# ... 15 lines not shown

def gemm_nt(A, W, out, *, M=None, N=None, K=None, lda=None, ldw=None, ldc=None, bias=None, act=L.ACT_NONE, aux=None, c2=None,
            gamma=None, rowscale=None, rows_per_sample=0, res=None, c_map=None, a_patch=None, c_patch=None, dtype=None, m_dev=None, perm=None):
    a = L.GemmArgs()
    a.dtype = dtype if dtype is not None else code_of(W)
    a.M = M if M is not None else A.shape[0]
    a.N = N if N is not None else W.shape[0]
    a.K = K if K is not None else W.shape[1]
    a.A, a.lda = _p(A), (lda if lda is not None else (A.stride(0) if a_patch is None else 0))
    a.W, a.ldw = _p(W), (ldw if ldw is not None else W.stride(0))
    a.C, a.ldc = _p(out), (ldc if ldc is not None else (out.stride(0) if c_patch is None else 0))
    a.out_f32 = int(out.dtype == torch.float32)
    if a_patch is not None:
        a.a_mode, a.Hin, a.Win, a.Cin = L.ADDR_PATCH2, *a_patch
    if c_patch is not None:
        a.c_mode, a.Hin, a.Win, a.Cin = L.ADDR_PATCH2, *c_patch
    a.c_map = _map(c_map)
    a.bias = _p(bias)
    a.c2, a.ldc2 = _p(c2), (c2.stride(0) if c2 is not None else 0)
    a.act, a.aux, a.ldaux = act, _p(aux), (aux.stride(0) if aux is not None else 0)
    a.gamma, a.rowscale, a.rows_per_sample = _p(gamma), _p(rowscale), rows_per_sample
    a.res, a.ldres = _p(res), ((res.stride(0) if c_patch is None else 0) if res is not None else 0)
    a.m_dev, a.perm = _p(m_dev), _p(perm)
    L.check(L.lib().lnx_gemm_nt(C.byref(a), _stream()), "lnx_gemm_nt")
    return out


def gemm_nt_group(problems, accumulate=False):
    arr = (L.GemmArgs * len(problems))()
    for a, (A, W, out, bias, res) in zip(arr, problems):
        a.dtype = code_of(W)
        a.M, a.N, a.K = A.shape[0], W.shape[0], W.shape[1]
        a.A, a.lda, a.W, a.ldw = _p(A), A.stride(0), _p(W), W.stride(0)
        ref = out if out is not None else problems[0][2]
        a.C, a.ldc, a.out_f32 = _p(out), (out.stride(0) if out is not None else 0), int(ref.dtype == torch.float32)
        a.bias = _p(bias)
        a.res, a.ldres = _p(res), (res.stride(0) if res is not None else 0)
    if not L.lib().lnx_gemm_nt_group_ok(arr, len(problems), int(accumulate)):
        raise L.LnxError("lnx_gemm_nt_group: the problem list does not qualify")
    L.check(L.lib().lnx_gemm_nt_group(arr, len(problems), int(accumulate), _stream()), "lnx_gemm_nt_group")


def quantize_fp8(x, *, amax=None):
    x2 = x.reshape(-1, x.shape[-1])
    if amax is None:
        amax = torch.zeros(1, device=x.device, dtype=torch.float32)
        L.check(L.lib().lnx_amax(_p(x2), code_of(x2), C.c_int64(x2.stride(0)), x2.shape[0], x2.shape[1], _p(amax), _stream()), "lnx_amax")
    y = torch.empty(x2.shape, device=x.device, dtype=torch.uint8)
    scale = torch.empty(1, device=x.device, dtype=torch.float32)
    L.check(L.lib().lnx_quantize_fp8(_p(x2), code_of(x2), C.c_int64(x2.stride(0)), x2.shape[0], x2.shape[1], _p(amax), _p(y), C.c_int64(y.stride(0)), _p(scale), _stream()),
            "lnx_quantize_fp8")
    return y.view(torch.float8_e4m3fn).reshape(x.shape), scale


def gemm_nt_fp8(A8, a_scale, W8, w_scale, out, *, bias=None, act=L.ACT_NONE, aux=None, c2=None, rowscale=None, rows_per_sample=0, res=None):
    a = L.GemmArgs()
    a.dtype = L.BF16
    a.M, a.N, a.K = A8.shape[0], W8.shape[0], W8.shape[1]
    a.A, a.lda = _p(A8), A8.stride(0)
    a.W, a.ldw = _p(W8), W8.stride(0)
    a.C, a.ldc = _p(out), out.stride(0)
    a.out_f32 = int(out.dtype == torch.float32)
    a.bias = _p(bias)
    a.c2, a.ldc2 = _p(c2), (c2.stride(0) if c2 is not None else 0)
    a.act, a.aux, a.ldaux = act, _p(aux), (aux.stride(0) if aux is not None else 0)
    a.rowscale, a.rows_per_sample = _p(rowscale), rows_per_sample
    a.res, a.ldres = _p(res), (res.stride(0) if res is not None else 0)
    L.check(L.lib().lnx_gemm_nt_fp8(C.byref(a), _p(a_scale), _p(w_scale), _stream()), "lnx_gemm_nt_fp8")
    return out


def quantize_mxfp8(x):
    x2 = x.reshape(-1, x.shape[-1])
    rows, cols = x2.shape
    y = torch.empty(rows, cols, device=x.device, dtype=torch.uint8)
    sc = torch.empty(cols // 128, rows, 4, device=x.device, dtype=torch.uint8)
    L.check(L.lib().lnx_quantize_mxfp8(_p(x2), code_of(x2), C.c_int64(x2.stride(0)), rows, cols, _p(y), C.c_int64(y.stride(0)), _p(sc), _stream()),
            "lnx_quantize_mxfp8")
    return y.view(torch.float8_e4m3fn), sc


def dequantize_mxfp8(x8, scales):
    rows, cols = x8.shape
    e = scales.permute(1, 0, 2).reshape(rows, cols // 32).to(torch.float32) - 127.0
    return (x8.to(torch.float32).view(rows, cols // 32, 32) * torch.exp2(e).unsqueeze(-1)).view(rows, cols)


def gemm_nt_mxfp8(A8, a_scales, W8, w_scales, out, *, bias=None, act=L.ACT_NONE, aux=None, c2=None, rowscale=None, rows_per_sample=0, res=None,
                  c8=None, c8_scales=None):
    a = L.GemmArgs()
    a.dtype = L.BF16
    a.M, a.N, a.K = A8.shape[0], W8.shape[0], W8.shape[1]
    a.A, a.lda = _p(A8), A8.stride(0)
    a.W, a.ldw = _p(W8), W8.stride(0)
    a.C, a.ldc = _p(out), out.stride(0)
    a.out_f32 = int(out.dtype == torch.float32)
    a.bias = _p(bias)
    a.c2, a.ldc2 = _p(c2), (c2.stride(0) if c2 is not None else 0)
    a.act, a.aux, a.ldaux = act, _p(aux), (aux.stride(0) if aux is not None else 0)
    a.rowscale, a.rows_per_sample = _p(rowscale), rows_per_sample
    a.res, a.ldres = _p(res), (res.stride(0) if res is not None else 0)
    if c8 is not None:
        a.c8, a.ldc8, a.c8_scales = _p(c8), c8.stride(0), _p(c8_scales)
    assert tuple(a_scales.shape) == (a.K // 128, a.M, 4) and tuple(w_scales.shape) == (a.K // 128, a.N, 4)
    L.check(L.lib().lnx_gemm_nt_mxfp8(C.byref(a), _p(a_scales), _p(w_scales), _stream()), "lnx_gemm_nt_mxfp8")
    return out


def _wgrad_args(dY, A, dW, *, M=None, N=None, K=None, lda=None, lddw=None, db=None, a_patch=None, k_perm_c=0, k_store=0, splits=0, dtype=None, ws=None,
                m_dev=None, defer=False) -> L.WgradArgs:
    a = L.WgradArgs()
    a.dtype = dtype if dtype is not None else code_of(dY)
    a.M = M if M is not None else dY.shape[0]
    a.N = N if N is not None else dY.shape[1]
    a.K = K if K is not None else (A.shape[1] if a_patch is None else 4 * a_patch[2])
    a.dY, a.lddy = _p(dY), dY.stride(0)
    a.A, a.lda = _p(A), (lda if lda is not None else (A.stride(0) if a_patch is None else 0))
    if a_patch is not None:
        a.a_mode, a.Hin, a.Win, a.Cin = L.ADDR_PATCH2, *a_patch
    a.dW, a.lddw = _p(dW), (lddw if lddw is not None else dW.stride(0))
    a.k_perm_c, a.db, a.splits, a.k_store = k_perm_c, _p(db), splits, k_store
    if ws is not None:
        a.ws, a.ws_floats = _p(ws), ws.numel()
    a.m_dev = _p(m_dev)
    a.defer = int(bool(defer))
    return a


def gemm_tn(dY, A, dW, **kw):
    a = _wgrad_args(dY, A, dW, **kw)
    L.check(L.lib().lnx_gemm_tn(C.byref(a), _stream()), "lnx_gemm_tn")
    return dW


def gemm_tn_query(dY, A, dW, **kw) -> L.TnLaunch:
    a, out = _wgrad_args(dY, A, dW, **kw), L.TnLaunch()
    L.check(L.lib().lnx_gemm_tn_query(C.byref(a), C.byref(out)), "lnx_gemm_tn_query")
    return out


def gemm_tn_query_shape(*, dtype, M, N, K, lddy=None, lda=None, a_patch=None, k_perm_c=0, k_store=0, splits=0, ws_floats=0) -> L.TnLaunch:
    epv = 4 if dtype == F32 else 8
    a, out = L.WgradArgs(), L.TnLaunch()
    a.dtype, a.M, a.N, a.K = dtype, M, N, K
    a.lddy = lddy if lddy is not None else -(-N // epv) * epv
    a.lda = lda if lda is not None else (K if a_patch is None else 0)
    if a_patch is not None:
        a.a_mode, a.Hin, a.Win, a.Cin = L.ADDR_PATCH2, *a_patch
    a.k_perm_c, a.splits, a.k_store = k_perm_c, splits, k_store
    if ws_floats > 0:
        a.ws, a.ws_floats = C.c_void_p(0x1000), ws_floats
    L.check(L.lib().lnx_gemm_tn_query(C.byref(a), C.byref(out)), "lnx_gemm_tn_query")
    return out


def gemm_tn_flush():
    L.check(L.lib().lnx_gemm_tn_flush(_stream()), "lnx_gemm_tn_flush")


def _ln_args(x, w, b, y, eps, *, M=None, C_=None, ldx=None, ldy=None, x_map=None, y_map=None, add=None, ldadd=None, mean=None, rstd=None, y8=None, y8_scales=None,
             perm=None, m_dev=None, rows_per_sample=0):
    a = L.LnArgs()
    a.M = M if M is not None else x.shape[0]
    a.C = C_ if C_ is not None else x.shape[-1]
    a.eps = eps
    a.x, a.x_dtype, a.ldx, a.x_map = _p(x), code_of(x), (ldx if ldx is not None else x.stride(-2)), _map(x_map)
    a.w, a.b = _p(w), _p(b)
    a.y, a.y_dtype, a.ldy, a.y_map = _p(y), code_of(y), (ldy if ldy is not None else y.stride(-2)), _map(y_map)
    a.add, a.ldadd = _p(add), ((ldadd if ldadd is not None else add.stride(-2)) if add is not None else 0)
    a.mean, a.rstd = _p(mean), _p(rstd)
    if y8 is not None:
        a.y8, a.ldy8, a.y8_scales = _p(y8), y8.stride(0), _p(y8_scales)
    a.perm, a.m_dev, a.rows_per_sample = _p(perm), _p(m_dev), int(rows_per_sample)
    return a


def layernorm_fwd(x, w, b, y, eps, **kw):
    a = _ln_args(x, w, b, y, eps, **kw)
    L.check(L.lib().lnx_layernorm_fwd(C.byref(a), _stream()), "lnx_layernorm_fwd")
    return y


def layernorm_fwd_query(x, w, b, y, eps=0.0, **kw) -> L.LnLaunch:
    a, out = _ln_args(x, w, b, y, eps, **kw), L.LnLaunch()
    if L.lib().lnx_layernorm_fwd_query(C.byref(a), C.byref(out)) != 0:
        raise L.LnxError(f"lnx_layernorm_fwd_query refused: {L.lib().lnx_last_error().decode()}")
    return out


def _ln_bwd_args(dy, x, w, mean, rstd, dx, *, M=None, C_=None, lddy=None, ldx=None, lddx=None, dy_map=None, x_map=None, gin=None,
                 ldgin=None, dw=None, db=None, relu_mask=False, ws=None, dx2=None, lddx2=None, dx2_rowscale=None, dx2_rows_per_sample=0, dx2_8=None,
                 dx2_8_scales=None, defer=False, perm=None, m_dev=None, dx2_inv=None, dx2_nkeep=None):
    a = L.LnBwdArgs()
    a.M = M if M is not None else dy.shape[0]
    a.C = C_ if C_ is not None else x.shape[-1]
    a.dy, a.dy_dtype, a.lddy, a.dy_map = _p(dy), code_of(dy), (lddy if lddy is not None else dy.stride(-2)), _map(dy_map)
    a.x, a.x_dtype, a.ldx, a.x_map = _p(x), code_of(x), (ldx if ldx is not None else x.stride(-2)), _map(x_map)
    a.w, a.mean, a.rstd = _p(w), _p(mean), _p(rstd)
    a.gin, a.ldgin = _p(gin), ((ldgin if ldgin is not None else gin.stride(-2)) if gin is not None else 0)
    a.dx, a.dx_dtype, a.lddx = _p(dx), code_of(dx), (lddx if lddx is not None else dx.stride(-2))
    a.dw, a.db, a.relu_mask = _p(dw), _p(db), int(relu_mask)
    a.ws, a.ws_floats = _p(ws), (ws.numel() if ws is not None else 0)
    a.defer = int(defer)
    if dx2 is not None:
        a.dx2, a.dx2_dtype, a.lddx2 = _p(dx2), code_of(dx2), (lddx2 if lddx2 is not None else dx2.stride(-2))
        a.dx2_rowscale, a.dx2_rows_per_sample = _p(dx2_rowscale), int(dx2_rows_per_sample)
        if dx2_8 is not None:
            a.dx2_8, a.dx2_8_scales, a.lddx2_8 = _p(dx2_8), _p(dx2_8_scales), dx2_8.stride(-2)
    if perm is not None or dx2_inv is not None:
        a.dx2_rows_per_sample = int(dx2_rows_per_sample)
    a.perm, a.m_dev, a.dx2_inv, a.dx2_nkeep = _p(perm), _p(m_dev), _p(dx2_inv), _p(dx2_nkeep)
    return a


def layernorm_bwd(dy, x, w, mean, rstd, dx, **kw):
    a = _ln_bwd_args(dy, x, w, mean, rstd, dx, **kw)
    L.check(L.lib().lnx_layernorm_bwd(C.byref(a), _stream()), "lnx_layernorm_bwd")
    return dx


def layernorm_bwd_query(dy, x, w, mean, rstd, dx, **kw) -> L.LnLaunch:
    a, out = _ln_bwd_args(dy, x, w, mean, rstd, dx, **kw), L.LnLaunch()
    if L.lib().lnx_layernorm_bwd_query(C.byref(a), C.byref(out)) != 0:
        raise L.LnxError(f"lnx_layernorm_bwd_query refused: {L.lib().lnx_last_error().decode()}")
    return out


def layernorm_bwd_flush():
    L.check(L.lib().lnx_layernorm_bwd_flush(_stream()), "lnx_layernorm_bwd_flush")


def dwconv7(x, w49, bias, y, *, flip=False, res=None, perm=None, nkeep=None):
    B, H, W, Cc = x.shape
    a = L.DwconvArgs()
    a.B, a.H, a.W, a.C = B, H, W, Cc
    a.x, a.x_dtype, a.w49, a.bias = _p(x), code_of(x), _p(w49), _p(bias)
    a.flip, a.res, a.y, a.y_dtype = int(flip), _p(res), _p(y), code_of(y)
    if perm is not None:
        L.check(L.lib().lnx_dwconv7_fwd_kept(C.byref(a), _p(perm), _p(nkeep), _stream()), "lnx_dwconv7_fwd_kept")
        return y
    L.check(L.lib().lnx_dwconv7_fwd(C.byref(a), _stream()), "lnx_dwconv7_fwd")
    return y


def dwconv7_wgrad(x, dy, dw, db, *, perm=None, nkeep=None):
    B, H, W, Cc = x.shape
    a = L.DwconvWgradArgs()
    a.B, a.H, a.W, a.C = B, H, W, Cc
    a.x, a.x_dtype, a.dy, a.dy_dtype, a.dw, a.db = _p(x), code_of(x), _p(dy), code_of(dy), _p(dw), _p(db)
    if L.is_deterministic():
        ws = torch.empty(max(dwconv7_wgrad_ws_floats(B, H, W, Cc, a.x_dtype, a.dy_dtype), 1), device=x.device, dtype=torch.float32)
        a.ws, a.ws_floats = _p(ws), ws.numel()
    if perm is not None:
        L.check(L.lib().lnx_dwconv7_wgrad_kept(C.byref(a), _p(perm), _p(nkeep), _stream()), "lnx_dwconv7_wgrad_kept")
        return
    L.check(L.lib().lnx_dwconv7_wgrad(C.byref(a), _stream()), "lnx_dwconv7_wgrad")


def dwconv7_wgrad_ws_floats(B, H, W, Cc, x_dtype, dy_dtype) -> int:
    return int(L.lib().lnx_dwconv7_wgrad_ws_floats(B, H, W, Cc, x_dtype, dy_dtype))


def rope_cos_table(freqs, H, W, out=None, dsin=None):
    heads, half = freqs.shape[1], freqs.shape[2]
    if out is None:
        out = torch.empty(H * W, heads, half, device=freqs.device, dtype=torch.float32)
    L.check(L.lib().lnx_rope_cos_table_hd(_p(freqs), heads, 2 * half, H, W, _p(out), _p(dsin) if dsin is not None else None, _stream()),
            "lnx_rope_cos_table_hd")
    return out


def rope_cossin_table(freqs, H, W):
    heads, half = freqs.shape[1], freqs.shape[2]
    cos = torch.empty(H * W, heads, half, device=freqs.device, dtype=torch.float32)
    sin = torch.empty_like(cos)
    L.check(L.lib().lnx_rope_cossin_table_hd(_p(freqs), heads, 2 * half, H, W, _p(cos), _p(sin), None, _stream()), "lnx_rope_cossin_table_hd")
    return cos, sin


def rope_cos_tables(entries):
    arr = (L.RopeTable * len(entries))()
    for t, (freqs, H, W, out, dsin, *rest) in zip(arr, entries):
        t.freqs, t.cos_out, t.dsin_out = _p(freqs), _p(out), _p(dsin) if dsin is not None else None
        t.heads, t.H, t.W, t.head_dim = freqs.shape[1], H, W, 2 * freqs.shape[2]
        if rest and rest[0] is not None:
            t.rope_mode, t.sin_out = L.ROPE_ROTATE, _p(rest[0])
    L.check(L.lib().lnx_rope_cos_tables(arr, len(entries), _stream()), "lnx_rope_cos_tables")


def attn_bwd_ws_floats(B, N, heads, head_dim=64):
    fn = L.lib().lnx_attn_bwd_ws_floats_hd
    fn.restype = C.c_int64
    return int(fn(B, N, heads, head_dim))


def _head_dim(qkv, heads, head_dim):
    if head_dim is not None:
        return int(head_dim)
    return qkv.shape[-1] // (3 * heads) if qkv.dim() >= 2 and qkv.shape[-1] % (3 * heads) == 0 else 64


def attn_fwd(qkv, cos_tab, o, lse, B, N, E, heads, *, drop_mask=None, drop_rate=0.0, head_dim=None, sin_tab=None, nkeep=None):
    a = L.AttnArgs()
    if sin_tab is not None:
        a.rope_mode, a.sin_tab = L.ROPE_ROTATE, _p(sin_tab)
    a.dtype, a.B, a.N, a.E, a.heads = code_of(qkv), B, N, E, heads
# ... 377 lines not shown
```

Baseline: 13890 images/sec.

## Group pairs of weight-gradient GEMMs into a single ring-kernel launch

Adds a grouped TN (weight-gradient) GEMM kernel that runs up to four products in one launch, with a shared split plan and per-product block ranges. The transformer MLP (fc2+fc1), attention (proj+qkv) and conv-block pointwise wgrads are now issued as pairs when the pair is eligible. The aim is fewer launches and better CU fill, since small wgrad products under-occupy the GPU. In exchange, the first wgrad of each pair is delayed until the second one's input is ready, which reduces overlap with dgrad. The grouped kernel also reserves the larger LDS footprint for both tile orientations, which may lower occupancy.

Measured after the change: 13660 images/sec. -1.6%, worse.

```diff
diff --git a/include/lnx.h b/include/lnx.h
--- a/include/lnx.h
+++ b/include/lnx.h
@@ -114,6 +114,10 @@
 int lnx_gemm_tn_query(const lnx_wgrad_args* args, lnx_tn_launch* out);
 int lnx_gemm_tn_flush(void* stream);
 int lnx_gemm_tn_discard(void);
+
+int lnx_gemm_tn_group_ok(const lnx_wgrad_args* products, int n);
+int lnx_gemm_tn_group_query(const lnx_wgrad_args* products, int n, lnx_tn_launch* out, int* grid);
+int lnx_gemm_tn_group(const lnx_wgrad_args* products, int n, void* stream);
 
 
 typedef struct lnx_ln_args {
diff --git a/linnaeus_amd/_lib.py b/linnaeus_amd/_lib.py
--- a/linnaeus_amd/_lib.py
+++ b/linnaeus_amd/_lib.py
@@ -379,6 +379,10 @@
             _lib.lnx_plan_set_trainable.argtypes = [C.c_void_p, C.c_char_p]
         if hasattr(_lib, "lnx_gemm_tn_query"):
             _lib.lnx_gemm_tn_query.argtypes = [C.POINTER(WgradArgs), C.POINTER(TnLaunch)]
+        if hasattr(_lib, "lnx_gemm_tn_group"):
+            _lib.lnx_gemm_tn_group_ok.argtypes = [C.POINTER(WgradArgs), C.c_int]
+            _lib.lnx_gemm_tn_group_query.argtypes = [C.POINTER(WgradArgs), C.c_int, C.POINTER(TnLaunch), C.POINTER(C.c_int)]
+            _lib.lnx_gemm_tn_group.argtypes = [C.POINTER(WgradArgs), C.c_int, C.c_void_p]
         if hasattr(_lib, "lnx_layernorm_fwd_query"):
             _lib.lnx_layernorm_fwd_query.argtypes = [C.POINTER(LnArgs), C.POINTER(LnLaunch)]
             _lib.lnx_layernorm_bwd_query.argtypes = [C.POINTER(LnBwdArgs), C.POINTER(LnLaunch)]
@@ -412,7 +416,7 @@
 
 EXPORTS = [
     "lnx_last_error", "lnx_version", "lnx_device_cus", "lnx_set_cu_margin", "lnx_set_deterministic", "lnx_get_deterministic", "lnx_tile_sched_static",
-    "lnx_gemm_nt", "lnx_last_nt_kernel", "lnx_nt_kernel_launches", "lnx_nt_dispatch", "lnx_gemm_tn", "lnx_gemm_tn_query", "lnx_gemm_tn_flush", "lnx_gemm_tn_discard", "lnx_amax", "lnx_quantize_fp8", "lnx_gemm_nt_fp8", "lnx_quantize_mxfp8", "lnx_gemm_nt_mxfp8", "lnx_dropout_mul", "lnx_dropout_residual", "lnx_plan_dropout_bytes", "lnx_plan_set_dropout", "lnx_plan_attn_dropout_bytes", "lnx_plan_set_attn_dropout",
+    "lnx_gemm_nt", "lnx_last_nt_kernel", "lnx_nt_kernel_launches", "lnx_nt_dispatch", "lnx_gemm_tn", "lnx_gemm_tn_query", "lnx_gemm_tn_flush", "lnx_gemm_tn_discard", "lnx_gemm_tn_group_ok", "lnx_gemm_tn_group_query", "lnx_gemm_tn_group", "lnx_amax", "lnx_quantize_fp8", "lnx_gemm_nt_fp8", "lnx_quantize_mxfp8", "lnx_gemm_nt_mxfp8", "lnx_dropout_mul", "lnx_dropout_residual", "lnx_plan_dropout_bytes", "lnx_plan_set_dropout", "lnx_plan_attn_dropout_bytes", "lnx_plan_set_attn_dropout",
     "lnx_layernorm_fwd", "lnx_layernorm_bwd", "lnx_layernorm_bwd_flush", "lnx_layernorm_bwd_discard", "lnx_layernorm_fwd_query", "lnx_layernorm_bwd_query",
     "lnx_dwconv7_fwd", "lnx_dwconv7_fwd_kept", "lnx_dwconv7_wgrad", "lnx_dwconv7_wgrad_kept", "lnx_dwconv7_wgrad_ws_floats",
     "lnx_gemm_nt_group_ok", "lnx_gemm_nt_group", "lnx_rope_cos_table", "lnx_rope_cos_table_hd", "lnx_rope_cossin_table_hd", "lnx_rope_cos_tables", "lnx_attn_bwd_ws_floats", "lnx_attn_bwd_ws_floats_hd", "lnx_attn_fwd", "lnx_attn_bwd", "lnx_attn_bwd_sized", "lnx_attn_fwd_compact", "lnx_attn_bwd_compact", "lnx_attn_bwd_flush", "lnx_attn_bwd_discard", "lnx_attn_dispatch", "lnx_last_attn_kernel", "lnx_last_attn_bwd_launches",
diff --git a/linnaeus_amd/csrc/api.cpp b/linnaeus_amd/csrc/api.cpp
--- a/linnaeus_amd/csrc/api.cpp
+++ b/linnaeus_amd/csrc/api.cpp
@@ -19,7 +19,7 @@
 }
 
 extern "C" const char* lnx_last_error(void) { return g_err; }
-extern "C" int lnx_version(void) { return 118; }
+extern "C" int lnx_version(void) { return 119; }
 extern "C" int lnx_device_cus(void) {
     int dev = 0;
     if (hipGetDevice(&dev) != hipSuccess) return -1;
diff --git a/linnaeus_amd/csrc/gemm2.hip b/linnaeus_amd/csrc/gemm2.hip
--- a/linnaeus_amd/csrc/gemm2.hip
+++ b/linnaeus_amd/csrc/gemm2.hip
@@ -260,7 +260,7 @@
     } while (0)
 
 template <int RW, int CW, bool PATCH>
-__global__ __launch_bounds__(512) void gemm_tn_v2_kernel(const WgradP p) {
+__device__ __forceinline__ void tn_v2_body(const WgradP& p, const int block) {
     typedef bf16_t T;
     constexpr int RROW = RW * 2, CROW = CW * 2;
     constexpr int RBYTES = TBM * RROW, CBYTES = TBM * CROW;
@@ -276,7 +276,7 @@
     const int wr = wave / WC, wc = wave % WC;
     const int s = lane & 15, g = lane >> 4;
 
-    int bid = xcd_remap(blockIdx.x, p.tiles_n * p.tiles_k * p.splits);
+    int bid = xcd_remap(block, p.tiles_n * p.tiles_k * p.splits);
     const int split = bid / (p.tiles_n * p.tiles_k);
     bid -= split * (p.tiles_n * p.tiles_k);
     const int tc = bid % p.tiles_k;
@@ -466,6 +466,28 @@
     }
 }
 
+template <int RW, int CW, bool PATCH>
+__global__ __launch_bounds__(512) void gemm_tn_v2_kernel(const WgradP p) {
+    tn_v2_body<RW, CW, PATCH>(p, (int)blockIdx.x);
+}
+
+constexpr int TN_GROUP = 4;
+struct TnGroupP {
+    WgradP p[TN_GROUP];
+    int block_start[TN_GROUP];
+    int wide_r[TN_GROUP];
+    int n;
+};
+__global__ __launch_bounds__(512) void gemm_tn_v2_group_kernel(const TnGroupP b) {
+    int j = 0;
+#pragma unroll
+    for (int i = 1; i < TN_GROUP; ++i)
+        if (i < b.n && (int)blockIdx.x >= b.block_start[i]) j = i;
+    const int block = (int)blockIdx.x - b.block_start[j];
+    if (b.wide_r[j]) tn_v2_body<256, 128, false>(b.p[j], block);
+    else tn_v2_body<128, 256, false>(b.p[j], block);
+}
+
 __device__ __forceinline__ void tn_reduce_body(const WgradP& p, int RW, int CW, const int64_t idx) {
     const int tiles = p.tiles_n * p.tiles_k;
     const int tile_f4 = RW * CW / 4;
@@ -576,6 +598,24 @@
     return n;
 }
 
+static void tn_second_stage(const WgradP& p, int RW, int CW, hipStream_t st, bool defer) {
+    const int tiles = p.tiles_n * p.tiles_k;
+    const int64_t work = (int64_t)tiles * (RW * CW / 4) + (p.db ? p.N : 0);
+    const int blocks = (int)cdiv(work, 256);
+    if (defer) {
+        if (g_tn_pending.n > 0 && (g_tn_pending_stream != st || g_tn_pending.n == TN_BATCH)) (void)tn_flush(nullptr);
+        TnReduceDesc& d = g_tn_pending.d[g_tn_pending.n++];
+        d.p = p;
+        d.RW = RW;
+        d.CW = CW;
+        d.block_start = g_tn_pending_blocks;
+        g_tn_pending_blocks += blocks;
+        g_tn_pending_stream = st;
+    } else {
+        hipLaunchKernelGGL(gemm_tn_reduce_kernel, dim3((unsigned)blocks), dim3(256), 0, st, p, RW, CW);
+    }
+}
+
 int launch_tn_v2(const WgradP& p, const TnPlan& t, hipStream_t st, bool defer) {
     static_assert(TBM == TN_RING_ROWS, "tn_plan splits the contraction in this kernel's ring stages");
     const bool wide_r = t.RW == 256, patch = t.patch;
@@ -587,23 +627,25 @@
     if (wide_r) rc = patch ? launch_with_lds<gemm_tn_v2_kernel<256, 128, true>>(grid, 512, lds, st, p) : launch_with_lds<gemm_tn_v2_kernel<256, 128, false>>(grid, 512, lds, st, p);
     else rc = patch ? launch_with_lds<gemm_tn_v2_kernel<128, 256, true>>(grid, 512, lds, st, p) : launch_with_lds<gemm_tn_v2_kernel<128, 256, false>>(grid, 512, lds, st, p);
     if (rc != 0) return rc;
-    if (p.ws) {
-        const int64_t work = (int64_t)tiles * (RW * CW / 4) + (p.db ? p.N : 0);
-        const int blocks = (int)cdiv(work, 256);
-        if (defer) {
-            if (g_tn_pending.n > 0 && (g_tn_pending_stream != st || g_tn_pending.n == TN_BATCH)) (void)tn_flush(nullptr);
-            TnReduceDesc& d = g_tn_pending.d[g_tn_pending.n++];
-            d.p = p;
-            d.RW = RW;
-            d.CW = CW;
-            d.block_start = g_tn_pending_blocks;
-            g_tn_pending_blocks += blocks;
-            g_tn_pending_stream = st;
-        } else {
-            hipLaunchKernelGGL(gemm_tn_reduce_kernel, dim3((unsigned)blocks), dim3(256), 0, st, p, RW, CW);
-        }
-    }
+    if (p.ws) tn_second_stage(p, RW, CW, st, defer);
     return 0;
 }
 
-}
+int launch_tn_v2_group(const WgradP* p, const TnGroupPlan& g, hipStream_t st, const bool* defer) {
+    static_assert(TN_GROUP == TN_GROUP_MAX, "TnGroupPlan and the kernel's batch hold the same number of products");
+    TnGroupP b{};
+    b.n = g.n;
+    for (int j = 0; j < g.n; ++j) {
+        b.p[j] = p[j];
+        b.block_start[j] = g.block_start[j];
+        b.wide_r[j] = g.t[j].RW == 256 ? 1 : 0;
+    }
+    const size_t lds = NarrowRing::NST * (size_t)(TBM * (256 + 128) * 2);
+    const int rc = launch_with_lds<gemm_tn_v2_group_kernel>(g.grid, 512, lds, st, b);
+    if (rc != 0) return rc;
+    for (int j = 0; j < g.n; ++j)
+        if (p[j].ws) tn_second_stage(p[j], g.t[j].RW, g.t[j].CW, st, defer[j]);
+    return 0;
+}
+
+}
diff --git a/linnaeus_amd/csrc/gemm_common.hpp b/linnaeus_amd/csrc/gemm_common.hpp
--- a/linnaeus_amd/csrc/gemm_common.hpp
+++ b/linnaeus_amd/csrc/gemm_common.hpp
@@ -606,5 +606,15 @@
 int tn_discard();
 bool tn_v2_ok(const WgradP& p, int dtype);
 
+constexpr int TN_GROUP_MAX = 4;
+struct TnGroupPlan {
+    int n;
+    TnPlan t[TN_GROUP_MAX];
+    int block_start[TN_GROUP_MAX];
+    int grid;
+};
+const char* tn_group_plan(const WgradP* p, const int* dtype, int n, int splits_hint, TnGroupPlan& g);
+int launch_tn_v2_group(const WgradP* p, const TnGroupPlan& g, hipStream_t st, const bool* defer);
+
 }
 using namespace lnxg;
diff --git a/linnaeus_amd/csrc/gemm_tn_dispatch.cpp b/linnaeus_amd/csrc/gemm_tn_dispatch.cpp
--- a/linnaeus_amd/csrc/gemm_tn_dispatch.cpp
+++ b/linnaeus_amd/csrc/gemm_tn_dispatch.cpp
@@ -6,6 +6,22 @@
 
 bool tn_v2_ok(const WgradP& p, int dtype) {
     return dtype == LNX_BF16 && p.M % TN_RING_ROWS == 0 && p.M >= 4096 && p.N >= 8 && p.K >= 8;
+}
+
+static void tn_ring_tiles(const WgradP& p, TnPlan& t) {
+    auto waste = [&](int rw, int cw) { return (double)cdiv(p.N, rw) * rw * cdiv(p.K, cw) * cw; };
+    static const char* force = getenv("LNX_TN_ORIENT");
+    const bool wide_r = force ? force[0] == 'r' : waste(256, 128) <= waste(128, 256);
+    t.RW = wide_r ? 256 : 128;
+    t.CW = wide_r ? 128 : 256;
+    t.tiles_n = cdiv(p.N, t.RW);
+    t.tiles_k = cdiv(p.K, t.CW);
+}
+
+static bool tn_wants_workspace(const WgradP& p, const TnPlan& t, bool fits) {
+    static const bool no_ws = getenv("LNX_TN_ATOMIC") != nullptr;
+    const bool sparse_tiles = (double)p.N * p.k_store < 0.7 * (double)(t.tiles_n * t.tiles_k) * (256 * 128);
+    return !(no_ws || p.ws == nullptr || !fits || t.splits < 2 || sparse_tiles);
 }
 
 TnPlan tn_plan(const WgradP& p, int dtype, int splits_hint) {
@@ -33,14 +49,8 @@
         t.workspace = false;
         return t;
     }
-    auto waste = [&](int rw, int cw) { return (double)cdiv(p.N, rw) * rw * cdiv(p.K, cw) * cw; };
-    static const char* force = getenv("LNX_TN_ORIENT");
-    const bool wide_r = force ? force[0] == 'r' : waste(256, 128) <= waste(128, 256);
-    const int RW = wide_r ? 256 : 128, CW = wide_r ? 128 : 256;
-    t.RW = RW;
-    t.CW = CW;
-    t.tiles_n = cdiv(p.N, RW);
-    t.tiles_k = cdiv(p.K, CW);
+    tn_ring_tiles(p, t);
+    const int RW = t.RW;
     const int tiles = t.tiles_n * t.tiles_k;
     const int mtiles = p.M / TN_RING_ROWS;
     int splits = splits_hint;
@@ -61,11 +71,62 @@
     const int per = cdiv(mtiles, splits);
     t.m_per_split = per * TN_RING_ROWS;
     t.splits = cdiv(mtiles, per);
-    static const bool no_ws = getenv("LNX_TN_ATOMIC") != nullptr;
-    const bool sparse_tiles = (double)p.N * p.k_store < 0.7 * (double)tiles * (256 * 128);
     if (det) t.workspace = t.splits >= 2;
-    else t.workspace = !(no_ws || p.ws == nullptr || have < ws_need(t.splits) || t.splits < 2 || sparse_tiles);
+    else t.workspace = tn_wants_workspace(p, t, have >= ws_need(t.splits));
     return t;
+}
+
+const char* tn_group_plan(const WgradP* p, const int* dtype, int n, int splits_hint, TnGroupPlan& g) {
+    g = TnGroupPlan{};
+    if (n < 1 || n > TN_GROUP_MAX) return "a group holds 1 to 4 products";
+    if (nt_switches().force_v1) return "LNX_GEMM_V1 is set: no ring kernel";
+    int sum_tiles = 0;
+    for (int j = 0; j < n; ++j) {
+        if (p[j].a_mode == LNX_ADDR_PATCH2) return "patch-mode products are launched alone";
+        if (!tn_v2_ok(p[j], dtype[j])) return "every member must be a ring-kernel product (bf16, M % 64 == 0, M >= 4096)";
+        if (p[j].M != p[0].M || p[j].m_dev != p[0].m_dev) return "the members must share M and m_dev";
+        g.t[j].ring = true;
+        g.t[j].patch = false;
+        tn_ring_tiles(p[j], g.t[j]);
+        sum_tiles += g.t[j].tiles_n * g.t[j].tiles_k;
+    }
+    g.n = n;
+    const int mtiles = p[0].M / TN_RING_ROWS;
+    int splits = splits_hint;
+    if (splits <= 0) {
+        splits = 256 / sum_tiles;
+        if (splits < 1) splits = 1;
+        const int max_splits = mtiles / 8 > 0 ? mtiles / 8 : 1;
+        if (splits > max_splits) splits = max_splits;
+    }
+    if (splits > mtiles) splits = mtiles;
+    if (splits < 1) splits = 1;
+    const bool det = deterministic();
+    auto ws_need = [&](int j, int sp) { return (size_t)sp * g.t[j].tiles_n * g.t[j].tiles_k * (256 * 128) + (size_t)sp * g.t[j].tiles_n * g.t[j].RW; };
+    auto have = [&](int j) { return p[j].ws ? (size_t)p[j].ws_floats : (size_t)0; };
+    if (det) {
+        auto fits = [&](int sp) {
+            const int as_launched = cdiv(mtiles, cdiv(mtiles, sp));
+            for (int j = 0; j < n; ++j)
+                if (ws_need(j, as_launched) > have(j)) return false;
+            return true;
+        };
+        while (splits > 1 && !fits(splits)) --splits;
+    }
+    const int per = cdiv(mtiles, splits);
+    splits = cdiv(mtiles, per);
+    int start = 0;
+    for (int j = 0; j < n; ++j) {
+        TnPlan& t = g.t[j];
+        t.m_per_split = per * TN_RING_ROWS;
+        t.splits = splits;
+        if (det) t.workspace = splits >= 2;
+        else t.workspace = tn_wants_workspace(p[j], t, have(j) >= ws_need(j, splits));
+        g.block_start[j] = start;
+        start += t.tiles_n * t.tiles_k * splits;
+    }
+    g.grid = start;
+    return nullptr;
 }
 
 }
@@ -108,14 +169,7 @@
     p.m_dev = a->m_dev;
 }
 
-}
-
-extern "C" int lnx_gemm_tn_query(const lnx_wgrad_args* a, lnx_tn_launch* out) {
-    LNX_CHECK(out != nullptr, "lnx_gemm_tn_query: null result");
-    if (tn_check_sizes(a, "lnx_gemm_tn_query") != 0) return 1;
-    WgradP p;
-    fill_wgrad_p(a, p);
-    const TnPlan t = tn_plan(p, a->dtype, a->splits);
+void tn_report(const TnPlan& t, lnx_tn_launch* out) {
     out->kernel = t.ring ? LNX_TN_KERNEL_RING : LNX_TN_KERNEL_V1;
     out->rw = t.RW;
     out->cw = t.CW;
@@ -125,6 +179,87 @@
     out->splits = t.splits;
     out->m_per_split = t.m_per_split;
     out->workspace = t.workspace ? 1 : 0;
+}
+
+}
+
+extern "C" int lnx_gemm_tn_query(const lnx_wgrad_args* a, lnx_tn_launch* out) {
+    LNX_CHECK(out != nullptr, "lnx_gemm_tn_query: null result");
+    if (tn_check_sizes(a, "lnx_gemm_tn_query") != 0) return 1;
+    WgradP p;
+    fill_wgrad_p(a, p);
+    const TnPlan t = tn_plan(p, a->dtype, a->splits);
+    tn_report(t, out);
+    return 0;
+}
+
+namespace {
+
+bool tn_no_defer() {
+    static const bool no_defer = getenv("LNX_TN_NO_DEFER") != nullptr;
+    return no_defer;
+}
+
+const char TN_SIZES_REFUSED[] = "";
+const char* tn_group_setup(const lnx_wgrad_args* a, int n, const char* who, WgradP* p, TnGroupPlan& g) {
+    if (a == nullptr || n < 1 || n > TN_GROUP_MAX) return "a group holds 1 to 4 products";
+    int dtype[TN_GROUP_MAX];
+    for (int j = 0; j < n; ++j) {
+        if (tn_check_sizes(&a[j], who) != 0) return TN_SIZES_REFUSED;
+        if (a[j].splits != a[0].splits) return "the members must ask for the same splits";
+        fill_wgrad_p(&a[j], p[j]);
+        dtype[j] = a[j].dtype;
+    }
+    return tn_group_plan(p, dtype, n, a[0].splits, g);
+}
+
+}
+
+extern "C" int lnx_gemm_tn_group_ok(const lnx_wgrad_args* a, int n) {
+    WgradP p[TN_GROUP_MAX];
+    TnGroupPlan g;
+    return tn_group_setup(a, n, "lnx_gemm_tn_group_ok", p, g) == nullptr ? 1 : 0;
+}
+
+extern "C" int lnx_gemm_tn_group_query(const lnx_wgrad_args* a, int n, lnx_tn_launch* out, int* grid) {
+    LNX_CHECK(out != nullptr, "lnx_gemm_tn_group_query: null result");
+    WgradP p[TN_GROUP_MAX];
+    TnGroupPlan g;
+    const char* why = tn_group_setup(a, n, "lnx_gemm_tn_group_query", p, g);
+    if (why == TN_SIZES_REFUSED) return 1;
+    LNX_CHECK(why == nullptr, "lnx_gemm_tn_group_query: %s", why);
+    for (int j = 0; j < n; ++j) tn_report(g.t[j], &out[j]);
+    if (grid) *grid = g.grid;
+    return 0;
+}
+
+extern "C" int lnx_gemm_tn_group(const lnx_wgrad_args* a, int n, void* stream) {
+    WgradP p[TN_GROUP_MAX];
+    TnGroupPlan g;
+    const char* why = tn_group_setup(a, n, "lnx_gemm_tn_group", p, g);
+    if (why == TN_SIZES_REFUSED) return 1;
+    LNX_CHECK(why == nullptr, "lnx_gemm_tn_group: %s", why);
+    bool defer[TN_GROUP_MAX];
+    for (int j = 0; j < n; ++j) {
+        LNX_CHECK(a[j].dY && a[j].A && a[j].dW, "lnx_gemm_tn_group: null operand (product %d)", j);
+        LNX_CHECK((((uintptr_t)a[j].A) & 15) == 0 && (((uintptr_t)a[j].dY) & 15) == 0, "lnx_gemm_tn_group: operands must be 16-byte aligned (product %d)", j);
+        const TnPlan& t = g.t[j];
+        p[j].tiles_n = t.tiles_n;
+        p[j].tiles_k = t.tiles_k;
+        p[j].splits = t.splits;
+        p[j].m_per_split = t.m_per_split;
+        if (!t.workspace) p[j].ws = nullptr;
+        defer[j] = a[j].defer != 0 && !tn_no_defer();
+        for (int i = 0; i < j; ++i) {
+            if (!p[i].ws || !p[j].ws) continue;
+            const size_t ni = (size_t)t.splits * (g.t[i].tiles_n * g.t[i].tiles_k * (256 * 128) + g.t[i].tiles_n * g.t[i].RW);
+            const size_t nj = (size_t)t.splits * (t.tiles_n * t.tiles_k * (256 * 128) + t.tiles_n * t.RW);
+            LNX_CHECK(p[i].ws + ni <= p[j].ws || p[j].ws + nj <= p[i].ws, "lnx_gemm_tn_group: products %d and %d share workspace", i, j);
+        }
+    }
+    const int rc = launch_tn_v2_group(p, g, (hipStream_t)stream, defer);
+    if (rc != 0) return rc;
+    LNX_LAUNCH_CHECK();
     return 0;
 }
 
@@ -141,9 +276,8 @@
     p.m_per_split = t.m_per_split;
     if (t.ring && !t.workspace) p.ws = nullptr;
     hipStream_t st = (hipStream_t)stream;
-    static const bool no_defer = getenv("LNX_TN_NO_DEFER") != nullptr;
     int rc;
-    if (t.ring) rc = launch_tn_v2(p, t, st, a->defer != 0 && !no_defer);
+    if (t.ring) rc = launch_tn_v2(p, t, st, a->defer != 0 && !tn_no_defer());
     else rc = launch_tn_v1(p, a->dtype, st);
     if (rc != 0) return rc;
     LNX_LAUNCH_CHECK();
diff --git a/linnaeus_amd/csrc/plan.cpp b/linnaeus_amd/csrc/plan.cpp
--- a/linnaeus_amd/csrc/plan.cpp
+++ b/linnaeus_amd/csrc/plan.cpp
@@ -133,6 +133,7 @@
     int64_t gcos_floats = 0;
     int freq_pending = 0;
     bool freq_defer = true;
+    bool tn_group = true;
     bool ln_defer = true;
     int64_t o_tnws = 0;
     int64_t o_lsws = 0, lsws_floats = 0;
@@ -436,6 +437,7 @@
     p->esz = c.dtype == LNX_BF16 ? 2 : 4;
     p->meta_chain = !env_off("LNX_META_CHAIN");
     p->ln_defer = !env_off("LNX_LN_DEFER");
+    p->tn_group = !env_off("LNX_TN_GROUP");
     p->det = lnx_get_deterministic() != 0;
     p->freq_defer = !env_off("LNX_FREQ_DEFER");
     for (int s = 0; s < 2; ++s) p->chain_ok[s] = p->meta_chain && lnx_meta_heads_supported(c.dims[2 + s]) != 0;
@@ -1134,8 +1136,8 @@
     return lnx_layernorm_bwd(&a, c.st);
 }
 
-int wgrad_to(const Ctx& c, int M, int N, int K, const void* dY, int64_t lddy, const void* A, int64_t lda, float* dW, float* db, int64_t lddw, int k_store, int slot,
-             const int* m_dev = nullptr) {
+lnx_wgrad_args wgrad_args(const Ctx& c, int M, int N, int K, const void* dY, int64_t lddy, const void* A, int64_t lda, float* dW, float* db, int64_t lddw, int k_store,
+                          int slot, const int* m_dev) {
     lnx_wgrad_args a;
     memset(&a, 0, sizeof a);
     a.m_dev = m_dev;
@@ -1151,8 +1153,19 @@
         a.ws_floats = LNX_TN_WS_FLOATS;
         a.defer = slot >= 0 ? 1 : 0;
     }
-    Timed t(c, M >= 1024 ? 1 : -1, 2.0 * M * N * K, (double)c.p->esz * ((double)M * N + (double)M * K) + 8.0 * N * K);
+    return a;
+}
+double wgrad_bytes(const Ctx& c, const lnx_wgrad_args& a) { return (double)c.p->esz * ((double)a.M * a.N + (double)a.M * a.K) + 8.0 * a.N * a.K; }
+int wgrad_to(const Ctx& c, int M, int N, int K, const void* dY, int64_t lddy, const void* A, int64_t lda, float* dW, float* db, int64_t lddw, int k_store, int slot,
+             const int* m_dev = nullptr) {
+    const lnx_wgrad_args a = wgrad_args(c, M, N, K, dY, lddy, A, lda, dW, db, lddw, k_store, slot, m_dev);
+    Timed t(c, M >= 1024 ? 1 : -1, 2.0 * M * N * K, wgrad_bytes(c, a));
     return lnx_gemm_tn(&a, c.st);
+}
+bool wgrad_pair_ok(const Ctx& c, const lnx_wgrad_args* ab) { return c.p->tn_group && lnx_gemm_tn_group_ok(ab, 2) != 0; }
+int wgrad_pair(const Ctx& c, const lnx_wgrad_args* ab) {
+    Timed t(c, ab[0].M >= 1024 ? 1 : -1, 2.0 * ab[0].M * ((double)ab[0].N * ab[0].K + (double)ab[1].N * ab[1].K), wgrad_bytes(c, ab[0]) + wgrad_bytes(c, ab[1]));
+    return lnx_gemm_tn_group(ab, 2, c.st);
 }
 int wgrad(const Ctx& c, int M, int N, int K, const void* dY, int64_t lddy, const void* A, int64_t lda, int wparam, int bparam, int64_t lddw, int k_store = 0,
           int slot = -1, const int* m_dev = nullptr) {
@@ -1671,9 +1684,18 @@
         else RUN(lnx_scale_cast(g, C, IDM, p->drop_ptr(p->drop_mlp[s][i]), N, sC, c.dt, C, M, C, c.st));
     }
     if (p->dmask) RUN(lnx_dropout_mul(sC, c.dt, p->dmask + k.dm_fc2, p->inv_keep, M, C, c.st));
-    RUN(wfork(0));
-    RUN(wgrad(cw, M, C, hid, sC, C, c.at<void>(k.act), hid, k.fc2.param, k.fc2b, hid, 0, 0, cm.m_dev));
-    RUN(wdone(0));
+    const lnx_wgrad_args w_mlp[2] = {
+        wgrad_args(cw, M, C, hid, sC, C, c.at<void>(k.act), hid, p->G[k.fc2.param], k.fc2b >= 0 ? p->G[k.fc2b] : nullptr, hid, 0, 0, cm.m_dev),
+        wgrad_args(cw, M, hid, C, sA, hid, c.at<void>(k.n2), C, p->G[k.fc1.param], k.fc1b >= 0 ? p->G[k.fc1b] : nullptr, C, 0, 1, cm.m_dev)};
+    const lnx_wgrad_args w_attn[2] = {
+        wgrad_args(cw, M, C, C, sC, C, c.at<void>(k.o), C, p->G[k.proj.param], k.projb >= 0 ? p->G[k.projb] : nullptr, C, 0, 2, ca.m_dev),
+        wgrad_args(cw, M, 3 * C, C, sA, 3 * C, c.at<void>(k.n1), C, p->G[k.qkv.param], k.qkvb >= 0 ? p->G[k.qkvb] : nullptr, C, 0, 3, ca.m_dev)};
+    const bool pair_mlp = wgrad_pair_ok(cw, w_mlp), pair_attn = wgrad_pair_ok(cw, w_attn);
+    if (!pair_mlp) {
+        RUN(wfork(0));
+        RUN(wgrad(cw, M, C, hid, sC, C, c.at<void>(k.act), hid, k.fc2.param, k.fc2b, hid, 0, 0, cm.m_dev));
+        RUN(wdone(0));
+    }
     lnx_gemm_args a = gemm_base(c, M, hid, C, sC, C, c.wtptr(k.fc2), k.fc2.ld_t, sA, hid, false);
     a.m_dev = cm.m_dev;
     a.act = fp8_rows(p, M, C) ? LNX_ACT_GELU_BWD : LNX_ACT_MUL_AUX; a.aux = c.at<void>(k.hpre); a.ldaux = hid;
@@ -1683,12 +1705,13 @@
     p->dy8_ready = false;
     if (p->dmask) RUN(lnx_dropout_mul(sA, c.dt, p->dmask + k.dm_hid, p->inv_keep, M, hid, c.st));
     RUN(wfork(1));
-    RUN(wgrad(cw, M, hid, C, sA, hid, c.at<void>(k.n2), C, k.fc1.param, k.fc1b, C, 0, 1, cm.m_dev));
+    if (pair_mlp) RUN(wgrad_pair(cw, w_mlp));
+    else RUN(wgrad(cw, M, hid, C, sA, hid, c.at<void>(k.n2), C, k.fc1.param, k.fc1b, C, 0, 1, cm.m_dev));
     RUN(wdone(1));
     a = gemm_base(c, M, C, hid, sA, hid, c.wtptr(k.fc1), k.fc1.ld_t, sD, C, false);
     a.m_dev = cm.m_dev;
     RUN(linear_dgrad(c, a, k.fc1, false, p->o_h8, p->o_h8s));
-    RUN(wjoin(0));
+    RUN(wjoin(pair_mlp ? 1 : 0));
     Dx2 d2;
     d2.p = sC; d2.rowscale = p->drop_ptr(p->drop_attn[s][i]); d2.rps = N; d2.inv = ca.inv; d2.nkeep = ca.nkeep;
     if (mx_dgrad) {
@@ -1696,9 +1719,11 @@
     }
     RUN(ln_bwd(c, M, C, sD, c.dt, C, IDM, c.at<float>(k.xmid), LNX_F32, C, IDM, k.n2w, k.n2b, c.at<float>(k.mean2), c.at<float>(k.rstd2), g, g, LNX_F32, C, false, d2, cm));
     if (p->dmask) RUN(lnx_dropout_mul(sC, c.dt, p->dmask + k.dm_proj, p->inv_keep, M, C, c.st));
-    RUN(wfork(2));
-    RUN(wgrad(cw, M, C, C, sC, C, c.at<void>(k.o), C, k.proj.param, k.projb, C, 0, 2, ca.m_dev));
-    RUN(wdone(2));
+    if (!pair_attn) {
+        RUN(wfork(2));
+        RUN(wgrad(cw, M, C, C, sC, C, c.at<void>(k.o), C, k.proj.param, k.projb, C, 0, 2, ca.m_dev));
+        RUN(wdone(2));
+    }
     a = gemm_base(c, M, C, C, sC, C, c.wtptr(k.proj), k.proj.ld_t, sD, C, false);
     a.m_dev = ca.m_dev;
     RUN(linear_dgrad(c, a, k.proj, !mx_dgrad, p->o_a8, p->o_a8s));
@@ -1729,10 +1754,11 @@
         RUN(lnx_attn_bwd_compact(&ab, ca.nkeep, p->gcos_floats, c.st));
     }
     RUN(wfork(3));
-    RUN(wgrad(cw, M, 3 * C, C, sA, 3 * C, c.at<void>(k.n1), C, k.qkv.param, k.qkvb, C, 0, 3, ca.m_dev));
+    if (pair_attn) RUN(wgrad_pair(cw, w_attn));
+    else RUN(wgrad(cw, M, 3 * C, C, sA, 3 * C, c.at<void>(k.n1), C, k.qkv.param, k.qkvb, C, 0, 3, ca.m_dev));
     RUN(lnx_gemm_tn_flush(cw.st));
     RUN(wdone(3));
-    RUN(wjoin(2));
+    RUN(wjoin(pair_attn ? 3 : 2));
     void* dn1 = (ca || cprev) ? sD : sC;
     a = gemm_base(c, M, C, 3 * C, sA, 3 * C, c.wtptr(k.qkv), k.qkv.ld_t, dn1, C, false);
     a.m_dev = ca.m_dev;
@@ -1791,8 +1817,14 @@
         float* S = c.at<float>(p->o_lsws);
         float* T = S + (int64_t)C * 4 * C;
         HIPRUN(hipMemsetAsync(S, 0, ((size_t)C * 4 * C + C) * 4, (hipStream_t)cw.st));
-        RUN(wgrad_into(cw, M, C, 4 * C, sC, C, sB, 4 * C, S, T, 4 * C, 0, cl.m_dev));
-        RUN(wgrad(cw, M, 4 * C, C, sA, 4 * C, c.at<void>(k.ln), C, k.w1.param, k.b1, C, 0, 1, cl.m_dev));
+        const lnx_wgrad_args w_pw[2] = {wgrad_args(cw, M, C, 4 * C, sC, C, sB, 4 * C, S, T, 4 * C, 0, 0, cl.m_dev),
+                                        wgrad_args(cw, M, 4 * C, C, sA, 4 * C, c.at<void>(k.ln), C, p->G[k.w1.param], k.b1 >= 0 ? p->G[k.b1] : nullptr, C, 0, 1, cl.m_dev)};
+        if (wgrad_pair_ok(cw, w_pw)) {
+            RUN(wgrad_pair(cw, w_pw));
+        } else {
+            RUN(wgrad_into(cw, M, C, 4 * C, sC, C, sB, 4 * C, S, T, 4 * C, 0, cl.m_dev));
+            RUN(wgrad(cw, M, 4 * C, C, sA, 4 * C, c.at<void>(k.ln), C, k.w1.param, k.b1, C, 0, 1, cl.m_dev));
+        }
         RUN(lnx_gemm_tn_flush(cw.st));
         RUN(lnx_layerscale_apply_wgrad(S, T, 4 * C, p->P[k.w2.param], p->P[k.b2], 4 * C, p->P[k.gamma], p->G[k.w2.param], p->G[k.b2], 4 * C, p->G[k.gamma], C, 4 * C, cw.st));
         RUN(wg_done(c, 0));
diff --git a/linnaeus_amd/ops.py b/linnaeus_amd/ops.py
--- a/linnaeus_amd/ops.py
+++ b/linnaeus_amd/ops.py
@@ -191,6 +191,47 @@
         a.ws, a.ws_floats = C.c_void_p(0x1000), ws_floats
     L.check(L.lib().lnx_gemm_tn_query(C.byref(a), C.byref(out)), "lnx_gemm_tn_query")
     return out
+
+
+def _wgrad_group(products):
+    arr = (L.WgradArgs * len(products))()
+    for i, (dY, A, dW, kw) in enumerate(products):
+        arr[i] = _wgrad_args(dY, A, dW, **kw)
+    return arr
+
+
+def gemm_tn_group(products):
+    arr = _wgrad_group(products)
+    L.check(L.lib().lnx_gemm_tn_group(arr, len(products), _stream()), "lnx_gemm_tn_group")
+    return [p[2] for p in products]
+
+
+def gemm_tn_group_ok(products) -> bool:
+    return bool(L.lib().lnx_gemm_tn_group_ok(_wgrad_group(products), len(products)))
+
+
+def gemm_tn_group_query(products):
+    arr, out, grid = _wgrad_group(products), (L.TnLaunch * len(products))(), C.c_int(0)
+    L.check(L.lib().lnx_gemm_tn_group_query(arr, len(products), out, C.byref(grid)), "lnx_gemm_tn_group_query")
+    return list(out), grid.value
+
+
+def gemm_tn_group_query_shapes(shapes):
+    n = len(shapes)
+    arr, out, grid = (L.WgradArgs * max(n, 1))(), (L.TnLaunch * max(n, 1))(), C.c_int(0)
+    for a, sh in zip(arr, shapes):
+        epv = 4 if sh["dtype"] == F32 else 8
+        a.dtype, a.M, a.N, a.K = sh["dtype"], sh["M"], sh["N"], sh["K"]
+        a.lddy = -(-sh["N"] // epv) * epv
+        a.lda = sh["K"] if "patch" not in sh else 0
+        if "patch" in sh:
+            a.a_mode, a.Hin, a.Win, a.Cin = L.ADDR_PATCH2, *sh["patch"]
+        a.splits = sh.get("splits", 0)
+        if sh.get("ws_floats", 0) > 0:
+            a.ws, a.ws_floats = C.c_void_p(0x1000), sh["ws_floats"]
+        a.m_dev = C.c_void_p(sh.get("m_dev", 0) or None)
+    L.check(L.lib().lnx_gemm_tn_group_query(arr, n, out, C.byref(grid)), "lnx_gemm_tn_group_query")
+    return list(out)[:n], grid.value
 
 
 def gemm_tn_flush():
```
